# apache/cloudberry

Hardware: NVIDIA H100
Metric: TPC-H SF100 Q1 rows/sec (higher is better)
Workload: dtype int64

## Files before the change

### cloudberry_b200/capi.py

```python
import ctypes as C
import os
import re

import numpy as np

from . import plan as P
from .relation import HostRelation, NP_DTYPE

HERE = os.path.dirname(os.path.abspath(__file__))
ROOT = os.path.dirname(HERE)
_GPU = None
_EXEC = None


class CbgpuError(RuntimeError):
    def __init__(self, code, msg):
        super().__init__("cbgpu error %d: %s" % (code, msg))
        self.code = code


class CbgpuVisimapEntry(C.Structure):
    _fields_ = [("first_row_num", C.c_int64), ("data", C.c_void_p), ("len", C.c_int32)]


class CbgpuPairs(C.Structure):
    _fields_ = [("npairs", C.c_int64), ("outer_idx", C.c_void_p), ("inner_idx", C.c_void_p)]


class CbpOp(C.Structure):
    _fields_ = [("code", C.c_int32), ("a", C.c_int32), ("imm", C.c_int64)]


class CbpColumn(C.Structure):
    _fields_ = [("data", C.c_void_p), ("nulls", C.c_void_p), ("dict_hash", C.c_void_p), ("type", C.c_int32), ("src", C.c_int32)]


class CbgpuJoinFilter(C.Structure):
    _fields_ = [("ncols", C.c_int32), ("cols", C.POINTER(CbpColumn)), ("nops", C.c_int32), ("ops", C.POINTER(CbpOp))]


(CBP_END, CBP_LOAD, CBP_CONST, CBP_ADD, CBP_SUB, CBP_MUL, CBP_FADD, CBP_FSUB, CBP_FMUL, CBP_I2F, CBP_EQ, CBP_NE, CBP_LT, CBP_LE,
 CBP_GT, CBP_GE, CBP_FEQ, CBP_FNE, CBP_FLT, CBP_FLE, CBP_FGT, CBP_FGE, CBP_AND, CBP_OR, CBP_NOT, CBP_FILTER, CBP_PROBE, CBP_DUP,
 CBP_POP, CBP_F8ORD) = range(30)


def join_filter(cols, ops):
    ca = (CbpColumn * max(len(cols), 1))()
    for i, (rel, c, src) in enumerate(cols):
        L = rel.ctx.L
        ca[i] = CbpColumn(L.cbgpu_rel_col_devptr(rel.h, c), L.cbgpu_rel_nulls_dev(rel.h, c), L.cbgpu_rel_dict_hash_dev(rel.h, c),
                          L.cbgpu_rel_col_type(rel.h, c), src)
    oa = (CbpOp * max(len(ops), 1))(*[CbpOp(code, a, imm) for code, a, imm in ops])
    f = CbgpuJoinFilter(len(cols), ca, len(ops), oa)
    f._keep = (ca, oa)
    return f


class CbAggStateDatum(C.Structure):
    _fields_ = [("n", C.c_int64), ("lo", C.c_int64), ("hi", C.c_int64)]


TUPSER_STATE_NUMERIC, TUPSER_STATE_INT8 = 101, 102


class CbTupAttr(C.Structure):
    _fields_ = [("type", C.c_int32), ("dscale", C.c_int32), ("bpchar_len", C.c_int32), ("ntexts", C.c_int32),
                ("texts", C.POINTER(C.c_char_p)), ("text_lens", C.POINTER(C.c_int32)), ("state", C.POINTER(CbAggStateDatum))]


def _tup_attrs(attrs):
    arr = (CbTupAttr * max(len(attrs), 1))()
    keep = []
    for i, a in enumerate(attrs):
        arr[i].type, arr[i].dscale, arr[i].bpchar_len = a[0], a[1], a[2]
        if a[0] in (TUPSER_STATE_NUMERIC, TUPSER_STATE_INT8):
            st = CbAggStateDatum()
            keep.append(st)
            arr[i].state = C.pointer(st)
        texts = a[3] if len(a) > 3 and a[3] is not None else []
        if texts:
            bufs = [C.create_string_buffer(bytes(t), len(t)) for t in texts]
            ptrs = (C.c_char_p * len(texts))(*[C.cast(b, C.c_char_p) for b in bufs])
            lens = (C.c_int32 * len(texts))(*[len(t) for t in texts])
            keep += [bufs, ptrs, lens]
            arr[i].ntexts = len(texts)
            arr[i].texts = ptrs
            arr[i].text_lens = lens
    return arr, keep


def tupser_rows(attrs, rows, nulls=None, max_chunk=8160, end=True):
    L = ex()
    n = len(attrs)
    arr, keep = _tup_attrs(attrs)
    out = bytearray()
    buf = C.create_string_buffer(1 << 20)
    for r, row in enumerate(rows):
        cells, held = [], []
        for i, v in enumerate(row):
            if attrs[i][0] in (TUPSER_STATE_NUMERIC, TUPSER_STATE_INT8) and v is not None:
                st = CbAggStateDatum(*[int(x) for x in v])
                held.append(st)
                cells.append(C.addressof(st))
            else:
                cells.append(0 if v is None else int(v))
        vals = (C.c_int64 * max(n, 1))(*cells)
        isn = (C.c_uint8 * max(n, 1))(*([int(x) for x in nulls[r]] if nulls is not None else [0] * n))
        k = L.cb_tupser_row(arr, n, vals, isn, max_chunk, buf, len(buf))
        if k < 0:
            raise CbgpuError(int(k), "cb_tupser_row failed")
        out += buf.raw[:k]
    if end:
        k = L.cb_tupser_end_of_stream(buf, len(buf))
        out += buf.raw[:k]
    return bytes(out)


def tupser_parse(attrs, data):
    L = ex()
    n = len(attrs)
    arr, keep = _tup_attrs(attrs)
    buf = C.create_string_buffer(bytes(data), len(data))
    pos = 0
    rows, nulls = [], []
    vals = (C.c_int64 * max(n, 1))()
    isn = (C.c_uint8 * max(n, 1))()
    used = C.c_int64()
    while True:
        rc = L.cb_tupser_next(arr, n, C.byref(buf, pos), len(data) - pos, C.byref(used), vals, isn)
        if rc == 1:
            row = []
            for i in range(n):
                if attrs[i][0] in (TUPSER_STATE_NUMERIC, TUPSER_STATE_INT8) and not isn[i]:
                    st = arr[i].state.contents
                    row.append((int(st.n), int(st.lo), int(st.hi)))
                else:
                    row.append(int(vals[i]))
            rows.append(row)
            nulls.append([int(isn[i]) for i in range(n)])
            pos += used.value
            continue
        if rc == 0:
            return rows, nulls, pos + used.value, True
        if rc == -1:
            return rows, nulls, pos, False
        raise CbgpuError(int(rc), "cb_tupser_next: malformed chunk stream at byte %d" % pos)


class CbAocsColumnSpec(C.Structure):
    _fields_ = [("relcol", C.c_int32), ("filenum", C.c_int32), ("attlen", C.c_int32), ("varkind", C.c_int32), ("typalign", C.c_int32),
                ("compresstype", C.c_int32), ("eof", C.c_int64), ("dict", C.c_void_p)]


def aocs_column_spec(c):
    return CbAocsColumnSpec(*c[:7], c[7].h if len(c) > 7 and c[7] is not None else None)


def aocs_dict_collect_segfile(ctx, basepath, segno, checksum, col):
    spec = aocs_column_spec(col)
    err = C.create_string_buffer(512)
    rc = ex().cb_aocs_dict_collect_segfile(ctx.h, os.fsencode(basepath), segno, 1 if checksum else 0, C.byref(spec), err, 512)
    if rc != 0:
        raise CbgpuError(rc, err.value.decode() or ctx.error())


def aocs_segfile_path(basepath, segno, filenum):
    buf = C.create_string_buffer(4096)
    if ex().cb_aocs_segfile_path(os.fsencode(basepath), segno, filenum, buf, 4096) != 0:
        return None
    return os.fsdecode(buf.value)


class DeviceDict:

    def __init__(self, ctx, max_entries=4096, arena_bytes=1 << 20, bpchar=True):
        self.ctx = ctx
        h = C.c_void_p()
        ctx.check(ctx.L.cbgpu_dict_create(ctx.h, max_entries, arena_bytes, 1 if bpchar else 0, C.byref(h)))
        self.h = h

    def collect(self, file_bytes, checksum, compresstype=0, typalign=4):
        buf = np.frombuffer(file_bytes, dtype=np.uint8)
        self.ctx.check(self.ctx.L.cbgpu_aocs_dict_collect(self.ctx.h, buf.ctypes.data, len(buf), 1 if checksum else 0, compresstype, typalign,
                                                          self.h))

    def finalize(self):
        n = C.c_int32()
        self.ctx.check(self.ctx.L.cbgpu_dict_finalize(self.h, C.byref(n)))
        return int(n.value)

    def entries(self):
        out = []
        n = self.finalize()
        p = C.c_void_p()
        ln = C.c_int32()
        f = self.ctx.L.cbgpu_dict_entry
        f.argtypes = [C.c_void_p, C.c_int32, C.POINTER(C.c_void_p), C.POINTER(C.c_int32)]
        for i in range(n):
            self.ctx.check(f(self.h, i, C.byref(p), C.byref(ln)))
            out.append(C.string_at(p.value, ln.value))
        return out

    def lookup(self, text):
        b = text if isinstance(text, bytes) else text.encode()
        return int(self.ctx.L.cbgpu_dict_lookup(self.h, b, len(b)))

    def free(self):
        if self.h:
            self.ctx.L.cbgpu_dict_free(self.h)
            self.h = None


class CbNumericDatum(C.Structure):
    _fields_ = [("lo", C.c_int64), ("hi", C.c_int64), ("dscale", C.c_int32), ("text", C.c_char * 84)]


class CbTupleTableSlot(C.Structure):
    _fields_ = [("tts_empty", C.c_bool), ("tts_nvalid", C.c_int32), ("tts_types", C.POINTER(C.c_int32)),
                ("tts_values", C.POINTER(C.c_int64)), ("tts_isnull", C.POINTER(C.c_bool)),
                ("tts_state_n", C.POINTER(C.c_int64)), ("tts_state_lo", C.POINTER(C.c_int64)),
                ("tts_state_hi", C.POINTER(C.c_int64))]


class CbInstrumentation(C.Structure):
    _fields_ = [("ntuples", C.c_double), ("nloops", C.c_double), ("kernels", C.c_int64), ("device_ms", C.c_double),
                ("rows_in", C.c_int64), ("motion_repartitions", C.c_int64), ("hashjoin_nbatch", C.c_int64), ("agg_npartitions", C.c_int64)]


class CbPlanState(C.Structure):
    pass


CbPlanState._fields_ = [
    ("type", C.c_int), ("plan", C.POINTER(P.CbPlan)), ("state", C.c_void_p), ("ExecProcNode", C.c_void_p),
    ("instrument", CbInstrumentation), ("lefttree", C.POINTER(CbPlanState)), ("righttree", C.POINTER(CbPlanState)),
    ("ps_ResultTupleSlot", C.POINTER(CbTupleTableSlot)), ("squelched", C.c_bool), ("priv", C.c_void_p),
]


class CbEState(C.Structure):
    _fields_ = [("es_ctx", C.c_void_p), ("es_nrels", C.c_int32), ("es_range_table", C.POINTER(C.c_void_p)),
                ("es_segindex", C.c_int32), ("es_numsegments", C.c_int32), ("es_interconnect", C.c_void_p),
                ("es_errcode", C.c_int32), ("es_errmsg", C.c_char * 512), ("es_error_hook", C.c_void_p),
                ("es_force_generic", C.c_int32), ("es_processed", C.c_int64), ("es_cluster", C.c_void_p),
                ("es_interrupt_pending", C.c_void_p), ("es_interrupt_arg", C.c_void_p), ("es_operator_mem_kb", C.c_int64),
                ("es_hashjoin_batches_run", C.c_int64), ("es_agg_partitions_run", C.c_int64)]


def header_symbols(header):
    text = open(os.path.join(ROOT, "include", header)).read()
    text = re.sub(r"/\*.*?\*/", "", text, flags=re.S)
    names = set()
    for m in re.finditer(r"\b((?:cbgpu|cb)_[A-Za-z0-9_]+)\s*\(", text):
        name = m.group(1)
        if name.startswith(("cb_type_width",)):
            continue
        names.add(name)
    return sorted(names)


def build():
    import subprocess
    subprocess.check_call(["make", "-s", "-C", os.path.join(HERE, "csrc"), "-j8", "all"])


def _preload_bundled_nccl():
    try:
        import importlib.util
        spec = importlib.util.find_spec("nvidia.nccl")
        for d in (spec.submodule_search_locations if spec else []):
            cand = os.path.join(d, "lib", "libnccl.so.2")
            if os.path.exists(cand):
                C.CDLL(cand, mode=C.RTLD_GLOBAL)
                return
    except Exception:
        pass


def gpu():
    global _GPU
    if _GPU is None:
        so = os.path.join(os.environ.get("CBGPU_LIBDIR") or HERE, "libcbgpu.so")
        if not os.path.exists(so):
            raise CbgpuError(-1, "libcbgpu.so is not built (run __graft_entry__.build()); there is no CPU fallback")
        _preload_bundled_nccl()
        L = C.CDLL(so, mode=C.RTLD_GLOBAL)
        vp, i32, i64, u64, dbl = C.c_void_p, C.c_int32, C.c_int64, C.c_uint64, C.c_double
        sig = {
            "cbgpu_ctx_create": (C.c_int, [C.c_int, C.POINTER(vp)]),
            "cbgpu_ctx_destroy": (None, [vp]),
            "cbgpu_last_error": (C.c_char_p, [vp]),
            "cbgpu_sync": (C.c_int, [vp]),
            "cbgpu_check_status": (C.c_int, [vp]),
            "cbgpu_device_count": (C.c_int, []),
            "cbgpu_sm_count": (C.c_int, [vp]),
            "cbgpu_kernel_launches": (i64, [vp]),
            "cbgpu_timer_start": (C.c_int, [vp]),
            "cbgpu_timer_stop_ms": (C.c_int, [vp, C.POINTER(dbl)]),
            "cbgpu_last_kernel_ms": (dbl, [vp]),
            "cbgpu_last_kernel_name": (C.c_char_p, [vp]),
            "cbgpu_kernel_log_reset": (None, [vp]),
            "cbgpu_kernel_log_longest": (C.c_int, [vp, C.c_char_p, C.c_int, C.POINTER(dbl)]),
            "cbgpu_trace_begin": (C.c_int, [vp]),
            "cbgpu_trace_end": (C.c_int, [vp]),
            "cbgpu_trace_get": (C.c_int, [vp, C.c_int, C.c_char_p, C.c_int, C.POINTER(dbl)]),
            "cbgpu_flush_l2": (C.c_int, [vp]),
            "cbgpu_host_alloc": (vp, [C.c_size_t]),
            "cbgpu_host_free": (None, [vp]),
            "cbgpu_hashbpchar": (C.c_uint32, [C.c_char_p, i32]),
            "cbgpu_rel_create": (C.c_int, [vp, i64, i32, C.POINTER(i32), C.POINTER(i32), C.POINTER(vp)]),
            "cbgpu_rel_free": (None, [vp]),
            "cbgpu_rel_nrows": (i64, [vp]),
            "cbgpu_rel_ncols": (i32, [vp]),
            "cbgpu_rel_col_type": (i32, [vp, i32]),
            "cbgpu_rel_col_dscale": (i32, [vp, i32]),
            "cbgpu_rel_load_column": (C.c_int, [vp, i32, vp, vp]),
            "cbgpu_rel_load_column_narrow": (C.c_int, [vp, i32, vp, i32]),
            "cbgpu_rel_read_column": (C.c_int, [vp, i32, i64, i64, vp, vp]),
            "cbgpu_rel_set_visimap": (C.c_int, [vp, vp]),
            "cbgpu_rel_read_visimap": (C.c_int, [vp, vp]),
            "cbgpu_dict_create": (C.c_int, [vp, i32, i64, i32, C.POINTER(vp)]),
            "cbgpu_dict_free": (None, [vp]),
            "cbgpu_aocs_dict_collect": (C.c_int, [vp, vp, i64, i32, i32, i32, vp]),
            "cbgpu_dict_finalize": (C.c_int, [vp, C.POINTER(i32)]),
            "cbgpu_dict_entry": (C.c_int, [vp, i32, C.POINTER(C.c_char_p), C.POINTER(i32)]),
            "cbgpu_dict_lookup": (i32, [vp, C.c_char_p, i32]),
            "cbgpu_aocs_decode_dict_column": (C.c_int, [vp, vp, i64, i32, i32, i32, vp, vp, i32, i64, C.POINTER(i64)]),
            "cbgpu_aocs_apply_visimap": (C.c_int, [vp, vp, i64, i32, vp, i32, vp, i64, C.POINTER(i64)]),
            "cbgpu_rel_set_dict_hash": (C.c_int, [vp, i32, vp, i32]),
            "cbgpu_rel_set_nrows": (C.c_int, [vp, i64]),
            "cbgpu_rel_copy_rows": (C.c_int, [vp, i64, vp, i64, i64]),
            "cbgpu_rel_col_devptr": (vp, [vp, i32]),
            "cbgpu_rel_nbytes": (C.c_size_t, [vp]),
            "cbgpu_ht_build": (C.c_int, [vp, vp, C.POINTER(i32), i32, C.POINTER(vp)]),
            "cbgpu_ht_free": (None, [vp]),
            "cbgpu_ht_nrows": (i64, [vp]),
            "cbgpu_ht_has_duplicates": (C.c_int, [vp]),
            "cbgpu_ht_probe_pairs": (C.c_int, [vp, vp, vp, C.POINTER(i32), i32, vp, i64, vp]),
            "cbgpu_ht_probe_pairs_outer": (C.c_int, [vp, vp, vp, C.POINTER(i32), i32, i32, i32, vp]),
            "cbgpu_ht_build_batched": (C.c_int, [vp, vp, C.POINTER(i32), i32, i32, C.POINTER(vp)]),
            "cbgpu_ht_nbatch": (C.c_int, [vp]),
            "cbgpu_ht_load_batch": (C.c_int, [vp, i32]),
            "cbgpu_ht_probe_pairs_batched": (C.c_int, [vp, vp, vp, C.POINTER(i32), i32, i32, i32, vp, vp, vp, C.POINTER(i64)]),
            "cbgpu_ht_probe_pairs_filtered": (C.c_int, [vp, vp, vp, C.POINTER(i32), i32, i32, C.POINTER(CbgpuJoinFilter), vp, vp, vp,
                                                        C.POINTER(i64)]),
            "cbgpu_rel_nulls_dev": (vp, [vp, i32]),
            "cbgpu_rel_dict_hash_dev": (vp, [vp, i32]),
            "cbgpu_pairs_free": (None, [vp]),
            "cbgpu_merge_sorted_runs": (C.c_int, [vp, vp, C.POINTER(i32), C.POINTER(i32), C.POINTER(i32), i32, i32, C.POINTER(vp),
                                                  C.POINTER(i32)]),
            "cbgpu_dev_free": (None, [vp, vp]),
            "cbgpu_read_u32": (C.c_int, [vp, vp, i64, vp]),
            "cbgpu_motion_unique_id": (C.c_int, [vp]),
            "cbgpu_motion_create": (C.c_int, [vp, C.c_int, C.c_int, vp, C.POINTER(vp)]),
            "cbgpu_motion_create_boot": (C.c_int, [vp, C.c_int, C.c_int, vp, vp, C.POINTER(vp)]),
            "cbgpu_motion_destroy": (None, [vp]),
            "cbgpu_motion_abort": (None, [vp]),
            "cbgpu_motion_host_syncs": (i64, [vp]),
            "cbgpu_motion_collectives": (i64, [vp]),
            "cbgpu_motion_bytes_sent": (i64, [vp]),
            "cbgpu_motion_direct_bytes": (i64, [vp]),
            "cbgpu_motion_direct_available": (C.c_int, [vp]),
            "cbgpu_gen_lineitem": (C.c_int, [vp, vp, u64, i64, i64, i64]),
            "cbgpu_gen_orders": (C.c_int, [vp, vp, u64, i64, i64]),
            "cbgpu_gen_customer": (C.c_int, [vp, vp, u64]),
            "cbgpu_gen_supplier": (C.c_int, [vp, vp, u64]),
            "cbgpu_aocs_decode_column": (C.c_int, [vp, vp, i64, i32, i32, i32, i32, vp, i32, i64, C.POINTER(i64)]),
            "cbgpu_aocs_decode_column_ex": (C.c_int, [vp, vp, i64, i32, i32, i32, i32, i32, vp, i32, i64, C.POINTER(i64)]),
            "cbgpu_gen_customer_range": (C.c_int, [vp, vp, u64, i64]),
            "cbgpu_gen_supplier_range": (C.c_int, [vp, vp, u64, i64]),
            "cbgpu_gen_ssb_lineorder": (C.c_int, [vp, vp, u64, i64, i64, i64, i64]),
        }
        for name, (res, args) in sig.items():
            f = getattr(L, name)
            f.restype = res
            f.argtypes = args
        _GPU = L
    return _GPU


def ex():
    global _EXEC
    if _EXEC is None:
        gpu()
        so = os.path.join(os.environ.get("CBGPU_LIBDIR") or HERE, "libcbexec.so")
        if not os.path.exists(so):
            raise CbgpuError(-1, "libcbexec.so is not built (run __graft_entry__.build())")
        L = C.CDLL(so)
        vp = C.c_void_p
        L.cb_CreateExecutorState.restype = C.POINTER(CbEState)
        L.cb_CreateExecutorState.argtypes = [vp, C.POINTER(vp), C.c_int32]
        L.cb_FreeExecutorState.argtypes = [C.POINTER(CbEState)]
        L.cb_estate_error.restype = C.c_char_p
        L.cb_estate_error.argtypes = [C.POINTER(CbEState)]
        L.cb_ExecInitNode.restype = C.POINTER(CbPlanState)
        L.cb_ExecInitNode.argtypes = [C.POINTER(P.CbPlan), C.POINTER(CbEState), C.c_int]
        L.cb_ExecProcNode.restype = C.POINTER(CbTupleTableSlot)
        L.cb_ExecProcNode.argtypes = [C.POINTER(CbPlanState)]
        L.cb_MultiExecProcNode.restype = vp
        L.cb_MultiExecProcNode.argtypes = [C.POINTER(CbPlanState)]
        L.cb_ExecProcNodeBatch.restype = C.c_int
        L.cb_ExecProcNodeBatch.argtypes = [C.POINTER(CbPlanState), C.POINTER(vp)]
        for n in ("cb_ExecEndNode", "cb_ExecReScan", "cb_ExecSquelchNode"):
            getattr(L, n).restype = None
            getattr(L, n).argtypes = [C.POINTER(CbPlanState)]
        L.cb_slot_text.restype = C.c_int
        L.cb_slot_text.argtypes = [C.POINTER(CbTupleTableSlot), C.c_int, C.c_char_p, C.c_int]
        L.cb_slot_float8.restype = C.c_double
        L.cb_slot_float8.argtypes = [C.POINTER(CbTupleTableSlot), C.c_int]
        L.cb_numeric_sum_text.argtypes = [C.c_int64, C.c_int64, C.c_int32, C.c_char_p, C.c_int32]
        L.cb_numeric_avg_text.argtypes = [C.c_int64, C.c_int64, C.c_int32, C.c_int64, C.c_char_p, C.c_int32]
        L.cb_interconnect_nccl_create.restype = vp
        L.cb_interconnect_nccl_create.argtypes = [vp]
        L.cb_interconnect_destroy.argtypes = [vp]
        L.cb_aocs_segfile_path.restype = C.c_int
        L.cb_aocs_segfile_path.argtypes = [C.c_char_p, C.c_int, C.c_int, C.c_char_p, C.c_size_t]
        L.cb_aocs_dict_collect_segfile.restype = C.c_int
        L.cb_aocs_dict_collect_segfile.argtypes = [vp, C.c_char_p, C.c_int, C.c_int, C.POINTER(CbAocsColumnSpec), C.c_char_p, C.c_size_t]
        L.cb_aocs_load_segfile.restype = C.c_int
        L.cb_aocs_load_segfile.argtypes = [vp, C.c_char_p, C.c_int, C.c_int, C.c_int, C.POINTER(CbAocsColumnSpec), vp, C.c_int64,
                                           C.POINTER(CbgpuVisimapEntry), C.c_int, C.POINTER(C.c_int64), C.POINTER(C.c_int64),
                                           C.c_char_p, C.c_size_t]
        L.cb_tupser_row.restype = C.c_int64
        L.cb_tupser_row.argtypes = [C.POINTER(CbTupAttr), C.c_int, C.POINTER(C.c_int64), C.POINTER(C.c_uint8), C.c_int, vp, C.c_int64]
        L.cb_tupser_end_of_stream.restype = C.c_int
        L.cb_tupser_end_of_stream.argtypes = [vp, C.c_int64]
        L.cb_tupser_next.restype = C.c_int64
        L.cb_tupser_next.argtypes = [C.POINTER(CbTupAttr), C.c_int, vp, C.c_int64, C.POINTER(C.c_int64), C.POINTER(C.c_int64),
                                     C.POINTER(C.c_uint8)]
        L.cb_cluster_create.restype = vp
        L.cb_cluster_create.argtypes = [vp, C.c_int32]
        L.cb_cluster_set_range_table.restype = C.c_int
        L.cb_cluster_set_range_table.argtypes = [vp, C.c_int32, C.POINTER(vp), C.c_int32]
        L.cb_cluster_estate.restype = C.POINTER(CbEState)
        L.cb_cluster_estate.argtypes = [vp, C.c_int32]
        L.cb_cluster_init_plan.restype = C.c_int
        L.cb_cluster_init_plan.argtypes = [vp, C.POINTER(P.CbPlan)]
        L.cb_cluster_next.restype = C.POINTER(CbTupleTableSlot)
        L.cb_cluster_next.argtypes = [vp]
        L.cb_cluster_current_segment.restype = C.c_int32
        L.cb_cluster_current_segment.argtypes = [vp]
        L.cb_cluster_end.argtypes = [vp]
        L.cb_cluster_destroy.argtypes = [vp]
        L.cb_cluster_error.restype = C.c_char_p
        L.cb_cluster_error.argtypes = [vp]
        _EXEC = L
    return _EXEC


def hashbpchar(text):
    b = text.encode() if isinstance(text, str) else text
    return int(gpu().cbgpu_hashbpchar(b, len(b)))


class Context:
    def __init__(self, device=0):
        self.L = gpu()
        h = C.c_void_p()
        rc = self.L.cbgpu_ctx_create(device, C.byref(h))
        self.h = h
        if rc:
            raise CbgpuError(rc, self.error())

    def error(self):
        return (self.L.cbgpu_last_error(self.h) or b"").decode()

    def check(self, rc):
        if rc:
            raise CbgpuError(rc, self.error())

    def sync(self):
        self.check(self.L.cbgpu_sync(self.h))

    def launches(self):
        return int(self.L.cbgpu_kernel_launches(self.h))

    def timer_start(self):
        self.check(self.L.cbgpu_timer_start(self.h))

    def timer_stop_ms(self):
        ms = C.c_double()
        self.check(self.L.cbgpu_timer_stop_ms(self.h, C.byref(ms)))
        return ms.value

    def last_kernel(self):
        return (self.L.cbgpu_last_kernel_name(self.h) or b"").decode(), float(self.L.cbgpu_last_kernel_ms(self.h))

    def kernel_log_reset(self):
        self.L.cbgpu_kernel_log_reset(self.h)

    def longest_kernel(self):
        buf = C.create_string_buffer(128)
        ms = C.c_double()
        self.check(self.L.cbgpu_kernel_log_longest(self.h, buf, 128, C.byref(ms)))
        return buf.value.decode(), ms.value

    def trace_begin(self):
        self.check(self.L.cbgpu_trace_begin(self.h))

    def trace_end(self):
        n = self.L.cbgpu_trace_end(self.h)
        out = []
        buf = C.create_string_buffer(128)
        ms = C.c_double()
        for i in range(n):
            self.check(self.L.cbgpu_trace_get(self.h, i, buf, 128, C.byref(ms)))
            out.append((buf.value.decode(), ms.value))
        return out

    def flush_l2(self):
        self.check(self.L.cbgpu_flush_l2(self.h))

    def sm_count(self):
        return int(self.L.cbgpu_sm_count(self.h))

    def close(self):
        if self.h:
            self.L.cbgpu_ctx_destroy(self.h)
            self.h = None


ALLGATHER_FN = C.CFUNCTYPE(C.c_int, C.c_void_p, C.c_void_p, C.c_void_p, C.c_size_t)


class Motion:

    @staticmethod
    def unique_id():
        buf = C.create_string_buffer(128)
        rc = gpu().cbgpu_motion_unique_id(buf)
        if rc:
            raise CbgpuError(rc, "ncclGetUniqueId failed")
        return buf.raw

    def __init__(self, ctx, rank, nranks, unique_id=None, allgather=None):
        self.ctx = ctx
        self.rank = rank
        self.nranks = nranks
        h = C.c_void_p()
        if unique_id is not None:
            buf = C.create_string_buffer(unique_id, 128)
            ctx.check(ctx.L.cbgpu_motion_create(ctx.h, rank, nranks, buf, C.byref(h)))
        else:
            def _cb(_arg, mine, allp, nbytes):
                try:
                    parts = allgather(C.string_at(mine, nbytes))
                    if len(parts) != nranks or any(len(x) != nbytes for x in parts):
                        return 1
                    C.memmove(allp, b"".join(parts), nbytes * nranks)
                    return 0
                except Exception:
                    return 1
            self._cb = ALLGATHER_FN(_cb)
            ctx.check(ctx.L.cbgpu_motion_create_boot(ctx.h, rank, nranks, C.cast(self._cb, C.c_void_p), None, C.byref(h)))
        self.h = h

    def bytes_sent(self):
        return int(self.ctx.L.cbgpu_motion_bytes_sent(self.h)) + int(self.ctx.L.cbgpu_motion_direct_bytes(self.h))

    def direct(self):
        return bool(self.ctx.L.cbgpu_motion_direct_available(self.h))

    def host_syncs(self):
        return int(self.ctx.L.cbgpu_motion_host_syncs(self.h))

    def collectives(self):
        return int(self.ctx.L.cbgpu_motion_collectives(self.h))

    def close(self):
        if self.h:
            self.ctx.L.cbgpu_motion_destroy(self.h)
            self.h = None

    def abort(self):
        if self.h:
            self.ctx.L.cbgpu_motion_abort(self.h)
            self.h = None


class DeviceRelation:

    def __init__(self, ctx, nrows, types, dscales=None, name="rel"):
        self.ctx = ctx
        self.name = name
        self.types = list(types)
        self.dscales = list(dscales) if dscales is not None else [2 if t == P.NUMERIC else 0 for t in types]
        n = len(types)
        h = C.c_void_p()
        ctx.check(ctx.L.cbgpu_rel_create(ctx.h, nrows, n, (C.c_int32 * n)(*self.types), (C.c_int32 * n)(*self.dscales),
                                         C.byref(h)))
        self.h = h
        self.nrows = nrows

    @classmethod
    def adopt(cls, ctx, handle, name="batch"):
        L = ctx.L
        d = cls.__new__(cls)
        d.ctx = ctx
        d.name = name
        d.h = C.c_void_p(handle) if not isinstance(handle, C.c_void_p) else handle
        n = int(L.cbgpu_rel_ncols(d.h))
        d.types = [int(L.cbgpu_rel_col_type(d.h, i)) for i in range(n)]
        d.dscales = [int(L.cbgpu_rel_col_dscale(d.h, i)) for i in range(n)]
        d.nrows = int(L.cbgpu_rel_nrows(d.h))
        return d

    @classmethod
    def from_host(cls, ctx, rel: HostRelation):
        d = cls(ctx, rel.nrows, rel.types, rel.dscales, rel.name)
        d.load(rel)
        return d

    def load(self, rel: HostRelation, sync=True):
        L = self.ctx.L
        for i, col in enumerate(rel.columns):
            nl = rel.nulls[i]
            if nl is not None:
                nl = np.ascontiguousarray(nl, dtype=np.uint8)
            self.ctx.check(L.cbgpu_rel_load_column(self.h, i, col.ctypes.data, nl.ctypes.data if nl is not None else None))
            if rel.dict_hashes[i] is not None:
                dh = np.ascontiguousarray(rel.dict_hashes[i], dtype=np.uint32)
                self.ctx.check(L.cbgpu_rel_set_dict_hash(self.h, i, dh.ctypes.data, len(dh)))
        if rel.visimap is not None:
            vm = np.ascontiguousarray(rel.visimap, dtype=np.uint8)
            self.ctx.check(L.cbgpu_rel_set_visimap(self.h, vm.ctypes.data))
        if sync:
            self.ctx.sync()

    def load_aocs_column(self, col, file_bytes, checksum, attlen, varkind=0, typalign=4, row_offset=0, compresstype=0):
        buf = np.frombuffer(file_bytes, dtype=np.uint8)
        n = C.c_int64()
        self.ctx.check(self.ctx.L.cbgpu_aocs_decode_column_ex(self.ctx.h, buf.ctypes.data, len(buf), 1 if checksum else 0, compresstype,
                                                              attlen, varkind, typalign, self.h, col, row_offset, C.byref(n)))
        return int(n.value)

    def load_aocs_dict_column(self, col, file_bytes, checksum, dictionary, compresstype=0, typalign=4, row_offset=0):
        buf = np.frombuffer(file_bytes, dtype=np.uint8)
        n = C.c_int64()
        self.ctx.check(self.ctx.L.cbgpu_aocs_decode_dict_column(self.ctx.h, buf.ctypes.data, len(buf), 1 if checksum else 0, compresstype,
                                                                typalign, dictionary.h, self.h, col, row_offset, C.byref(n)))
        return int(n.value)

    def apply_visimap(self, file_bytes, checksum, entries, row_offset=0):
        buf = np.frombuffer(file_bytes, dtype=np.uint8)
        arr = (CbgpuVisimapEntry * max(len(entries), 1))()
        keep = []
        for i, (first, payload) in enumerate(entries):
            arr[i].first_row_num = first
            if payload is None:
                arr[i].data = None
                arr[i].len = 0
            else:
                b = C.create_string_buffer(bytes(payload), len(payload))
                keep.append(b)
                arr[i].data = C.cast(b, C.c_void_p)
                arr[i].len = len(payload)
        n = C.c_int64()
        self.ctx.check(self.ctx.L.cbgpu_aocs_apply_visimap(self.ctx.h, buf.ctypes.data, len(buf), 1 if checksum else 0, arr, len(entries),
                                                           self.h, row_offset, C.byref(n)))
        return int(n.value)

    def load_segfile(self, basepath, segno, checksum, cols, entries=(), row_offset=0):
        specs = (CbAocsColumnSpec * len(cols))(*[aocs_column_spec(c) for c in cols])
        arr = (CbgpuVisimapEntry * max(len(entries), 1))()
        keep = []
        for i, (first, payload) in enumerate(entries):
            arr[i].first_row_num = first
            if payload is not None:
                b = C.create_string_buffer(bytes(payload), len(payload))
                keep.append(b)
                arr[i].data = C.cast(b, C.c_void_p)
                arr[i].len = len(payload)
        n, h = C.c_int64(), C.c_int64()
        err = C.create_string_buffer(512)
        rc = ex().cb_aocs_load_segfile(self.ctx.h, os.fsencode(basepath), segno, 1 if checksum else 0, len(cols), specs, self.h, row_offset,
                                       arr, len(entries), C.byref(n), C.byref(h), err, 512)
        if rc != 0:
            raise CbgpuError(rc, err.value.decode() or self.ctx.error())
        return int(n.value), int(h.value)

    def read_visimap(self):
        out = np.zeros((self.rows() + 7) // 8, dtype=np.uint8)
        self.ctx.check(self.ctx.L.cbgpu_rel_read_visimap(self.h, out.ctypes.data))
        return np.unpackbits(out, bitorder="little")[:self.rows()].astype(bool)

    def load_column_ptr(self, col, host_ptr, host_width=None):
        if host_width is None or host_width == P.TYPE_WIDTH[self.types[col]]:
            self.ctx.check(self.ctx.L.cbgpu_rel_load_column(self.h, col, host_ptr, None))
        else:
            self.ctx.check(self.ctx.L.cbgpu_rel_load_column_narrow(self.h, col, host_ptr, host_width))

    def set_dict_hash(self, col, hashes):
        dh = np.ascontiguousarray(hashes, dtype=np.uint32)
        self.ctx.check(self.ctx.L.cbgpu_rel_set_dict_hash(self.h, col, dh.ctypes.data, len(dh)))

    def read_column(self, col, lo=0, hi=None):
        hi = self.rows() if hi is None else hi
        out = np.empty(hi - lo, dtype=NP_DTYPE[self.types[col]])
        nulls = np.zeros(hi - lo, dtype=np.uint8)
        self.ctx.check(self.ctx.L.cbgpu_rel_read_column(self.h, col, lo, hi, out.ctypes.data, nulls.ctypes.data))
        return out, nulls

    def rows(self):
        return int(self.ctx.L.cbgpu_rel_nrows(self.h))

    def nbytes(self):
        return int(self.ctx.L.cbgpu_rel_nbytes(self.h))

    def free(self):
        if self.h:
            self.ctx.L.cbgpu_rel_free(self.h)
            self.h = None


def _slot_row(E, slot):
    s = slot.contents
    row, states = [], []
    buf = C.create_string_buffer(160)
    for i in range(s.tts_nvalid):
        states.append((s.tts_state_n[i], ((s.tts_state_hi[i] << 64) | (s.tts_state_lo[i] & (2 ** 64 - 1)))))
        if s.tts_isnull[i]:
            row.append(None)
            continue
        t = s.tts_types[i]
        if t == P.FLOAT8:
            row.append(E.cb_slot_float8(slot, i + 1))
        elif t in (P.NUMERIC, P.NUMERIC128):
            E.cb_slot_text(slot, i + 1, buf, 160)
            row.append(buf.value.decode())
        else:
            row.append(int(s.tts_values[i]))
    return row, states


class Result:
    def __init__(self):
        self.rows = []
        self.states = []
        self.segments = []
        self.instrument = {}


def _collect_instrument(ps, out):
    if not ps:
        return
    n = ps.contents
    ins = n.instrument
    out[n.plan.contents.plan_node_id] = {"node": n.type, "ntuples": ins.ntuples, "kernels": ins.kernels,
                                         "device_ms": ins.device_ms, "rows_in": ins.rows_in,
                                         "motion_repartitions": ins.motion_repartitions, "hashjoin_nbatch": ins.hashjoin_nbatch,
                                         "agg_npartitions": ins.agg_npartitions}
    _collect_instrument(n.lefttree, out)
    _collect_instrument(n.righttree, out)


class Executor:

    def __init__(self, ctx, range_table, force_generic=False, motion=None, operator_mem_kb=0):
        self.ctx = ctx
        self.E = ex()
        n = len(range_table)
        arr = (C.c_void_p * max(n, 1))(*[r.h for r in range_table])
        self.estate = self.E.cb_CreateExecutorState(ctx.h, arr, n)
        self.estate.contents.es_force_generic = 1 if force_generic else 0
        self.estate.contents.es_operator_mem_kb = int(operator_mem_kb)
        self._keep = [arr, range_table]
        self.ic = None
        if motion is not None:
            self.ic = self.E.cb_interconnect_nccl_create(motion.h)
            self.estate.contents.es_interconnect = self.ic
            self.estate.contents.es_segindex = motion.rank
            self.estate.contents.es_numsegments = motion.nranks
            self._keep.append(motion)

    def run(self, plan_node):
        E = self.E
        es = self.estate
        es.contents.es_errcode = 0
        ps = E.cb_ExecInitNode(P.plan_ptr(plan_node), es, 0)
        if not ps:
            raise CbgpuError(es.contents.es_errcode, E.cb_estate_error(es).decode())
        res = Result()
        try:
            while True:
                slot = E.cb_ExecProcNode(ps)
                if es.contents.es_errcode:
                    raise CbgpuError(es.contents.es_errcode, E.cb_estate_error(es).decode())
                if not slot or slot.contents.tts_empty:
                    break
                row, st = _slot_row(E, slot)
                res.rows.append(row)
                res.states.append(st)
                res.segments.append(0)
            _collect_instrument(ps, res.instrument)
        finally:
            E.cb_ExecEndNode(ps)
        return res

    def run_batch(self, plan_node, name="batch"):
        E = self.E
        es = self.estate
        es.contents.es_errcode = 0
        ps = E.cb_ExecInitNode(P.plan_ptr(plan_node), es, 0)
        if not ps:
            raise CbgpuError(es.contents.es_errcode, E.cb_estate_error(es).decode())
        try:
            h = C.c_void_p()
            rc = E.cb_ExecProcNodeBatch(ps, C.byref(h))
            if rc or es.contents.es_errcode:
                raise CbgpuError(rc or es.contents.es_errcode, E.cb_estate_error(es).decode())
            return DeviceRelation.adopt(self.ctx, h, name)
        finally:
            E.cb_ExecEndNode(ps)

    def close(self):
        if self.estate:
            self.E.cb_FreeExecutorState(self.estate)
            self.estate = None
        if self.ic:
            self.E.cb_interconnect_destroy(self.ic)
            self.ic = None


class Cluster:

    def __init__(self, ctx, segment_range_tables, force_generic=False):
        self.ctx = ctx
        self.E = ex()
        self.nsegs = len(segment_range_tables)
        self.h = self.E.cb_cluster_create(ctx.h, self.nsegs)
        self._keep = []
        for s, rt in enumerate(segment_range_tables):
            arr = (C.c_void_p * max(len(rt), 1))(*[r.h for r in rt])
            self._keep += [arr, rt]
            rc = self.E.cb_cluster_set_range_table(self.h, s, arr, len(rt))
            if rc:
                raise CbgpuError(rc, "bad range table")
            self.E.cb_cluster_estate(self.h, s).contents.es_force_generic = 1 if force_generic else 0

    def run(self, plan_node):
        E = self.E
        rc = E.cb_cluster_init_plan(self.h, P.plan_ptr(plan_node))
        if rc:
            msg = E.cb_cluster_error(self.h).decode()
            E.cb_cluster_end(self.h)
            raise CbgpuError(rc, msg)
        res = Result()
        try:
            while True:
                slot = E.cb_cluster_next(self.h)
                err = E.cb_cluster_error(self.h)
                if err:
                    raise CbgpuError(-1, err.decode())
                if not slot or slot.contents.tts_empty:
                    break
                row, st = _slot_row(E, slot)
                res.rows.append(row)
                res.states.append(st)
                res.segments.append(int(E.cb_cluster_current_segment(self.h)))
        finally:
            E.cb_cluster_end(self.h)
        return res

    def close(self):
        if self.h:
            self.E.cb_cluster_destroy(self.h)
            self.h = None
```

### cloudberry_b200/csrc/common.cuh

```cuda
#pragma once

#include <cuda_runtime.h>
#include <stdint.h>
#include <stdio.h>
#include <string.h>

#include "../../include/cbgpu.h"

#include <stdlib.h>
#include <string.h>

#define CB_MAX_COLS_REL 64

struct cbgpu_ctx
{
	int			device;
	cudaStream_t stream;
	char		err[512];
	int			sm_count;
	int64_t		launches;
	cudaEvent_t ev_t0, ev_t1, ev_k0, ev_k1;
	double		last_kernel_ms;
	const char *last_kernel_name;
	bool		kernel_timed;
#define CB_KLOG 32
	cudaEvent_t klog_ev[CB_KLOG][2];
	const char *klog_name[CB_KLOG];
	int			klog_n;
	bool		klog_ready;
#define CB_TRACE 1024
	bool		trace_on;
	int			trace_n;
	cudaEvent_t *trace_ev;
	const char *trace_name[CB_TRACE];
	void	   *flush_buf;
	size_t		flush_bytes;
	int		   *d_status;
	int		   *h_status;
	int64_t		status_seen_at;
	bool		opt_debug, opt_pf_spec;
	int			opt_bloom_div;
#define CB_SCRATCH_SLOTS 7
	void	   *scratch[CB_SCRATCH_SLOTS];
	size_t		scratch_bytes[CB_SCRATCH_SLOTS];
#define CB_EARLY_CACHE 16
	struct
	{
		const void *keydata;
		int64_t		nrows;
		const void *red0;
		int			worth;
	}			early_cache[CB_EARLY_CACHE];
	int			early_cache_n;
	uint64_t	pf_cache[32];
	int			pf_cache_n;
	int			opt_pf_keep_div;
	int64_t		opt_pf_min_rows;
	struct AggSnap *agg_snap;
	void	   *small_dev;
	size_t		small_dev_bytes;
};

static inline void *
cb_scratch(cbgpu_ctx *ctx, int slot, size_t bytes)
{
	if (ctx->scratch_bytes[slot] < bytes)
	{
		free(ctx->scratch[slot]);
		ctx->scratch[slot] = malloc(bytes);
		ctx->scratch_bytes[slot] = ctx->scratch[slot] ? bytes : 0;
	}
	if (ctx->scratch[slot])
		memset(ctx->scratch[slot], 0, bytes);
	return ctx->scratch[slot];
}

struct cbgpu_rel
{
	cbgpu_ctx  *ctx;
	int64_t		nrows;
	int64_t		capacity;
	int32_t		ncols;
	int32_t		types[CB_MAX_COLS_REL];
	int32_t		dscales[CB_MAX_COLS_REL];
	void	   *data[CB_MAX_COLS_REL];
	uint8_t	   *nulls[CB_MAX_COLS_REL];
	uint32_t   *dict_hash[CB_MAX_COLS_REL];
	int32_t		dict_n[CB_MAX_COLS_REL];
	uint8_t	   *visimap;
	bool		owns[CB_MAX_COLS_REL];
	void	   *slab;
};

struct AggDev
{
	uint32_t	mask;
	int32_t		nkeys;
	int32_t		naccs;
	int32_t		npart;
	int32_t		part_shift;
	int32_t		part_id;
	int32_t    *state;
	uint32_t   *hash;
	int64_t    *keys;
	uint32_t   *keynull;
	int64_t    *n;
	unsigned long long *sum;
	int32_t    *ngroups;
	int32_t    *full;
};

#define AGG_SNAP_MAXG 64
#define AGG_SNAP_MAXCAP 4096
struct AggSnap
{
	int32_t		ngroups;
	int32_t		full;
	int32_t		anynull;
	int32_t		retry;
	int32_t		audit;
	int32_t		pad[3];
	uint32_t	keynull[AGG_SNAP_MAXG];
	int64_t		keys[AGG_SNAP_MAXG][CBP_MAX_KEYS];
	int64_t		n[AGG_SNAP_MAXG][CBP_MAX_AGGS];
	int64_t		lo[AGG_SNAP_MAXG][CBP_MAX_AGGS];
	int64_t		hi[AGG_SNAP_MAXG][CBP_MAX_AGGS];
};

struct cbgpu_aggtable
{
	cbgpu_ctx  *ctx;
	AggDev		d;
	void	   *base;
	int64_t		capacity;
	int32_t		kinds[CBP_MAX_AGGS];
	bool		counted;
	int64_t		ngroups;
	int32_t		anynull;
	bool		snap_valid;
	AggSnap    *snap;
};

#ifdef __CUDACC__
__device__ __forceinline__ void
agg_snapshot_block(const AggDev &t, AggSnap *out)
{
	__shared__ int s_n,
				s_an;
	const size_t cap = (size_t) t.mask + 1;

	if (threadIdx.x == 0)
	{
		s_n = 0;
		s_an = 0;
	}
	__syncthreads();
	for (size_t i = threadIdx.x; i < cap; i += blockDim.x)
	{
		if (((volatile int32_t *) t.state)[i] != 2)
			continue;
		const int	g = atomicAdd(&s_n, 1);

		if (t.keynull[i])
			s_an = 1;
		if (g >= AGG_SNAP_MAXG)
			continue;
		out->keynull[g] = t.keynull[i];
		for (int k = 0; k < t.nkeys; k++)
			out->keys[g][k] = t.keys[i * t.nkeys + k];
		for (int a = 0; a < t.naccs; a++)
		{
			out->n[g][a] = ((volatile int64_t *) t.n)[i * t.naccs + a];
			out->lo[g][a] = (int64_t) ((volatile unsigned long long *) t.sum)[(i * t.naccs + a) * 2];
			out->hi[g][a] = (int64_t) ((volatile unsigned long long *) t.sum)[(i * t.naccs + a) * 2 + 1];
		}
	}
	__syncthreads();
	if (threadIdx.x == 0)
	{
		out->full = *(volatile int32_t *) t.full;
		out->anynull = s_an;
		out->ngroups = s_n;
	}
	__threadfence_system();
}
#endif
void		cb_agg_adopt_snapshot(cbgpu_aggtable *t, const AggSnap *snap);


#ifdef __CUDACC__
#define CB_HD_DECL __host__ __device__ __forceinline__
#else
#define CB_HD_DECL static inline
#endif
#define HT_EMPTY 0xFFFFFFFFFFFFFFFFull
struct HtDev
{
	unsigned long long *slots;
	uint32_t	mask;
	uint32_t   *bloom;
	uint32_t	bloom_mask;
	int32_t		nkeys;
	const void *keydata[CBP_MAX_KEYS];
	const uint8_t *keynulls[CBP_MAX_KEYS];
	const uint32_t *keydict[CBP_MAX_KEYS];
	int32_t		keytype[CBP_MAX_KEYS];
	int32_t		keyslot;
	int32_t		nbatch;
	int32_t		batch_shift;
	int32_t		batch_id;
};

CB_HD_DECL bool
ht_in_batch(int32_t nbatch, int32_t batch_shift, int32_t batch_id, uint32_t hash)
{
	return nbatch <= 1 || (int32_t) (hash >> batch_shift) == batch_id;
}

CB_HD_DECL bool
ht_key_in_domain(int32_t keyslot, int64_t key)
{
	return keyslot == 1 ? key == (int64_t) (int32_t) key : (uint64_t) key <= 0xFFFFFFFFull;
}

struct cbgpu_hashtable
{
	cbgpu_ctx  *ctx;
	HtDev		d;
	cbgpu_rel  *inner;
	int64_t		nslots;
	int64_t		ninserted;
	int		   *d_flags;
	int			has_dups;
	int64_t		total_rows;
	int64_t		built_bytes;
};

static inline int
cb_fail(cbgpu_ctx *ctx, int code, const char *fmt, const char *a = "", long long b = 0)
{
	if (ctx)
		snprintf(ctx->err, sizeof(ctx->err), fmt, a, b);
	return code;
}

#define CB_CUDA(ctx, call) \
	do { \
		cudaError_t e__ = (call); \
		if (e__ != cudaSuccess) \
		{ \
			if (ctx) \
				snprintf((ctx)->err, sizeof((ctx)->err), "%s:%d: %s: %s", __FILE__, __LINE__, #call, cudaGetErrorString(e__)); \
			(void) cudaGetLastError();	 \
			 \
			return e__ == cudaErrorMemoryAllocation ? CBGPU_ERR_NOMEM : CBGPU_ERR_CUDA; \
		} \
	} while (0)

void		cb_trace_mark(cbgpu_ctx *ctx, const char *name);
#define CB_LAUNCHED(ctx, name) \
	do { \
		(ctx)->launches++; \
		if ((ctx)->trace_on) \
			cb_trace_mark(ctx, name); \
		cudaError_t e__ = cudaGetLastError(); \
		if (e__ != cudaSuccess) \
		{ \
			snprintf((ctx)->err, sizeof((ctx)->err), "launch %s: %s", name, cudaGetErrorString(e__)); \
			return CBGPU_ERR_CUDA; \
		} \
	} while (0)

int			cb_check_status(cbgpu_ctx *ctx, const char *what);
#define CB_STATUS_RIDE(ctx) cudaMemcpyAsync((ctx)->h_status, (ctx)->d_status, sizeof(int), cudaMemcpyDeviceToHost, (ctx)->stream)
#define CB_STATUS_FETCHED(ctx) ((ctx)->status_seen_at = (ctx)->launches)

static inline int
cb_type_w(int t)
{
	return cb_type_width((CbTypeId) t);
}

#define CB_HD __host__ __device__ __forceinline__

CB_HD uint32_t
pg_rot(uint32_t x, int k)
{
	return (x << k) | (x >> (32 - k));
}

#define PG_FINAL(a, b, c) \
	do { \
		c ^= b; c -= pg_rot(b, 14); \
		a ^= c; a -= pg_rot(c, 11); \
		b ^= a; b -= pg_rot(a, 25); \
		c ^= b; c -= pg_rot(b, 16); \
		a ^= c; a -= pg_rot(c, 4); \
		b ^= a; b -= pg_rot(a, 14); \
		c ^= b; c -= pg_rot(b, 24); \
	} while (0)

#define PG_MIX(a, b, c) \
	do { \
		a -= c; a ^= pg_rot(c, 4); c += b; \
		b -= a; b ^= pg_rot(a, 6); a += c; \
		c -= b; c ^= pg_rot(b, 8); b += a; \
		a -= c; a ^= pg_rot(c, 16); c += b; \
		b -= a; b ^= pg_rot(a, 19); a += c; \
		c -= b; c ^= pg_rot(b, 4); b += a; \
	} while (0)

CB_HD uint32_t
pg_hash_uint32(uint32_t k)
{
	uint32_t	a, b, c;

	a = b = c = 0x9e3779b9u + (uint32_t) sizeof(uint32_t) + 3923095u;
	a += k;
	PG_FINAL(a, b, c);
	return c;
}

CB_HD uint32_t
pg_hashint8(int64_t val)
{
	uint32_t	lohalf = (uint32_t) val;
	uint32_t	hihalf = (uint32_t) ((uint64_t) val >> 32);

	lohalf ^= (val >= 0) ? hihalf : ~hihalf;
	return pg_hash_uint32(lohalf);
}

CB_HD uint32_t
pg_hash_bytes8(uint32_t w0, uint32_t w1)
{
	uint32_t	a, b, c;

	a = b = c = 0x9e3779b9u + 8u + 3923095u;
	b += w1;
	a += w0;
	PG_FINAL(a, b, c);
	return c;
}

CB_HD uint32_t
pg_hash_bpchar1(uint8_t ch)
{
	uint32_t	a, b, c;
	uint32_t	len = (ch == (uint8_t) ' ') ? 0u : 1u;

	a = b = c = 0x9e3779b9u + len + 3923095u;
	if (len)
		a += ch;
	PG_FINAL(a, b, c);
	return c;
}

CB_HD uint32_t
pg_hashfloat8(uint64_t bits)
{
	if ((bits << 1) == 0)
		return 0;
	if (((bits >> 52) & 0x7ff) == 0x7ff && (bits & 0xfffffffffffffull) != 0)
		bits = 0x7ff8000000000000ull;
	return pg_hash_bytes8((uint32_t) bits, (uint32_t) (bits >> 32));
}

static inline uint32_t
pg_hash_bytes_host(const unsigned char *k, int keylen)
{
	uint32_t	a, b, c;
	int			len = keylen;

	a = b = c = 0x9e3779b9u + (uint32_t) len + 3923095u;
	while (len >= 12)
	{
		a += (k[0] + ((uint32_t) k[1] << 8) + ((uint32_t) k[2] << 16) + ((uint32_t) k[3] << 24));
		b += (k[4] + ((uint32_t) k[5] << 8) + ((uint32_t) k[6] << 16) + ((uint32_t) k[7] << 24));
		c += (k[8] + ((uint32_t) k[9] << 8) + ((uint32_t) k[10] << 16) + ((uint32_t) k[11] << 24));
		PG_MIX(a, b, c);
		k += 12;
		len -= 12;
	}
	switch (len)
	{
		case 11: c += ((uint32_t) k[10] << 24);
		case 10: c += ((uint32_t) k[9] << 16);
		case 9:  c += ((uint32_t) k[8] << 8);
		case 8:  b += ((uint32_t) k[7] << 24);
		case 7:  b += ((uint32_t) k[6] << 16);
		case 6:  b += ((uint32_t) k[5] << 8);
		case 5:  b += k[4];
		case 4:  a += ((uint32_t) k[3] << 24);
		case 3:  a += ((uint32_t) k[2] << 16);
		case 2:  a += ((uint32_t) k[1] << 8);
		case 1:  a += k[0];
	}
	PG_FINAL(a, b, c);
	return c;
}

CB_HD uint32_t
pg_murmurhash32(uint32_t h)
{
	h ^= h >> 16;
	h *= 0x85ebca6bu;
	h ^= h >> 13;
	h *= 0xc2b2ae35u;
	h ^= h >> 16;
	return h;
}

CB_HD uint32_t
pg_hash_combine(uint32_t acc, uint32_t h, bool isnull)
{
	acc = (acc << 1) | (acc >> 31);
	return isnull ? acc : (acc ^ h);
}

CB_HD int32_t
pg_jump_consistent_hash(uint64_t key, int32_t num_segments)
{
	int64_t		b = -1;
	int64_t		j = 0;

	while (j < num_segments)
	{
		b = j;
		key = key * 2862933555777941757ULL + 1;
#ifdef __CUDA_ARCH__
		double		q = __ddiv_rn((double) (1LL << 31), (double) ((key >> 33) + 1));

		j = (int64_t) __dmul_rn((double) (b + 1), q);
#else
		double		q = (double) (1LL << 31) / (double) ((key >> 33) + 1);

		j = (int64_t) ((double) (b + 1) * q);
#endif
	}
	return (int32_t) b;
}

__device__ __forceinline__ uint32_t
pg_hash_datum(int type, int64_t v, const uint32_t *dict)
{
	switch (type)
	{
		case CB_INT4: case CB_DATE:
			return pg_hash_uint32((uint32_t) (int32_t) v);
		case CB_INT8:
			return pg_hashint8(v);
		case CB_FLOAT8:
			return pg_hashfloat8((uint64_t) v);
		case CB_BPCHAR1:
			return pg_hash_bpchar1((uint8_t) v);
		case CB_DICT8: case CB_DICT32:
			return dict ? __ldg(dict + v) : 0u;
		case CB_BOOL:
			return pg_hash_uint32((uint32_t) (int32_t) (int8_t) v);
		default:
			return 0u;
	}
}

CB_HD uint32_t
jh_mix32(uint32_t x)
{
	x ^= x >> 16;
	x *= 0x7feb352du;
	x ^= x >> 15;
	x *= 0x846ca68bu;
	x ^= x >> 16;
	return x;
}

CB_HD uint32_t
jh_int8(int64_t val)
{
	uint32_t	lohalf = (uint32_t) val;
	const uint32_t hihalf = (uint32_t) ((uint64_t) val >> 32);

	lohalf ^= (val >= 0) ? hihalf : ~hihalf;
	return jh_mix32(lohalf);
}

#ifdef __CUDACC__
__device__ __forceinline__ uint32_t
jh_hash_datum(int type, int64_t v, const uint32_t *dict)
{
	switch (type)
	{
		case CB_INT4: case CB_DATE:
			return jh_mix32((uint32_t) (int32_t) v);
		case CB_INT8:
			return jh_int8(v);
		default:
			return pg_hash_datum(type, v, dict);
	}
}
#endif

CB_HD uint32_t
ht_bloom_bits(uint32_t h, uint32_t *word, uint32_t bloom_mask)
{
	const uint32_t m1 = h * 0x9e3779b1u;
	const uint32_t m2 = h * 0x85ebca6bu;

	*word = (m1 >> 4) & bloom_mask;
	return (1u << (m2 >> 27)) | (1u << ((m2 >> 22) & 31));
}

#ifdef __CUDACC__
__device__ __forceinline__ uint64_t
l2_policy_evict_first(void)
{
	uint64_t	p;

	asm volatile("createpolicy.fractional.L2::evict_first.b64 %0, 1.0;" : "=l"(p));
	return p;
}

__device__ __forceinline__ uint64_t
l2_policy_evict_last(void)
{
	uint64_t	p;

	asm volatile("createpolicy.fractional.L2::evict_last.b64 %0, 1.0;" : "=l"(p));
	return p;
}

__device__ __forceinline__ uint32_t
ldg_hint_u32(const uint32_t *a, uint64_t pol)
{
	uint32_t	v;

	asm volatile("ld.global.nc.L2::cache_hint.u32 %0, [%1], %2;" : "=r"(v) : "l"(a), "l"(pol));
	return v;
}

// ... 171 lines not shown
```

### cloudberry_b200/csrc/ctx.cu

```cuda
#include "common.cuh"

#include <nvtx3/nvToolsExt.h>

#include <stdlib.h>

extern "C" int
cbgpu_device_count(void)
{
	int			n = 0;

	if (cudaGetDeviceCount(&n) != cudaSuccess)
		return 0;
	return n;
}

extern "C" int
cbgpu_ctx_create(int device, cbgpu_ctx **out)
{
	cbgpu_ctx  *ctx = (cbgpu_ctx *) calloc(1, sizeof(cbgpu_ctx));
	cudaDeviceProp prop;

	if (!ctx)
		return CBGPU_ERR_NOMEM;
	*out = ctx;
	ctx->device = device;
	CB_CUDA(ctx, cudaSetDevice(device));
	CB_CUDA(ctx, cudaGetDeviceProperties(&prop, device));
	ctx->sm_count = prop.multiProcessorCount;
	CB_CUDA(ctx, cudaStreamCreateWithFlags(&ctx->stream, cudaStreamNonBlocking));
	{
		cudaMemPool_t pool;
		unsigned long long keep = ~0ull;

		CB_CUDA(ctx, cudaDeviceGetDefaultMemPool(&pool, device));
		CB_CUDA(ctx, cudaMemPoolSetAttribute(pool, cudaMemPoolAttrReleaseThreshold, &keep));
	}
	CB_CUDA(ctx, cudaEventCreate(&ctx->ev_t0));
	CB_CUDA(ctx, cudaEventCreate(&ctx->ev_t1));
	CB_CUDA(ctx, cudaEventCreate(&ctx->ev_k0));
	CB_CUDA(ctx, cudaEventCreate(&ctx->ev_k1));
	CB_CUDA(ctx, cudaMalloc(&ctx->d_status, sizeof(int)));
	CB_CUDA(ctx, cudaMemsetAsync(ctx->d_status, 0, sizeof(int), ctx->stream));
	CB_CUDA(ctx, cudaMallocHost(&ctx->h_status, sizeof(int)));
	*ctx->h_status = 0;
	CB_CUDA(ctx, cudaMallocHost(&ctx->agg_snap, sizeof(AggSnap)));
	memset(ctx->agg_snap, 0, sizeof(AggSnap));
	ctx->opt_debug = getenv("CBGPU_DEBUG") != NULL;
	ctx->opt_pf_spec = getenv("CBGPU_PF_SPEC") != NULL;
	ctx->opt_pf_keep_div = getenv("CBGPU_PREFILTER_KEEP_DIV") && atoi(getenv("CBGPU_PREFILTER_KEEP_DIV")) > 0 ? atoi(getenv("CBGPU_PREFILTER_KEEP_DIV")) : 12;
	ctx->opt_pf_min_rows = getenv("CBGPU_PREFILTER_MIN_ROWS") ? atoll(getenv("CBGPU_PREFILTER_MIN_ROWS")) : ((int64_t) 16 << 20);
	ctx->opt_bloom_div = getenv("CBGPU_BLOOM_DIV") && atoi(getenv("CBGPU_BLOOM_DIV")) > 0 ? atoi(getenv("CBGPU_BLOOM_DIV")) : 2;
	ctx->flush_bytes = (size_t) 512 << 20;
	ctx->flush_buf = NULL;
	return CBGPU_OK;
}

extern "C" void
cbgpu_ctx_destroy(cbgpu_ctx *ctx)
{
	if (!ctx)
		return;
	cudaSetDevice(ctx->device);
	cudaStreamSynchronize(ctx->stream);
	if (ctx->flush_buf)
		cudaFree(ctx->flush_buf);
	cudaFree(ctx->d_status);
	cudaFreeHost(ctx->h_status);
	cudaFreeHost(ctx->agg_snap);
	if (ctx->small_dev)
		cudaFree(ctx->small_dev);
	for (int i = 0; i < CB_SCRATCH_SLOTS; i++)
		free(ctx->scratch[i]);
	cudaEventDestroy(ctx->ev_t0);
	cudaEventDestroy(ctx->ev_t1);
	cudaEventDestroy(ctx->ev_k0);
	cudaEventDestroy(ctx->ev_k1);
	cudaStreamDestroy(ctx->stream);
	free(ctx);
}

extern "C" const char *
cbgpu_last_error(cbgpu_ctx *ctx)
{
	return ctx ? ctx->err : "no context";
}

extern "C" void
cbgpu_range_push(const char *name)
{
	nvtxRangePushA(name);
}

extern "C" void
cbgpu_range_pop(void)
{
	nvtxRangePop();
}

extern "C" int
cbgpu_sync(cbgpu_ctx *ctx)
{
	CB_CUDA(ctx, cudaStreamSynchronize(ctx->stream));
	return CBGPU_OK;
}

int
cb_check_status(cbgpu_ctx *ctx, const char *what)
{
	if (ctx->status_seen_at != ctx->launches)
	{
		CB_CUDA(ctx, CB_STATUS_RIDE(ctx));
		CB_CUDA(ctx, cudaStreamSynchronize(ctx->stream));
		CB_STATUS_FETCHED(ctx);
	}
	if (*ctx->h_status != 0)
	{
		int			code = *ctx->h_status;

		CB_CUDA(ctx, cudaMemsetAsync(ctx->d_status, 0, sizeof(int), ctx->stream));
		*ctx->h_status = 0;
		snprintf(ctx->err, sizeof(ctx->err), "%s: %s", what,
				 code == CBGPU_ERR_OVERFLOW ? "value out of range (integer/numeric overflow)" :
				 code == CBGPU_ERR_NOMEM ? "device table or output buffer full" :
				 code == CBGPU_ERR_CORRUPT ? "stored block fails its checksum" :
				 code == CBGPU_ERR_PEER ? "a peer segment did not signal within the interconnect's time limit" : "device-side error");
		if (code > 0 || code < CBGPU_ERR_INTERRUPTED)
		{
			snprintf(ctx->err, sizeof(ctx->err), "%s: device status word holds %d, not an error code of this library", what, code);
			return CBGPU_ERR_CUDA;
		}
		return code;
	}
	return CBGPU_OK;
}

extern "C" int
cbgpu_check_status(cbgpu_ctx *ctx)
{
	return cb_check_status(ctx, "GPU pipeline");
}

extern "C" int
cbgpu_sm_count(cbgpu_ctx *ctx)
{
	return ctx->sm_count;
}

extern "C" int64_t
cbgpu_kernel_launches(cbgpu_ctx *ctx)
{
	return ctx->launches;
}

extern "C" int
cbgpu_timer_start(cbgpu_ctx *ctx)
{
	CB_CUDA(ctx, cudaEventRecord(ctx->ev_t0, ctx->stream));
	return CBGPU_OK;
}

extern "C" int
cbgpu_timer_stop_ms(cbgpu_ctx *ctx, double *ms)
{
	float		f = 0;

	CB_CUDA(ctx, cudaEventRecord(ctx->ev_t1, ctx->stream));
	CB_CUDA(ctx, cudaEventSynchronize(ctx->ev_t1));
	CB_CUDA(ctx, cudaEventElapsedTime(&f, ctx->ev_t0, ctx->ev_t1));
	*ms = f;
	return CBGPU_OK;
}

extern "C" double
cbgpu_last_kernel_ms(cbgpu_ctx *ctx)
{
	float		f = 0;

	if (!ctx->kernel_timed)
		return -1.0;
	if (cudaEventSynchronize(ctx->ev_k1) != cudaSuccess)
		return -1.0;
	if (cudaEventElapsedTime(&f, ctx->ev_k0, ctx->ev_k1) != cudaSuccess)
		return -1.0;
	return f;
}

int
cb_klog_begin(cbgpu_ctx *ctx, const char *name)
{
	int			i = ctx->klog_n;

	if (i >= CB_KLOG)
		return -1;
	if (!ctx->klog_ready)
	{
		for (int k = 0; k < CB_KLOG; k++)
		{
			cudaEventCreate(&ctx->klog_ev[k][0]);
			cudaEventCreate(&ctx->klog_ev[k][1]);
		}
		ctx->klog_ready = true;
	}
	ctx->klog_name[i] = name;
	cudaEventRecord(ctx->klog_ev[i][0], ctx->stream);
	ctx->klog_n = i + 1;
	return i;
}

void
cb_klog_end(cbgpu_ctx *ctx, int i)
{
	if (i >= 0)
		cudaEventRecord(ctx->klog_ev[i][1], ctx->stream);
}

void
cb_trace_mark(cbgpu_ctx *ctx, const char *name)
{
	if (ctx->trace_n >= CB_TRACE)
		return;
	ctx->trace_name[ctx->trace_n] = name;
	cudaEventRecord(ctx->trace_ev[ctx->trace_n + 1], ctx->stream);
	ctx->trace_n++;
}

extern "C" int
cbgpu_trace_begin(cbgpu_ctx *ctx)
{
	if (!ctx->trace_ev)
	{
		ctx->trace_ev = (cudaEvent_t *) calloc(CB_TRACE + 1, sizeof(cudaEvent_t));
		if (!ctx->trace_ev)
			return CBGPU_ERR_NOMEM;
		for (int i = 0; i <= CB_TRACE; i++)
			CB_CUDA(ctx, cudaEventCreate(&ctx->trace_ev[i]));
	}
	ctx->trace_n = 0;
	ctx->trace_on = true;
	CB_CUDA(ctx, cudaEventRecord(ctx->trace_ev[0], ctx->stream));
	return CBGPU_OK;
}

extern "C" int
cbgpu_trace_end(cbgpu_ctx *ctx)
{
	ctx->trace_on = false;
	CB_CUDA(ctx, cudaStreamSynchronize(ctx->stream));
	return ctx->trace_n;
}

extern "C" int
cbgpu_trace_get(cbgpu_ctx *ctx, int i, char *name, int namelen, double *ms)
{
	float		f = 0;

	if (i < 0 || i >= ctx->trace_n)
		return CBGPU_ERR_INVALID;
	CB_CUDA(ctx, cudaEventElapsedTime(&f, ctx->trace_ev[i], ctx->trace_ev[i + 1]));
	*ms = f;
	if (name && namelen > 0)
		snprintf(name, (size_t) namelen, "%s", ctx->trace_name[i]);
	return CBGPU_OK;
}

extern "C" void
cbgpu_kernel_log_reset(cbgpu_ctx *ctx)
{
	ctx->klog_n = 0;
}

extern "C" int
cbgpu_kernel_log_longest(cbgpu_ctx *ctx, char *name, int namelen, double *ms)
{
	float		best = -1.f;
	int			bi = -1;

	CB_CUDA(ctx, cudaStreamSynchronize(ctx->stream));
	for (int i = 0; i < ctx->klog_n; i++)
	{
		float		f = 0;

		if (cudaEventElapsedTime(&f, ctx->klog_ev[i][0], ctx->klog_ev[i][1]) == cudaSuccess && f > best)
		{
			best = f;
			bi = i;
		}
	}
	*ms = best;
	if (name && namelen > 0)
		snprintf(name, (size_t) namelen, "%s", bi >= 0 ? ctx->klog_name[bi] : "");
	return CBGPU_OK;
}

extern "C" const char *
cbgpu_last_kernel_name(cbgpu_ctx *ctx)
{
	return ctx->last_kernel_name ? ctx->last_kernel_name : "";
}

__global__ void
k_flush_fill(uint4 *p, size_t n, uint32_t v)
{
	size_t		i = (size_t) blockIdx.x * blockDim.x + threadIdx.x;
	size_t		stride = (size_t) gridDim.x * blockDim.x;

	for (; i < n; i += stride)
		p[i] = make_uint4(v, v, v, v);
}

extern "C" int
cbgpu_flush_l2(cbgpu_ctx *ctx)
{
	static uint32_t gen = 0;

	if (!ctx->flush_buf)
		CB_CUDA(ctx, cudaMalloc(&ctx->flush_buf, ctx->flush_bytes));
	k_flush_fill<<<ctx->sm_count * 4, 512, 0, ctx->stream>>>((uint4 *) ctx->flush_buf, ctx->flush_bytes / 16, ++gen);
	CB_LAUNCHED(ctx, "k_flush_fill");
	return CBGPU_OK;
}

extern "C" void *
cbgpu_host_alloc(size_t bytes)
{
	void	   *p = NULL;

	if (cudaMallocHost(&p, bytes ? bytes : 1) != cudaSuccess)
		return NULL;
	return p;
}

// ... 584 lines not shown
```

### cloudberry_b200/csrc/exec/cb_exec.c

```c
#include <stdarg.h>
#include <stdio.h>
#include <stdlib.h>
#include <string.h>

#include "../../../include/cb_exec.h"

static int
es_fail(CbEState *es, int code, const char *fmt,...)
{
	va_list		ap;

	if (es->es_errcode == 0)
	{
		va_start(ap, fmt);
		vsnprintf(es->es_errmsg, sizeof(es->es_errmsg), fmt, ap);
		va_end(ap);
		es->es_errcode = code;
		if (es->es_error_hook)
			es->es_error_hook(es, code, es->es_errmsg);
	}
	return code;
}

#define GPU(es, call) \
// ... 2912 lines not shown
		int32_t		types[CBP_MAX_OUT],
					dscales[CBP_MAX_OUT];
		int			ncols = cbgpu_rel_ncols(rel);
		cbgpu_rel  *small;

		for (int c = 0; c < ncols; c++)
		{
			types[c] = cbgpu_rel_col_type(rel, c);
			dscales[c] = cbgpu_rel_col_dscale(rel, c);
		}
		GPU(es, cbgpu_rel_create(es->es_ctx, nout, ncols, types, dscales, &small));
		p->owned.rels[p->owned.nrels++] = small;
		if (nout > 0)
		{
			void	   *didx;

			GPU(es, cbgpu_dev_alloc(es->es_ctx, sizeof(uint32_t) * (size_t) nout, &didx));
			p->owned.devs[p->owned.ndevs++] = didx;
			GPU(es, cbgpu_dev_write(es->es_ctx, didx, sizeof(uint32_t) * (size_t) nout, idx));
			GPU(es, cbgpu_rel_take_rows(small, rel, (const uint32_t *) didx, nout));
		}
		for (int c = 0; c < ncols; c++)
			if (cbgpu_rel_dict_hash_dev(rel, c))
				GPU(es, cbgpu_rel_share_dict_hash(small, c, rel, c));
		*out_rel = small;
	}
	memcpy(out_shape, shape, sizeof(PExpr) * (size_t) nshape);
	*out_nshape = nshape;
	return CBGPU_OK;
}

static int
limitsort_result(CbPlanState *ps)
{
	cbgpu_rel  *small;
	PExpr		shape[MAX_OUT];
	int			nshape;

	TRY(limitsort_run(ps, &small, shape, &nshape));
	return rel_to_result(ps->state, small, shape, nshape, NULL, 0, &np(ps)->rs);
}

static int
open_limitsort(CbPlanState *ps, CbStream **out)
{
	cbgpu_rel  *small;
	PExpr		shape[MAX_OUT];
	int			nshape;
	CbStream   *s;

	TRY(limitsort_run(ps, &small, shape, &nshape));
	s = stream_new(np(ps));
	TRY(stream_over_rel(ps->state, s, small, shape, nshape));
	*out = s;
	return CBGPU_OK;
}

static int
node_result(CbPlanState *ps)
{
	CbEState   *es = ps->state;
	NodePriv   *p = np(ps);

	if (p->rs)
		return CBGPU_OK;
	if (ps->type == T_CbAgg && !(es->es_operator_mem_kb > 0 && ((CbAgg *) ps->plan)->numCols > 0) && ps->plan->nquals == 0)
		return agg_result(ps);
	if (ps->type == T_CbLimitSort)
		return limitsort_result(ps);
	{
		CbStream   *s;
		cbgpu_rel  *rel;
		PExpr		shape[MAX_OUT];
		int			nshape;

		const uint32_t *sel = NULL;

		TRY(node_open(ps, &s));
		if (stream_is_plain(s, &rel, &sel))
		{
			int			exact = 1,
						c = 0;

			for (int i = 0; i < s->nout && exact; i++)
			{
				PExpr	   *x = &s->pe[s->out[i]];

				shape[i] = *x;
				if (x->kind == PE_STATE)
				{
					if (s->pe[x->cn].kind != PE_COL || s->col_idx[s->pe[x->cn].col] != c)
						exact = 0;
					c += 3;
				}
				else
				{
					if (x->kind != PE_COL || s->col_idx[x->col] != c)
						exact = 0;
					c++;
				}
			}
			if (exact && c == cbgpu_rel_ncols(rel) && !sel)
				return rel_to_result(es, rel, shape, s->nout, NULL, 0, &p->rs);
			if (exact && c == cbgpu_rel_ncols(rel))
			{
				int32_t		types[CBP_MAX_OUT],
							dscales[CBP_MAX_OUT];
				cbgpu_rel  *ordered;

				for (int k = 0; k < c; k++)
				{
					types[k] = cbgpu_rel_col_type(rel, k);
					dscales[k] = cbgpu_rel_col_dscale(rel, k);
				}
				GPU(es, cbgpu_rel_create(es->es_ctx, s->pipe.nrows, c, types, dscales, &ordered));
				p->owned.rels[p->owned.nrels++] = ordered;
				GPU(es, cbgpu_rel_take_rows(ordered, rel, sel, s->pipe.nrows));
				return rel_to_result(es, ordered, shape, s->nout, NULL, 0, &p->rs);
			}
		}
		TRY(stream_materialize(es, ps, s, &p->owned, &rel, shape, &nshape));
		return rel_to_result(es, rel, shape, nshape, NULL, 0, &p->rs);
	}
}

CbEState *
cb_CreateExecutorState(cbgpu_ctx *ctx, cbgpu_rel **range_table, int32_t nrels)
{
	CbEState   *es = calloc(1, sizeof(CbEState));

	es->es_ctx = ctx;
	es->es_nrels = nrels;
	es->es_range_table = calloc((size_t) (nrels ? nrels : 1), sizeof(cbgpu_rel *));
	for (int i = 0; i < nrels; i++)
		es->es_range_table[i] = range_table[i];
	es->es_numsegments = 1;
	return es;
}

void
cb_FreeExecutorState(CbEState *estate)
{
	if (!estate)
		return;
	free(estate->es_range_table);
	free(estate);
}

static CbTupleTableSlot *
make_slot(int natts)
{
	CbTupleTableSlot *slot = calloc(1, sizeof(CbTupleTableSlot));
	size_t		n = (size_t) (natts ? natts : 1);

	slot->tts_empty = true;
	slot->tts_nvalid = natts;
	slot->tts_types = calloc(n, sizeof(int32_t));
	slot->tts_values = calloc(n, sizeof(int64_t));
	slot->tts_isnull = calloc(n, sizeof(bool));
	slot->tts_state_n = calloc(n, sizeof(int64_t));
	slot->tts_state_lo = calloc(n, sizeof(int64_t));
	slot->tts_state_hi = calloc(n, sizeof(int64_t));
	return slot;
}

static void
free_slot(CbTupleTableSlot *slot)
{
	if (!slot)
		return;
	free(slot->tts_types);
	free(slot->tts_values);
	free(slot->tts_isnull);
	free(slot->tts_state_n);
	free(slot->tts_state_lo);
	free(slot->tts_state_hi);
	free(slot);
}

static CbTupleTableSlot *
exec_generic(CbPlanState *ps)
{
	NodePriv   *p = np(ps);
	CbTupleTableSlot *slot = ps->ps_ResultTupleSlot;
	ResultSet  *rs;

	slot->tts_empty = true;
	if (ps->squelched || ps->state->es_errcode)
		return NULL;
	if (ps->type == T_CbHash)
	{
		es_fail(ps->state, CBGPU_ERR_INVALID, "Hash node does not support ExecProcNode call convention");
		return NULL;
	}
	if (!p->rs)
	{
		if (node_result(ps) != CBGPU_OK)
			return NULL;
		ps->instrument.nloops += 1;
	}
	rs = p->rs;
	if (rs->cursor >= rs->nrows)
		return NULL;
	for (int i = 0; i < rs->ncols; i++)
	{
		size_t		o = (size_t) rs->cursor * rs->ncols + i;

		slot->tts_types[i] = rs->types[i];
		slot->tts_values[i] = rs->vals[o];
		slot->tts_isnull[i] = rs->nulls[o];
		slot->tts_state_n[i] = rs->st_n[o];
		slot->tts_state_lo[i] = rs->st_lo[o];
		slot->tts_state_hi[i] = rs->st_hi[o];
	}
	rs->cursor++;
	slot->tts_empty = false;
	ps->instrument.ntuples += 1;
	ps->state->es_processed++;
	return slot;
}

int
cb_ExecProcNodeBatch(CbPlanState *ps, cbgpu_rel **out)
{
	CbEState   *es = ps->state;
	NodePriv   *p = np(ps);
	CbStream   *s;
	cbgpu_rel  *rel = NULL;
	PExpr		shape[MAX_OUT];
	int			nshape;
	int			found = -1;

	*out = NULL;
	if (ps->squelched || es->es_errcode)
		return es->es_errcode ? es->es_errcode : CBGPU_ERR_INVALID;
	if (ps->type == T_CbHash || ps->type == T_CbAgg || ps->type == T_CbLimitSort)
		return es_fail(es, CBGPU_ERR_UNSUPPORTED, "batch output of node type %d (its result is finalised on the host)", (int) ps->type);
	TRY(node_open(ps, &s));
	TRY(stream_materialize_ex(es, ps, s, &p->owned, &rel, shape, &nshape, 2));
	for (int i = 0; i < p->owned.nrels; i++)
		if (p->owned.rels[i] == rel)
			found = i;
	if (found < 0)
		return es_fail(es, CBGPU_ERR_INVALID, "batch output lost track of its relation");
	p->owned.rels[found] = p->owned.rels[--p->owned.nrels];
	ps->instrument.ntuples += (double) cbgpu_rel_nrows(rel);
	ps->instrument.nloops += 1;
	*out = rel;
	return CBGPU_OK;
}

CbPlanState *
cb_ExecInitNode(CbPlan *node, CbEState *estate, int eflags)
{
	CbPlanState *ps;

	(void) eflags;
	if (!node)
		return NULL;
	switch (node->type)
	{
		case T_CbSeqScan: case T_CbHash: case T_CbHashJoin: case T_CbAgg: case T_CbMotion: case T_CbLimitSort:
			break;
		default:
			es_fail(estate, CBGPU_ERR_UNSUPPORTED, "unrecognized / unsupported node type: %d", (int) node->type);
			return NULL;
	}
	ps = calloc(1, sizeof(CbPlanState));
	ps->type = node->type;
	ps->plan = node;
	ps->state = estate;
	ps->ExecProcNode = exec_generic;
	ps->priv = calloc(1, sizeof(NodePriv));
	ps->ps_ResultTupleSlot = make_slot(node->ntargets);
	if (node->lefttree)
	{
		ps->lefttree = cb_ExecInitNode(node->lefttree, estate, eflags);
		if (!ps->lefttree)
			goto fail;
	}
	if (node->righttree)
	{
		ps->righttree = cb_ExecInitNode(node->righttree, estate, eflags);
		if (!ps->righttree)
			goto fail;
	}
	if (node->type != T_CbSeqScan && !ps->lefttree)
	{
		es_fail(estate, CBGPU_ERR_INVALID, "plan node %d needs an outer child", (int) node->type);
		goto fail;
	}
	return ps;
fail:
	cb_ExecEndNode(ps);
	return NULL;
}

CbTupleTableSlot *
cb_ExecProcNode(CbPlanState *node)
{
	return node->ExecProcNode(node);
}

cbgpu_hashtable *
cb_MultiExecProcNode(CbPlanState *node)
{
	if (node->type != T_CbHash)
	{
		es_fail(node->state, CBGPU_ERR_INVALID, "unrecognized node type for MultiExecProcNode: %d", (int) node->type);
		return NULL;
	}
	if (hash_build(node) != CBGPU_OK)
		return NULL;
	return np(node)->ht;
}

static void
node_reset(CbPlanState *node)
{
	NodePriv   *p = np(node);

	rs_free(p->rs);
	p->rs = NULL;
	owned_free(node->state, &p->owned);
	p->stream = NULL;
	p->opened = 0;
	p->ht = NULL;
	p->inner_rel = NULL;
	p->recv = NULL;
	p->recv_ready = 0;
	p->xstage = 0;
}

void
cb_ExecReScan(CbPlanState *node)
{
	if (!node)
		return;
	cb_ExecReScan(node->lefttree);
	cb_ExecReScan(node->righttree);
	node_reset(node);
	node->squelched = false;
}

void
cb_ExecSquelchNode(CbPlanState *node)
{
	if (!node || node->squelched)
		return;
	node->squelched = true;
	cb_ExecSquelchNode(node->lefttree);
	cb_ExecSquelchNode(node->righttree);
}

void
cb_ExecEndNode(CbPlanState *node)
{
	if (!node)
		return;
	cb_ExecEndNode(node->lefttree);
	cb_ExecEndNode(node->righttree);
	if (node->priv)
	{
		node_reset(node);
		free(node->priv);
	}
	free_slot(node->ps_ResultTupleSlot);
	free(node);
}

int
cb_slot_natts(const CbTupleTableSlot *slot)
{
	return slot->tts_nvalid;
}

int
cb_slot_isnull(const CbTupleTableSlot *slot, int attno)
{
	return slot->tts_isnull[attno - 1];
}

int64_t
cb_slot_int64(const CbTupleTableSlot *slot, int attno)
{
	return slot->tts_values[attno - 1];
}

double
cb_slot_float8(const CbTupleTableSlot *slot, int attno)
{
	double		d;

	memcpy(&d, &slot->tts_values[attno - 1], 8);
	return d;
}

int
cb_slot_text(const CbTupleTableSlot *slot, int attno, char *buf, int buflen)
{
	int			i = attno - 1;

	if (slot->tts_isnull[i])
		return snprintf(buf, (size_t) buflen, "NULL");
	switch (slot->tts_types[i])
	{
		case CB_NUMERIC:
		case CB_NUMERIC128:
			return snprintf(buf, (size_t) buflen, "%s", ((CbNumericDatum *) (intptr_t) slot->tts_values[i])->text);
		case CB_FLOAT8:
			return snprintf(buf, (size_t) buflen, "%.17g", cb_slot_float8(slot, attno));
		default:
			return snprintf(buf, (size_t) buflen, "%lld", (long long) slot->tts_values[i]);
	}
}

static int
ic_nccl_redistribute(CbInterconnect *ic, CbEState *es, int32_t motion_id, cbgpu_rel *send, const int64_t *counts,
					 const int64_t *offsets, cbgpu_rel **recv)
{
	(void) motion_id;
	GPU(es, cbgpu_motion_redistribute((cbgpu_motion *) ic->priv, send, counts, offsets, recv));
	return CBGPU_OK;
}

static int
ic_nccl_gather(CbInterconnect *ic, CbEState *es, int32_t motion_id, int32_t root, cbgpu_rel *send, int64_t nrows, cbgpu_rel **recv)
{
	(void) motion_id;
	GPU(es, cbgpu_motion_gather((cbgpu_motion *) ic->priv, root, send, nrows, recv));
	return CBGPU_OK;
}

static int
ic_nccl_broadcast(CbInterconnect *ic, CbEState *es, int32_t motion_id, cbgpu_rel *send, int64_t nrows, cbgpu_rel **recv)
{
	(void) motion_id;
	GPU(es, cbgpu_motion_broadcast((cbgpu_motion *) ic->priv, send, nrows, recv));
	return CBGPU_OK;
}

static int
ic_nccl_direct_begin(CbInterconnect *ic, CbEState *es, int32_t motion_id, int32_t ncols, const int32_t *types, const int32_t *dscales,
					 cbgpu_direct_dest *dest)
{
	(void) motion_id;
	(void) es;
	return cbgpu_motion_direct_begin((cbgpu_motion *) ic->priv, ncols, types, dscales, dest);
}

static int
ic_nccl_direct_end(CbInterconnect *ic, CbEState *es, int32_t motion_id, int32_t local_flags, uint64_t local_nullmask,
				   const int64_t *dev_sent_counts, int64_t *sent_counts, cbgpu_rel **recv, int32_t *outcome)
{
	int			rc;

	(void) motion_id;
	rc = cbgpu_motion_direct_end((cbgpu_motion *) ic->priv, local_flags, local_nullmask, dev_sent_counts, sent_counts, recv, outcome);
	if (rc != CBGPU_OK && es->es_errcode == 0)
		es_fail(es, rc, "%s", cbgpu_last_error(es->es_ctx));
	return rc;
}

static void
ic_nccl_abandon(CbInterconnect *ic, CbEState *es, int32_t motion_id, int32_t after_direct)
{
	(void) motion_id;
	(void) es;
	cbgpu_motion_abandon((cbgpu_motion *) ic->priv, after_direct);
}

CbInterconnect *
cb_interconnect_nccl_create(cbgpu_motion *motion)
{
	CbInterconnect *ic = calloc(1, sizeof(CbInterconnect));

	if (cbgpu_motion_direct_available(motion))
	{
		ic->direct_begin = ic_nccl_direct_begin;
		ic->direct_end = ic_nccl_direct_end;
	}
	ic->name = cbgpu_motion_direct_available(motion) ? "peer-memory windows + nccl" : "nccl";
	ic->nsegs = cbgpu_motion_nranks(motion);
	ic->segindex = cbgpu_motion_rank(motion);
	ic->redistribute = ic_nccl_redistribute;
	ic->gather = ic_nccl_gather;
	ic->broadcast = ic_nccl_broadcast;
	ic->abandon = ic_nccl_abandon;
	ic->priv = motion;
	return ic;
}

void
cb_interconnect_destroy(CbInterconnect *ic)
{
	free(ic);
}

struct CbCluster
{
	cbgpu_ctx  *ctx;
	int			nsegs;
	CbEState  **estates;
	CbPlanState **roots;
	int			cur;
	int			singleton;
	char		err[512];
};

CbCluster *
cb_cluster_create(cbgpu_ctx *ctx, int32_t nsegs)
{
	CbCluster  *c = calloc(1, sizeof(CbCluster));

	c->ctx = ctx;
	c->nsegs = nsegs;
	c->estates = calloc((size_t) nsegs, sizeof(CbEState *));
	c->roots = calloc((size_t) nsegs, sizeof(CbPlanState *));
	for (int s = 0; s < nsegs; s++)
	{
		c->estates[s] = cb_CreateExecutorState(ctx, NULL, 0);
		c->estates[s]->es_segindex = s;
		c->estates[s]->es_numsegments = nsegs;
		c->estates[s]->es_cluster = c;
	}
	return c;
}

int
cb_cluster_set_range_table(CbCluster *c, int32_t seg, cbgpu_rel **range_table, int32_t nrels)
{
	CbEState   *es;

	if (seg < 0 || seg >= c->nsegs)
		return CBGPU_ERR_INVALID;
	es = c->estates[seg];
	free(es->es_range_table);
	es->es_nrels = nrels;
	es->es_range_table = calloc((size_t) (nrels ? nrels : 1), sizeof(cbgpu_rel *));
	for (int i = 0; i < nrels; i++)
		es->es_range_table[i] = range_table[i];
	return CBGPU_OK;
}

CbEState *
cb_cluster_estate(CbCluster *c, int32_t seg)
{
	return (seg >= 0 && seg < c->nsegs) ? c->estates[seg] : NULL;
}

static int
slice_is_singleton(const CbPlan *p)
{
	if (!p)
		return 0;
	if (p->type == T_CbMotion)
	{
		int			t = ((const CbMotion *) p)->motionType;

		return t == CB_MOTIONTYPE_GATHER || t == CB_MOTIONTYPE_GATHER_SINGLE;
	}
	return slice_is_singleton(p->lefttree) || slice_is_singleton(p->righttree);
}

int
cb_cluster_init_plan(CbCluster *c, CbPlan *plan)
{
	for (int s = 0; s < c->nsegs; s++)
	{
		c->roots[s] = cb_ExecInitNode(plan, c->estates[s], 0);
		if (!c->roots[s])
		{
			snprintf(c->err, sizeof(c->err), "segment %d: %.480s", s, c->estates[s]->es_errmsg);
			return c->estates[s]->es_errcode ? c->estates[s]->es_errcode : CBGPU_ERR_INVALID;
		}
	}
	c->singleton = slice_is_singleton(plan);
	c->cur = 0;
	return CBGPU_OK;
}

static CbPlanState *
find_state(CbPlanState *ps, const CbPlan *plan)
{
	CbPlanState *r;

	if (!ps)
		return NULL;
	if (ps->plan == plan)
		return ps;
	r = find_state(ps->lefttree, plan);
	return r ? r : find_state(ps->righttree, plan);
}

static int
cluster_run_motion(CbPlanState *me)
{
	CbCluster  *c = (CbCluster *) me->state->es_cluster;
	CbMotion   *m = (CbMotion *) me->plan;
	int			nsegs = c->nsegs;
	CbPlanState **mps = calloc((size_t) nsegs, sizeof(CbPlanState *));
	cbgpu_rel **send = calloc((size_t) nsegs, sizeof(cbgpu_rel *));
	int64_t    *counts = calloc((size_t) nsegs * (size_t) nsegs, sizeof(int64_t));
	int64_t    *soff = calloc((size_t) nsegs * (size_t) nsegs, sizeof(int64_t));
	int			rc = CBGPU_OK;

// ... 190 lines not shown
```

### cloudberry_b200/csrc/hashtable.cu

```cuda
#include "common.cuh"
#include "pipeline.cuh"

#include <stdlib.h>

struct BuildParams
{
	HtDev		ht;
	int64_t		nrows;
	int		   *flags;
};

__device__ __forceinline__ bool
ht_row_hash(const HtDev &ht, uint32_t row, uint32_t *hash, int64_t *key0)
{
	uint32_t	h = 0;

	for (int k = 0; k < ht.nkeys; k++)
	{
		if (ht.keynulls[k] && ht.keynulls[k][row])
			return false;
		int64_t		v = cb_load_widen(ht.keydata[k], ht.keytype[k], row);

		if (k == 0)
			*key0 = v;
		h = pg_hash_combine(h, jh_hash_datum(ht.keytype[k], v, ht.keydict[k]), false);
	}
	*hash = h;
	return true;
}

__device__ __forceinline__ bool
ht_keys_equal_rows(const HtDev &ht, uint32_t ra, uint32_t rb)
{
	for (int k = 0; k < ht.nkeys; k++)
		if (cb_load_widen(ht.keydata[k], ht.keytype[k], ra) != cb_load_widen(ht.keydata[k], ht.keytype[k], rb))
			return false;
	return true;
}

__global__ void
k_ht_clear(unsigned long long *slots, size_t n)
{
	size_t		i = (size_t) blockIdx.x * blockDim.x + threadIdx.x;
	size_t		stride = (size_t) gridDim.x * blockDim.x;

	for (; i < n; i += stride)
		slots[i] = HT_EMPTY;
}

__global__ void __launch_bounds__(256)
k_ht_build(BuildParams p)
{
	const int64_t stride = (int64_t) gridDim.x * blockDim.x;
	int			inserted = 0;
	bool		dup = false;
	bool		outside = false;

	for (int64_t i = (int64_t) blockIdx.x * blockDim.x + threadIdx.x; i < p.nrows; i += stride)
	{
		uint32_t	h = 0, w;
		int64_t		key0 = 0;
		bool		v = ht_row_hash(p.ht, (uint32_t) i, &h, &key0);

		if (v && !ht_in_batch(p.ht.nbatch, p.ht.batch_shift, p.ht.batch_id, h))
			v = false;
		if (v && p.ht.keyslot && !ht_key_in_domain(p.ht.keyslot, key0))
		{
			outside = true;
			v = false;
		}
		const unsigned long long e = ((unsigned long long) (p.ht.keyslot ? (uint32_t) key0 : h) << 32) | (uint32_t) i;
		uint32_t	pos = h & p.ht.mask;
		const uint32_t bits = ht_bloom_bits(h, &w, p.ht.bloom_mask);

		if (p.ht.bloom)
		{
			const uint32_t word = v ? p.ht.bloom[w] : 0xFFFFFFFFu;

			if ((word & bits) != bits)
				atomicOr(p.ht.bloom + w, bits);
		}
		if (!v)
			continue;
		unsigned long long cur = p.ht.slots[pos];

		for (;;)
		{
			unsigned long long c = cur;

			if (c == HT_EMPTY)
			{
				c = atomicCAS(p.ht.slots + pos, HT_EMPTY, e);
				if (c == HT_EMPTY)
					break;
			}
			if (!dup && (uint32_t) (c >> 32) == (uint32_t) (e >> 32) &&
				(p.ht.keyslot || ht_keys_equal_rows(p.ht, (uint32_t) c, (uint32_t) e)))
				dup = true;
			pos = (pos + 1) & p.ht.mask;
			cur = p.ht.slots[pos];
		}
		inserted++;
	}
	if (dup)
		atomicExch(p.flags, 1);
	if (outside)
		atomicExch(p.flags + 2, 1);
	for (int o = 16; o; o >>= 1)
		inserted += __shfl_xor_sync(0xffffffffu, inserted, o);
	if ((threadIdx.x & 31) == 0 && inserted)
		atomicAdd(p.flags + 1, inserted);
}

static int
ht_fill(cbgpu_hashtable *ht, int batch)
{
	cbgpu_ctx  *ctx = ht->ctx;
	cbgpu_rel  *inner = ht->inner;
	BuildParams p;
	int			h_flags[3];

	ht->d.batch_id = batch;
	if (ht->d.bloom)
		CB_CUDA(ctx, cudaMemsetAsync(ht->d.bloom, 0, ((size_t) ht->d.bloom_mask + 1) * sizeof(uint32_t), ctx->stream));
	for (;;)
	{
		int			blocks = (int) ((ht->nslots + 255) / 256);

		CB_CUDA(ctx, cudaMemsetAsync(ht->d_flags, 0, 3 * sizeof(int), ctx->stream));
		if (blocks > ctx->sm_count * 8)
			blocks = ctx->sm_count * 8;
		k_ht_clear<<<blocks, 256, 0, ctx->stream>>>(ht->d.slots, (size_t) ht->nslots);
		CB_LAUNCHED(ctx, "k_ht_clear");
		p.ht = ht->d;
		p.nrows = inner->nrows;
		p.flags = ht->d_flags;
		if (inner->nrows > 0)
		{
			blocks = (int) ((inner->nrows + 255) / 256);
			if (blocks > ctx->sm_count * 8)
				blocks = ctx->sm_count * 8;
			k_ht_build<<<blocks, 256, 0, ctx->stream>>>(p);
			CB_LAUNCHED(ctx, "k_ht_build");
		}
		CB_CUDA(ctx, cudaMemcpyAsync(h_flags, ht->d_flags, sizeof(h_flags), cudaMemcpyDeviceToHost, ctx->stream));
		CB_CUDA(ctx, cudaStreamSynchronize(ctx->stream));
		if (h_flags[2] && ht->d.keyslot)
		{
			ht->d.keyslot = 0;
			if (ht->d.bloom)
				CB_CUDA(ctx, cudaMemsetAsync(ht->d.bloom, 0, ((size_t) ht->d.bloom_mask + 1) * sizeof(uint32_t), ctx->stream));
			continue;
		}
		break;
	}
	if (h_flags[0])
		ht->has_dups = 1;
	ht->ninserted = h_flags[1];
	return CBGPU_OK;
}

__global__ void
k_ht_batch_histogram(HtDev ht, int64_t nrows, unsigned long long *hist)
{
	for (int64_t i = (int64_t) blockIdx.x * blockDim.x + threadIdx.x; i < nrows; i += (int64_t) gridDim.x * blockDim.x)
	{
		uint32_t	h;
		int64_t		key0;

		if (ht_row_hash(ht, (uint32_t) i, &h, &key0))
			atomicAdd(hist + (h >> ht.batch_shift), 1ull);
	}
}

static int
ht_create(cbgpu_ctx *ctx, cbgpu_rel *inner, const int32_t *keycols, int32_t nkeys, int32_t nbatch, cbgpu_hashtable **out)
{
	cbgpu_hashtable *ht;
	int64_t		nslots = 64;
	int64_t		resident_rows = inner->nrows;

	*out = NULL;
	if (nkeys < 1 || nkeys > CBP_MAX_KEYS)
		return cb_fail(ctx, CBGPU_ERR_UNSUPPORTED, "hash join with %s%lld key columns is beyond the GPU path's limit (4)", "", nkeys);
	if (nbatch < 1 || nbatch > 4096 || (nbatch & (nbatch - 1)) != 0)
		return cb_fail(ctx, CBGPU_ERR_INVALID, "hash join with %s%lld batches (a power of two up to 4096 is expected)", "", nbatch);
	ht = (cbgpu_hashtable *) calloc(1, sizeof(cbgpu_hashtable));
	if (!ht)
		return CBGPU_ERR_NOMEM;
	ht->ctx = ctx;
	ht->inner = inner;
	ht->total_rows = inner->nrows;
	ht->d.nkeys = nkeys;
	ht->d.nbatch = nbatch;
	ht->d.batch_shift = 32;
	for (int b = nbatch; b > 1; b >>= 1)
		ht->d.batch_shift--;
	for (int k = 0; k < nkeys; k++)
	{
		int			c = keycols[k];

		if (c < 0 || c >= inner->ncols)
		{
			free(ht);
			return cb_fail(ctx, CBGPU_ERR_INVALID, "cbgpu_ht_build: bad key column%s %lld", "", c);
		}
		if (inner->types[c] == CB_NUMERIC)
		{
			free(ht);
			return cb_fail(ctx, CBGPU_ERR_UNSUPPORTED, "numeric hash join keys (hash_numeric) are not on the GPU path%s", "", 0);
		}
		if ((inner->types[c] == CB_DICT8 || inner->types[c] == CB_DICT32) && !inner->dict_hash[c])
		{
			free(ht);
			return cb_fail(ctx, CBGPU_ERR_INVALID, "dictionary column %s%lld used as a join key without dict hashes", "", c);
		}
		ht->d.keydata[k] = inner->data[c];
		ht->d.keynulls[k] = inner->nulls[c];
		ht->d.keydict[k] = inner->dict_hash[c];
		ht->d.keytype[k] = inner->types[c];
	}
	CB_CUDA(ctx, cudaSetDevice(ctx->device));
	if (nbatch > 1 && inner->nrows > 0)
	{
		unsigned long long *d_hist,
				   *h_hist = (unsigned long long *) calloc((size_t) nbatch, sizeof(unsigned long long));
		int			blocks = (int) ((inner->nrows + 255) / 256);

		if (!h_hist)
		{
			free(ht);
			return CBGPU_ERR_NOMEM;
		}
		if (blocks > ctx->sm_count * 8)
			blocks = ctx->sm_count * 8;
		CB_CUDA(ctx, cudaMallocAsync(&d_hist, sizeof(unsigned long long) * (size_t) nbatch, ctx->stream));
		CB_CUDA(ctx, cudaMemsetAsync(d_hist, 0, sizeof(unsigned long long) * (size_t) nbatch, ctx->stream));
		k_ht_batch_histogram<<<blocks, 256, 0, ctx->stream>>>(ht->d, inner->nrows, d_hist);
		CB_LAUNCHED(ctx, "k_ht_batch_histogram");
		CB_CUDA(ctx, cudaMemcpyAsync(h_hist, d_hist, sizeof(unsigned long long) * (size_t) nbatch, cudaMemcpyDeviceToHost, ctx->stream));
		CB_CUDA(ctx, cudaStreamSynchronize(ctx->stream));
		CB_CUDA(ctx, cudaFreeAsync(d_hist, ctx->stream));
		resident_rows = 0;
		for (int b = 0; b < nbatch; b++)
			if ((int64_t) h_hist[b] > resident_rows)
				resident_rows = (int64_t) h_hist[b];
		free(h_hist);
	}
	while (nslots < resident_rows * 2)
		nslots <<= 1;
	if (nslots > (1ll << 32))
	{
		free(ht);
		return cb_fail(ctx, CBGPU_ERR_UNSUPPORTED, "hash join build side too large for 32-bit slots%s (%lld rows)", "", inner->nrows);
	}
	ht->nslots = nslots;
	ht->d.mask = (uint32_t) (nslots - 1);
	CB_CUDA(ctx, cudaMallocAsync(&ht->d.slots, (size_t) nslots * sizeof(unsigned long long), ctx->stream));
	CB_CUDA(ctx, cudaMallocAsync(&ht->d_flags, 3 * sizeof(int), ctx->stream));
	if (nkeys == 1)
		switch (ht->d.keytype[0])
		{
			case CB_INT8:
				ht->d.keyslot = 2;
				break;
			case CB_INT4: case CB_DATE: case CB_DICT8: case CB_DICT32: case CB_BPCHAR1: case CB_BOOL:
				ht->d.keyslot = 1;
				break;
			default:
				break;
		}
	{
		int64_t		words = 32;
		const int	div = ctx->opt_bloom_div;

		while (words < resident_rows / div)
			words <<= 1;
		CB_CUDA(ctx, cudaMallocAsync(&ht->d.bloom, (size_t) words * sizeof(uint32_t), ctx->stream));
		ht->d.bloom_mask = (uint32_t) (words - 1);
		ht->built_bytes = nslots * 8 + words * 4;
	}
	*out = ht;
	return CBGPU_OK;
}

extern "C" int
cbgpu_ht_build(cbgpu_ctx *ctx, cbgpu_rel *inner, const int32_t *keycols, int32_t nkeys, cbgpu_hashtable **out)
{
	int			rc = ht_create(ctx, inner, keycols, nkeys, 1, out);

	if (rc == CBGPU_OK)
		rc = ht_fill(*out, 0);
	if (rc != CBGPU_OK && *out)
	{
		cbgpu_ht_free(*out);
		*out = NULL;
	}
	return rc;
}

extern "C" int64_t
cbgpu_ht_bytes_for(int64_t rows)
{
	int64_t		nslots = 64,
				words = 32;

	while (nslots < rows * 2)
		nslots <<= 1;
	while (words < rows / 2)
		words <<= 1;
	return nslots * 8 + words * 4;
}

extern "C" int
cbgpu_ht_build_batched(cbgpu_ctx *ctx, cbgpu_rel *inner, const int32_t *keycols, int32_t nkeys, int32_t nbatch, cbgpu_hashtable **out)
{
	int			rc = ht_create(ctx, inner, keycols, nkeys, nbatch, out);

	for (int b = 0; b < nbatch && rc == CBGPU_OK; b++)
		rc = ht_fill(*out, b);
	if (rc == CBGPU_OK && (*out)->d.keyslot == 0 && nbatch > 1)
		rc = ht_fill(*out, nbatch - 1);
	if (rc != CBGPU_OK && *out)
	{
		cbgpu_ht_free(*out);
		*out = NULL;
	}
	return rc;
}

extern "C" int
cbgpu_ht_nbatch(const cbgpu_hashtable *ht)
{
	return ht->d.nbatch > 1 ? ht->d.nbatch : 1;
}

extern "C" int
cbgpu_ht_load_batch(cbgpu_hashtable *ht, int32_t batch)
{
	if (batch < 0 || batch >= cbgpu_ht_nbatch(ht))
		return cb_fail(ht->ctx, CBGPU_ERR_INVALID, "hash join batch %s%lld out of range", "", batch);
	if (ht->d.nbatch > 1 && ht->d.batch_id == batch)
		return CBGPU_OK;
	return ht_fill(ht, batch);
}

extern "C" void
cbgpu_ht_free(cbgpu_hashtable *ht)
{
	if (!ht)
		return;
	cudaSetDevice(ht->ctx->device);
	cudaFreeAsync(ht->d.slots, ht->ctx->stream);
	if (ht->d.bloom)
		cudaFreeAsync(ht->d.bloom, ht->ctx->stream);
	cudaFreeAsync(ht->d_flags, ht->ctx->stream);
	free(ht);
}

extern "C" int64_t
cbgpu_ht_nrows(const cbgpu_hashtable *ht)
{
	return ht->d.nbatch > 1 ? ht->total_rows : ht->ninserted;
}

extern "C" int
cbgpu_ht_has_duplicates(const cbgpu_hashtable *ht)
{
	return ht->has_dups;
}

extern "C" const uint32_t *
cbgpu_ht_key_dict_hash(const cbgpu_hashtable *ht, int32_t k)
{
	return (k >= 0 && k < ht->d.nkeys) ? ht->d.keydict[k] : NULL;
}

struct JoinFilterDev
{
	const CbpColumn *cols;
	const CbpOp *ops;
	int32_t		nops;
	int32_t		jointype;
	uint32_t   *decision;
	int		   *status;
};

struct ProbeParams
{
	HtDev		ht;
	const void *okey[CBP_MAX_KEYS];
	const uint8_t *onulls[CBP_MAX_KEYS];
	const uint32_t *odict[CBP_MAX_KEYS];
	int32_t		otype[CBP_MAX_KEYS];
	const uint32_t *sel;
	int64_t		n;
	int32_t		left;
	uint8_t    *matched;
	int64_t		ninner;
	unsigned long long *counts;
	uint32_t   *out_outer;
	uint32_t   *out_inner;
	JoinFilterDev f;
};

__device__ __forceinline__ int32_t
ht_probe_row_batch(const ProbeParams &p, uint32_t row, int64_t *key, uint32_t *hash, bool *keynull)
{
	uint32_t	h = 0;
	bool		isnull = false;

	for (int k = 0; k < p.ht.nkeys; k++)
	{
		if (p.onulls[k] && p.onulls[k][row])
			isnull = true;
		key[k] = cb_load_widen(p.okey[k], p.otype[k], row);
		h = pg_hash_combine(h, jh_hash_datum(p.otype[k], key[k], p.odict[k]), false);
	}
	*hash = h;
	*keynull = isnull;
	return (p.ht.nbatch <= 1 || isnull) ? 0 : (int32_t) (h >> p.ht.batch_shift);
}

__device__ __forceinline__ bool
ht_probe_admits(const ProbeParams &p, uint32_t row, int64_t *key, uint32_t *h, bool *mine)
{
	bool		isnull;

	*mine = ht_probe_row_batch(p, row, key, h, &isnull) == p.ht.batch_id || p.ht.nbatch <= 1;
	if (!isnull && p.ht.bloom)
	{
		uint32_t	w;
		uint32_t	bits = ht_bloom_bits(*h, &w, p.ht.bloom_mask);

		if ((__ldg(p.ht.bloom + w) & bits) != bits)
			isnull = true;
	}
	if (!isnull && p.ht.keyslot && !ht_key_in_domain(p.ht.keyslot, key[0]))
		isnull = true;
	if (!isnull && !*mine)
		isnull = true;
	return !isnull;
}

__device__ __forceinline__ bool
ht_slot_key_equal(const ProbeParams &p, unsigned long long e, uint32_t h, const int64_t *key)
{
	if ((uint32_t) (e >> 32) != (p.ht.keyslot ? (uint32_t) key[0] : h))
		return false;
	for (int k = 0; k < p.ht.nkeys && !p.ht.keyslot; k++)
		if (cb_load_widen(p.ht.keydata[k], p.ht.keytype[k], (uint32_t) e) != key[k])
			return false;
	return true;
}

template <bool WRITE>
__global__ void __launch_bounds__(256)
k_ht_probe_pairs(ProbeParams p)
{
	int64_t		i = (int64_t) blockIdx.x * blockDim.x + threadIdx.x;
	int64_t		stride = (int64_t) gridDim.x * blockDim.x;

	for (; i < p.n; i += stride)
	{
		uint32_t	row = p.sel ? p.sel[i] : (uint32_t) i;
		uint32_t	h;
		int64_t		key[CBP_MAX_KEYS];
		bool		mine;
		unsigned long long cnt = 0;
		unsigned long long base = WRITE ? p.counts[i] : 0;

		if (ht_probe_admits(p, row, key, &h, &mine))
		{
			uint32_t	pos = h & p.ht.mask;

			for (;;)
			{
				unsigned long long e = p.ht.slots[pos];

				if (e == HT_EMPTY)
					break;
				if (ht_slot_key_equal(p, e, h, key))
				{
					if (WRITE)
					{
						p.out_outer[base + cnt] = row;
						p.out_inner[base + cnt] = (uint32_t) e;
					}
					else if (p.matched)
						p.matched[(uint32_t) e] = 1;
					cnt++;
				}
				pos = (pos + 1) & p.ht.mask;
			}
		}
		if (p.left && cnt == 0 && mine)
		{
			if (WRITE)
			{
				p.out_outer[base] = row;
				p.out_inner[base] = 0xFFFFFFFFu;
			}
			cnt = 1;
		}
		if (!WRITE)
			p.counts[i] = cnt;
	}
}

__device__ __forceinline__ bool
join_filter_passes(const JoinFilterDev &f, uint32_t orow, uint32_t irow)
{
	int64_t		st[CBP_STACK];
	uint64_t	snull = 0;
	int			sp = 0;

	for (int pc = 0; pc < f.nops; pc++)
	{
		const CbpOp op = f.ops[pc];

		if (op.code == CBP_LOAD)
		{
			const CbpColumn &c = f.cols[op.a];
			const uint32_t r = c.src ? irow : orow;
			const bool	isnull = c.nulls && c.nulls[r];

			st[sp] = isnull ? 0 : cb_load_widen(c.data, c.type, r);
			snull = isnull ? (snull | (1ull << sp)) : (snull & ~(1ull << sp));
			sp++;
		}
		else
			cbp_scalar_op(op, st, snull, sp, true, f.status);
	}
	return !(snull & 1) && st[0] != 0;
}

template <bool WRITE>
__global__ void __launch_bounds__(256)
k_ht_probe_filtered(ProbeParams p)
{
	int64_t		i = (int64_t) blockIdx.x * blockDim.x + threadIdx.x;
	int64_t		stride = (int64_t) gridDim.x * blockDim.x;
	const bool	left = p.f.jointype == CB_JOIN_LEFT;

	for (; i < p.n; i += stride)
	{
		const uint32_t row = p.sel ? p.sel[i] : (uint32_t) i;

		if (WRITE && !left)
		{
			const unsigned long long at = p.counts[i];

			if (p.counts[i + 1] != at)
			{
				p.out_outer[at] = row;
				p.out_inner[at] = p.f.decision[i];
			}
			continue;
		}
		uint32_t	h;
		int64_t		key[CBP_MAX_KEYS];
		bool		mine;
		unsigned long long cnt = 0;
		const unsigned long long base = WRITE ? p.counts[i] : 0;
		uint32_t	first = 0xFFFFFFFFu;

		if (ht_probe_admits(p, row, key, &h, &mine))
		{
			uint32_t	pos = h & p.ht.mask;

			for (;;)
			{
				unsigned long long e = p.ht.slots[pos];

				if (e == HT_EMPTY)
					break;
				if (ht_slot_key_equal(p, e, h, key) && join_filter_passes(p.f, row, (uint32_t) e))
				{
					if (!left)
					{
						first = (uint32_t) e;
						break;
					}
					if (WRITE)
					{
						p.out_outer[base + cnt] = row;
						p.out_inner[base + cnt] = (uint32_t) e;
					}
					cnt++;
				}
				pos = (pos + 1) & p.ht.mask;
			}
		}
		if (!left)
		{
			p.f.decision[i] = first;
			p.counts[i] = p.f.jointype == CB_JOIN_SEMI ? first != 0xFFFFFFFFu : (first == 0xFFFFFFFFu && mine);
			continue;
		}
		if (cnt == 0 && mine)
		{
			if (WRITE)
			{
				p.out_outer[base] = row;
				p.out_inner[base] = 0xFFFFFFFFu;
			}
			cnt = 1;
		}
		if (!WRITE)
			p.counts[i] = cnt;
	}
}

__global__ void
k_exclusive_scan_u64(unsigned long long *a, int64_t n)
{
	__shared__ unsigned long long carry;
	__shared__ unsigned long long warp_tot[32];

	if (threadIdx.x == 0)
		carry = 0;
	__syncthreads();
	for (int64_t base = 0; base < n; base += blockDim.x)
	{
		int64_t		i = base + threadIdx.x;
		unsigned long long v = i < n ? a[i] : 0;
		unsigned long long x = v;
		int			lane = threadIdx.x & 31,
					w = threadIdx.x >> 5;

		for (int o = 1; o < 32; o <<= 1)
		{
			unsigned long long y = __shfl_up_sync(0xffffffffu, x, o);

			if (lane >= o)
				x += y;
		}
		if (lane == 31)
			warp_tot[w] = x;
		__syncthreads();
		if (w == 0)
		{
			unsigned long long t = lane < (int) (blockDim.x >> 5) ? warp_tot[lane] : 0;

			for (int o = 1; o < 32; o <<= 1)
			{
				unsigned long long y = __shfl_up_sync(0xffffffffu, t, o);

				if (lane >= o)
					t += y;
			}
			warp_tot[lane] = t;
		}
		__syncthreads();
		unsigned long long prev = (w ? warp_tot[w - 1] : 0) + carry;

		if (i < n)
			a[i] = prev + x - v;
		__syncthreads();
// ... 579 lines not shown
```

### cloudberry_b200/csrc/probe_chain.cu

```cuda
#include "pipeline.cuh"
#include "xmatch.h"

#include <stdio.h>
#include <stdlib.h>

#define PC_THREADS 256
#define PC_TILE 2048
#define PC_BATCH 1024
#define PC_OCC 4
#define PC_U (PC_BATCH / PC_THREADS)
#define PC_Q0CAP (PC_BATCH + PC_TILE)
#define PC_QCAP (2 * PC_BATCH)
#define PC_MAXP 4
#define PC_MAXOUT 8
#define PC_NQ (2 * PC_MAXP + 1)

struct PcCol
{
	const void *data;
	const uint32_t *dict;
	int32_t		type;
	int32_t		src;
};

struct PcFilter
{
	const void *col;
	int32_t		width;
	int32_t		lo;
	uint32_t	span;
};

struct PcProbe
{
	HtDev		ht;
	int32_t		nkeys;
	int32_t		jointype;
	int32_t		kind;
	PcCol		key[2];
	int32_t		keytype[2];
	int32_t		mode;
	int32_t		smem_off;
};

#define PC_MAXEARLY 2
struct PcEarly
{
	const void *col;
	int32_t		width;
	int32_t		hashtype;
	const uint32_t *bloom;
	uint32_t	mask;
};

struct PcParams
{
	int64_t		nrows;
	const uint32_t *sel;
	const uint8_t *visimap;
	int32_t		nfilters;
	int32_t		np;
	PcFilter	filt[2];
	PcProbe		probe[PC_MAXP];
	int32_t		nearly;
	PcEarly		early[PC_MAXEARLY];
	uint32_t   *qmem;
	int64_t		q_cta_words;
	int32_t		q_off[PC_NQ];
	int32_t		q_cap[PC_NQ];
	int32_t		fuse0;
	uint32_t	smem_table_bytes;
	int32_t		sink_kind;
	AggDev		agg;
	int32_t		nkeys;
	PcCol		key[CBP_MAX_KEYS];
	int32_t		naccs;
	int32_t		acc_term[CBP_MAX_AGGS];
	int32_t		nterms;
	int32_t		term_kind[2];
	PcCol		term_a[2], term_b[2];
	long long	term_k[2];
	int32_t		nout;
	PcCol		out[PC_MAXOUT];
	void	   *outcol[PC_MAXOUT];
	int32_t		outtype[PC_MAXOUT];
	unsigned long long *out_count;
	int64_t		out_capacity;
	int32_t		nhash;
	int32_t		hashtype[CBP_MAX_KEYS];
	const uint32_t *hashdict[CBP_MAX_KEYS];
	int32_t		nsegs;
	int64_t		seg_capacity;
	void *const *part_cols;
	unsigned long long *const *part_counts;
	int32_t    *part_flags;
	int64_t		seg_base[64];
	int64_t		seg_cap[64];
	int		   *status;
};

struct PcPart
{
	unsigned	count[64];
	unsigned long long base[64];
	uint8_t		seg[PC_BATCH];
	uint16_t	rank[PC_BATCH];
};

struct PcQ
{
	const uint32_t *q;
	uint32_t	cap;
	uint32_t	iota_base;
	const uint32_t *sel;
};

__device__ __forceinline__ uint32_t
pc_row(const PcQ &Q, int src, uint32_t e)
{
	return Q.q ? Q.q[(size_t) src * Q.cap + e] : (Q.sel ? Q.sel[Q.iota_base + e] : Q.iota_base + e);
}

__device__ __forceinline__ int64_t
pc_load(const PcCol &c, const PcQ &Q, uint32_t e)
{
	return cb_load_widen(c.data, c.type, pc_row(Q, c.src, e));
}

__device__ __forceinline__ uint32_t
pc_reserve(unsigned *cnt, bool alive)
{
	const unsigned m = __ballot_sync(0xffffffffu, alive);
	const int	lane = threadIdx.x & 31;
	unsigned	base = 0;

	if (m == 0)
		return 0;
	if (lane == (__ffs(m) - 1))
		base = atomicAdd(cnt, (unsigned) __popc(m));
	base = __shfl_sync(0xffffffffu, base, __ffs(m) - 1);
	return base + __popc(m & ((1u << lane) - 1));
}

template <int KIND>
__device__ __forceinline__ uint32_t
pc_key_hash(const PcProbe &pr, int64_t k0, int64_t k1)
{
	if (KIND == 0)
		return pg_hash_combine(0u, jh_mix32((uint32_t) (int32_t) k0), false);
	if (KIND == 1)
		return pg_hash_combine(0u, jh_int8(k0), false);
	uint32_t	h = pg_hash_combine(0u, jh_hash_datum(pr.keytype[0], k0, pr.key[0].dict), false);

	if (pr.nkeys > 1)
		h = pg_hash_combine(h, jh_hash_datum(pr.keytype[1], k1, pr.key[1].dict), false);
	return h;
}

template <int KIND>
__device__ __forceinline__ int64_t
pc_load_key0(const PcProbe &pr, uint32_t row, uint64_t pol_stream)
{
	if (KIND == 0)
		return pr.key[0].src == 0 ? (int64_t) ldg_stream_s32((const int32_t *) pr.key[0].data + row, pol_stream)
			: (int64_t) __ldg((const int32_t *) pr.key[0].data + row);
	if (KIND == 1)
		return pr.key[0].src == 0 ? ldg_stream_s64((const long long *) pr.key[0].data + row, pol_stream)
			: __ldg((const long long *) pr.key[0].data + row);
	return cb_load_widen(pr.key[0].data, pr.key[0].type, row);
}

template <int KIND>
__device__ __noinline__ void
pc_stage_bloom(const PcProbe &pr, int j, PcQ Q, unsigned base, unsigned n, uint32_t *out, unsigned ocap, unsigned *ocnt)
{
	const bool	use_bloom = pr.ht.bloom != NULL && pr.jointype != CB_JOIN_ANTI;
	const uint64_t pol_stream = l2_policy_evict_first();
	const uint64_t pol_keep = l2_policy_evict_last();
	const int	lane = threadIdx.x & 31;
	uint32_t	e[PC_U], h[PC_U], w[PC_U], bits[PC_U], word[PC_U], bal[PC_U];
	int64_t		k0[PC_U], k1[PC_U];
	bool		v[PC_U];

#pragma unroll
	for (int u = 0; u < PC_U; u++)
	{
		const unsigned i = u * PC_THREADS + threadIdx.x;
		uint32_t	r0;

		v[u] = i < n;
		e[u] = base + (v[u] ? i : 0u);
		r0 = pc_row(Q, pr.key[0].src, e[u]);
		k0[u] = pc_load_key0<KIND>(pr, r0, pol_stream);
		k1[u] = (KIND == 2 && pr.nkeys > 1) ? pc_load(pr.key[1], Q, e[u]) : 0;
	}
#pragma unroll
	for (int u = 0; u < PC_U; u++)
	{
		h[u] = pc_key_hash<KIND>(pr, k0[u], k1[u]);
		bits[u] = ht_bloom_bits(h[u], &w[u], pr.ht.bloom_mask);
	}
	if (use_bloom)
	{
#pragma unroll
		for (int u = 0; u < PC_U; u++)
			word[u] = ldg_hint_u32(pr.ht.bloom + w[u], pol_keep);
	}
	unsigned	tot = 0,
				wb = 0;

#pragma unroll
	for (int u = 0; u < PC_U; u++)
	{
		const bool	pass = v[u] && (!use_bloom || (word[u] & bits[u]) == bits[u]);

		bal[u] = __ballot_sync(0xffffffffu, pass);
		tot += __popc(bal[u]);
	}
	if (tot == 0)
		return;
	if (lane == 0)
		wb = atomicAdd(ocnt, tot);
	wb = __shfl_sync(0xffffffffu, wb, 0);
#pragma unroll
	for (int u = 0; u < PC_U; u++)
	{
		if ((bal[u] >> lane) & 1)
		{
			const uint32_t pos = wb + __popc(bal[u] & ((1u << lane) - 1));

			for (int s = 0; s <= j; s++)
				out[(size_t) s * ocap + pos] = pc_row(Q, s, e[u]);
			out[(size_t) (j + 1) * ocap + pos] = h[u];
		}
		wb += __popc(bal[u]);
	}
}

template <int KIND>
__device__ __noinline__ void
pc_stage_ht(const PcProbe &pr, int j, PcQ Q, unsigned base, unsigned n, uint32_t *out, unsigned ocap, unsigned *ocnt)
{
	const uint64_t pol_stream = l2_policy_evict_first();
	const int	lane = threadIdx.x & 31;
	uint32_t	e[PC_U], h[PC_U], pos[PC_U], irow[PC_U], bal[PC_U];
	unsigned long long slot[PC_U];
	bool		v[PC_U];

#pragma unroll
	for (int u = 0; u < PC_U; u++)
	{
		const unsigned i = u * PC_THREADS + threadIdx.x;

		v[u] = i < n;
		e[u] = base + (v[u] ? i : 0u);
		h[u] = Q.q[(size_t) (j + 1) * Q.cap + e[u]];
		pos[u] = h[u] & pr.ht.mask;
	}
#pragma unroll
	for (int u = 0; u < PC_U; u++)
		slot[u] = v[u] ? __ldg(pr.ht.slots + pos[u]) : HT_EMPTY;
	unsigned	tot = 0,
				wb = 0;

#pragma unroll
	for (int u = 0; u < PC_U; u++)
	{
		bool		found = false;

		irow[u] = 0;
		if (slot[u] != HT_EMPTY)
		{
			const int64_t k0 = pc_load_key0<KIND>(pr, pc_row(Q, pr.key[0].src, e[u]), pol_stream);
			const int64_t k1 = (KIND == 2 && pr.nkeys > 1) ? pc_load(pr.key[1], Q, e[u]) : 0;
			unsigned long long x = slot[u];
			uint32_t	p = pos[u];

			if (pr.ht.keyslot)
			{
				const uint32_t tag = (uint32_t) k0;

				if (ht_key_in_domain(pr.ht.keyslot, k0))
					while (x != HT_EMPTY)
					{
						if ((uint32_t) (x >> 32) == tag)
						{
							found = true;
							irow[u] = (uint32_t) x;
							break;
						}
						p = (p + 1) & pr.ht.mask;
						x = __ldg(pr.ht.slots + p);
					}
			}
			else
				while (x != HT_EMPTY)
				{
					if ((uint32_t) (x >> 32) == h[u])
					{
						const uint32_t r = (uint32_t) x;

						if (cb_load_widen(pr.ht.keydata[0], pr.ht.keytype[0], r) == k0 &&
							(KIND != 2 || pr.nkeys < 2 || cb_load_widen(pr.ht.keydata[1], pr.ht.keytype[1], r) == k1))
						{
							found = true;
							irow[u] = r;
							break;
						}
					}
					p = (p + 1) & pr.ht.mask;
					x = __ldg(pr.ht.slots + p);
				}
		}
		bal[u] = __ballot_sync(0xffffffffu, v[u] && (pr.jointype == CB_JOIN_ANTI ? !found : found));
		tot += __popc(bal[u]);
	}
	if (tot == 0)
		return;
	if (lane == 0)
		wb = atomicAdd(ocnt, tot);
	wb = __shfl_sync(0xffffffffu, wb, 0);
#pragma unroll
	for (int u = 0; u < PC_U; u++)
	{
		if ((bal[u] >> lane) & 1)
		{
			const uint32_t opos = wb + __popc(bal[u] & ((1u << lane) - 1));

			for (int s = 0; s <= j; s++)
				out[(size_t) s * ocap + opos] = pc_row(Q, s, e[u]);
			out[(size_t) (j + 1) * ocap + opos] = irow[u];
		}
		wb += __popc(bal[u]);
	}
}

template <int KIND>
__device__ __noinline__ void
pc_stage_direct(const PcProbe &pr, int j, PcQ Q, unsigned base, unsigned n, uint32_t *out, unsigned ocap, unsigned *ocnt, const unsigned long long *slots)
{
	const uint64_t pol_stream = l2_policy_evict_first();
	const int	lane = threadIdx.x & 31;
	uint32_t	e[PC_U], h[PC_U], pos[PC_U], irow[PC_U], bal[PC_U];
	int64_t		k0[PC_U], k1[PC_U];
	unsigned long long slot[PC_U];
	bool		v[PC_U];

#pragma unroll
	for (int u = 0; u < PC_U; u++)
	{
		const unsigned i = u * PC_THREADS + threadIdx.x;

		v[u] = i < n;
		e[u] = base + (v[u] ? i : 0u);
		k0[u] = pc_load_key0<KIND>(pr, pc_row(Q, pr.key[0].src, e[u]), pol_stream);
// ... 73 lines not shown
				out[(size_t) s * ocap + opos] = pc_row(Q, s, e[u]);
			out[(size_t) (j + 1) * ocap + opos] = irow[u];
		}
		wb += __popc(bal[u]);
	}
}

__device__ __noinline__ void
pc_stage_sink(const PcParams &P, PcQ Q, unsigned base, unsigned n, unsigned long long *s_obase, PcPart *part)
{
	if (P.sink_kind == CBP_SINK_AGG)
	{
		for (unsigned b = 0; b < n; b += PC_THREADS)
		{
			const unsigned i = b + threadIdx.x;

			if (i < n)
			{
				const uint32_t e = base + i;
				int64_t		kv[CBP_MAX_KEYS];
				uint32_t	h = 0;

				for (int k = 0; k < P.nkeys; k++)
				{
					kv[k] = pc_load(P.key[k], Q, e);
					h = pg_hash_combine(h, pg_hash_datum(P.key[k].type, kv[k], P.key[k].dict), false);
				}
				h = pg_murmurhash32(h);
				int64_t		tv[2] = {0, 0};

				for (int t = 0; t < P.nterms; t++)
				{
					int64_t		a = pc_load(P.term_a[t], Q, e);

					if (P.term_kind[t] == 1)
					{
						int64_t		bb = pc_load(P.term_b[t], Q, e);
						int64_t		k = P.term_k[t];
						int64_t		d = (int64_t) ((uint64_t) k - (uint64_t) bb);
						int64_t		r = (int64_t) ((uint64_t) a * (uint64_t) d);

						if ((((k ^ bb) & (k ^ d)) < 0) || (__mul64hi(a, d) != (r >> 63)))
							atomicExch(P.status, CBGPU_ERR_OVERFLOW);
						tv[t] = r;
					}
					else if (P.term_kind[t] >= 2)
					{
						const int64_t bb = pc_load(P.term_b[t], Q, e);
						const int64_t r = P.term_kind[t] == 2 ? (int64_t) ((uint64_t) a - (uint64_t) bb) : (int64_t) ((uint64_t) a + (uint64_t) bb);

						if (P.term_kind[t] == 2 ? (((a ^ bb) & (a ^ r)) < 0) : ((~(a ^ bb) & (a ^ r)) < 0))
							atomicExch(P.status, CBGPU_ERR_OVERFLOW);
						tv[t] = r;
					}
					else
						tv[t] = a;
				}
				int			slot = agg_find_or_insert(P.agg, h, kv, 0);

				if (slot >= 0)
					for (int a = 0; a < P.naccs; a++)
					{
						atomicAdd((unsigned long long *) (P.agg.n + (size_t) slot * P.agg.naccs + a), 1ull);
						if (P.acc_term[a] >= 0)
							atomic_add128_signed(P.agg.sum + ((size_t) slot * P.agg.naccs + a) * 2, tv[P.acc_term[a]]);
					}
			}
			__syncwarp();
		}
	}
	else if (P.sink_kind == CBP_SINK_PARTITION)
	{
		if (threadIdx.x < 64)
			part->count[threadIdx.x] = 0;
		__syncthreads();
		for (unsigned i = threadIdx.x; i < n; i += PC_THREADS)
		{
			uint32_t	h = 0;

			for (int k = 0; k < P.nhash; k++)
				h = pg_hash_combine(h, pg_hash_datum(P.hashtype[k], pc_load(P.out[k], Q, base + i), P.hashdict[k]), false);
			const int	seg = pg_jump_consistent_hash(h, P.nsegs);

			part->seg[i] = (uint8_t) seg;
			part->rank[i] = (uint16_t) atomicAdd(&part->count[seg], 1u);
		}
		__syncthreads();
		if (threadIdx.x < P.nsegs && part->count[threadIdx.x])
		{
			unsigned long long b = atomicAdd(P.out_count + threadIdx.x, (unsigned long long) part->count[threadIdx.x]);

			if (P.part_cols)
				b = atomicAdd_system(P.part_counts[threadIdx.x], (unsigned long long) part->count[threadIdx.x]);
			part->base[threadIdx.x] = b;
			if ((int64_t) (b + part->count[threadIdx.x]) > P.seg_cap[threadIdx.x])
			{
				if (P.part_flags)
					atomicOr(P.part_flags, CBGPU_DX_OVERFLOW);
				else
					atomicExch(P.status, CBGPU_ERR_NOMEM);
			}
		}
		__syncthreads();
		for (unsigned i = threadIdx.x; i < n; i += PC_THREADS)
		{
			const int	seg = part->seg[i];
			const unsigned long long pos = part->base[seg] + part->rank[i];

			if ((int64_t) pos < P.seg_cap[seg])
			{
				const uint64_t dst = P.part_cols ? pos : (uint64_t) P.seg_base[seg] + pos;

				for (int c = 0; c < P.nout; c++)
					sink_store(P.part_cols ? P.part_cols[seg * P.nout + c] : P.outcol[c], P.outtype[c], dst, pc_load(P.out[c], Q, base + i));
			}
		}
	}
	else
	{
		if (threadIdx.x == 0)
			*s_obase = atomicAdd(P.out_count, (unsigned long long) n);
		__syncthreads();
		const unsigned long long ob = *s_obase;

		if ((int64_t) (ob + n) > P.out_capacity)
		{
			if (threadIdx.x == 0)
				atomicExch(P.status, CBGPU_ERR_NOMEM);
		}
		else
			for (unsigned i = threadIdx.x; i < n; i += PC_THREADS)
				for (int c = 0; c < P.nout; c++)
					sink_store(P.outcol[c], P.outtype[c], ob + i, pc_load(P.out[c], Q, base + i));
	}
}

__device__ __forceinline__ int32_t
pc_filter_value(const PcFilter &f, int64_t row)
{
	return f.width == 4 ? __ldg((const int32_t *) f.col + row) : (int32_t) __ldg((const uint8_t *) f.col + row);
}

__device__ __forceinline__ void
pc_unpack8(unsigned long long v, int4 *a, int4 *b)
{
	const unsigned lo = (unsigned) v,
				hi = (unsigned) (v >> 32);

	*a = make_int4((int) (lo & 0xff), (int) ((lo >> 8) & 0xff), (int) ((lo >> 16) & 0xff), (int) (lo >> 24));
	*b = make_int4((int) (hi & 0xff), (int) ((hi >> 8) & 0xff), (int) ((hi >> 16) & 0xff), (int) (hi >> 24));
}

__device__ __forceinline__ unsigned
pc_range8(int4 a, int4 b, int32_t lo, uint32_t span)
{
	return ((unsigned) ((unsigned) (a.x - lo) <= span) << 0) | ((unsigned) ((unsigned) (a.y - lo) <= span) << 1) |
		((unsigned) ((unsigned) (a.z - lo) <= span) << 2) | ((unsigned) ((unsigned) (a.w - lo) <= span) << 3) |
		((unsigned) ((unsigned) (b.x - lo) <= span) << 4) | ((unsigned) ((unsigned) (b.y - lo) <= span) << 5) |
		((unsigned) ((unsigned) (b.z - lo) <= span) << 6) | ((unsigned) ((unsigned) (b.w - lo) <= span) << 7);
}

struct PcKeys8
{
	int4		q[4];
};

template <bool WIDE>
__device__ __forceinline__ PcKeys8
pc_keys8_vec(const void *col, int64_t row0, uint64_t pol)
{
	PcKeys8		k;

	if (WIDE)
	{
		const int4 *p = (const int4 *) ((const long long *) col + row0);

#pragma unroll
		for (int i = 0; i < 4; i++)
			k.q[i] = ldg_stream_v4(p + i, pol);
	}
	else
	{
		const int4 *p = (const int4 *) ((const int32_t *) col + row0);

		k.q[0] = ldg_stream_v4(p, pol);
		k.q[1] = ldg_stream_v4(p + 1, pol);
		k.q[2] = k.q[3] = make_int4(0, 0, 0, 0);
	}
	return k;
}

template <bool WIDE>
__device__ __forceinline__ PcKeys8
pc_keys8_pred(const void *col, int64_t row0, unsigned am, uint64_t pol)
{
	PcKeys8		k;
	int			v[8];

	if (WIDE)
	{
		long long	t[8];

#pragma unroll
		for (int u = 0; u < 8; u++)
			t[u] = ((am >> u) & 1) ? ldg_stream_s64((const long long *) col + row0 + u, pol) : 0;
#pragma unroll
		for (int i = 0; i < 4; i++)
			k.q[i] = make_int4((int) (unsigned) t[2 * i], (int) (unsigned) ((unsigned long long) t[2 * i] >> 32), (int) (unsigned) t[2 * i + 1],
							   (int) (unsigned) ((unsigned long long) t[2 * i + 1] >> 32));
	}
	else
	{
#pragma unroll
		for (int u = 0; u < 8; u++)
			v[u] = ((am >> u) & 1) ? ldg_stream_s32((const int32_t *) col + row0 + u, pol) : 0;
		k.q[0] = make_int4(v[0], v[1], v[2], v[3]);
		k.q[1] = make_int4(v[4], v[5], v[6], v[7]);
		k.q[2] = k.q[3] = make_int4(0, 0, 0, 0);
	}
	return k;
}

template <bool WIDE>
__device__ __forceinline__ int64_t
pc_keys8_get(const PcKeys8 &k, int u)
{
	if (WIDE)
	{
		const int4	t = k.q[u >> 1];
		const unsigned lo = (u & 1) ? (unsigned) t.z : (unsigned) t.x;
		const unsigned hi = (u & 1) ? (unsigned) t.w : (unsigned) t.y;

		return (int64_t) (((unsigned long long) hi << 32) | lo);
	}
	const int4	t = k.q[u >> 2];

	return (int64_t) ((u & 3) == 0 ? t.x : (u & 3) == 1 ? t.y : (u & 3) == 2 ? t.z : t.w);
}

__device__ __forceinline__ bool
pc_warp_dense(bool full, unsigned am, unsigned at_least = 64u)
{
	return __all_sync(0xffffffffu, full) && __reduce_add_sync(0xffffffffu, (unsigned) __popc(am)) >= at_least;
}

template <bool WIDE>
__device__ __forceinline__ void
pc_stage_f_probe0(const PcProbe &pr, int64_t row0, const PcKeys8 &keys, unsigned am, uint32_t *out, unsigned cap, unsigned *ocnt)
{
	const bool	use_bloom = pr.ht.bloom != NULL && pr.jointype != CB_JOIN_ANTI;
	const uint64_t pol_keep = l2_policy_evict_last();
	const int	lane = threadIdx.x & 31;
	uint32_t	h[8];

#pragma unroll
	for (int u = 0; u < 8; u++)
		h[u] = WIDE ? jh_int8(pc_keys8_get<true>(keys, u)) : jh_mix32((uint32_t) (int32_t) pc_keys8_get<false>(keys, u));
	if (use_bloom)
	{
		uint32_t	bits[8], word[8];

#pragma unroll
		for (int u = 0; u < 8; u++)
		{
			uint32_t	w;

			bits[u] = ht_bloom_bits(h[u], &w, pr.ht.bloom_mask);
			word[u] = ((am >> u) & 1) ? ldg_hint_u32(pr.ht.bloom + w, pol_keep) : 0u;
		}
#pragma unroll
		for (int u = 0; u < 8; u++)
			if ((word[u] & bits[u]) != bits[u])
				am &= ~(1u << u);
	}
	const unsigned c = __popc(am);
	unsigned	x = c;

#pragma unroll
	for (int d = 1; d < 32; d <<= 1)
	{
		const unsigned y = __shfl_up_sync(0xffffffffu, x, d);

		if (lane >= d)
			x += y;
	}
	const unsigned total = __shfl_sync(0xffffffffu, x, 31);
	unsigned	wb = 0;

	if (lane == 31 && total)
		wb = atomicAdd(ocnt, total);
	wb = __shfl_sync(0xffffffffu, wb, 31);
	unsigned	pos = wb + x - c;

#pragma unroll
	for (int u = 0; u < 8; u++)
		if ((am >> u) & 1)
		{
			out[pos] = (uint32_t) (row0 + u);
			out[(size_t) cap + pos] = h[u];
			pos++;
		}
}

template <bool WIDE>
__device__ __forceinline__ unsigned
pc_early_filter8(const PcEarly &E, int64_t row0, bool full, unsigned am, uint64_t pol)
{
	const PcKeys8 keys = pc_warp_dense(full, am) ? pc_keys8_vec<WIDE>(E.col, row0, pol) : pc_keys8_pred<WIDE>(E.col, row0, am, pol);
	uint32_t	bits[8], word[8];

#pragma unroll
	for (int u = 0; u < 8; u++)
	{
		const int64_t kv = pc_keys8_get<WIDE>(keys, u);
		uint32_t	w;

		bits[u] = ht_bloom_bits(pg_hash_combine(0u, WIDE ? jh_int8(kv) : jh_mix32((uint32_t) (int32_t) kv), false), &w, E.mask);
		word[u] = ((am >> u) & 1) ? __ldg(E.bloom + w) : 0u;
	}
#pragma unroll
	for (int u = 0; u < 8; u++)
		if ((word[u] & bits[u]) != bits[u])
			am &= ~(1u << u);
	return am;
}

template <bool WIDE>
__device__ __forceinline__ unsigned
pc_bloom8_keys(const PcEarly &E, const PcKeys8 &keys, unsigned am)
{
	uint32_t	bits[8], word[8];

#pragma unroll
	for (int u = 0; u < 8; u++)
	{
		const int64_t kv = pc_keys8_get<WIDE>(keys, u);
		uint32_t	w;

		bits[u] = ht_bloom_bits(pg_hash_combine(0u, WIDE ? jh_int8(kv) : jh_mix32((uint32_t) (int32_t) kv), false), &w, E.mask);
		word[u] = ((am >> u) & 1) ? __ldg(E.bloom + w) : 0u;
	}
#pragma unroll
	for (int u = 0; u < 8; u++)
		if ((word[u] & bits[u]) != bits[u])
			am &= ~(1u << u);
	return am;
}

#define PF_MAXBLOOM 6
struct PfParams
{
	int64_t		nrows;
	const uint8_t *visimap;
	int32_t		nfilters;
	PcFilter	filt[2];
	int32_t		nbloom;
	PcEarly		bloom[PF_MAXBLOOM];
	uint32_t   *out;
	unsigned long long *out_count;
};

template <bool SPEC>
__global__ void __launch_bounds__(PC_THREADS, SPEC ? 4 : 8)
k_prefilter(const __grid_constant__ PfParams P)
{
	__shared__ uint32_t buf[PC_TILE];
	__shared__ unsigned s_cnt;
	__shared__ unsigned long long s_gbase;
	const int64_t ntiles = (P.nrows + PC_TILE - 1) / PC_TILE;
	const unsigned o0 = threadIdx.x * 8;
	const int	lane = threadIdx.x & 31;
	const uint64_t pol_stream = l2_policy_evict_first();

	for (int64_t tile = blockIdx.x; tile < ntiles; tile += gridDim.x)
	{
		const int64_t base = tile * PC_TILE;
		const unsigned nvalid = (unsigned) (P.nrows - base < PC_TILE ? P.nrows - base : PC_TILE);
		const bool	full = o0 + 8 <= nvalid;
		unsigned	am = 0;

		PcKeys8		keys0;
		bool		have0 = false;

		if (threadIdx.x == 0)
			s_cnt = 0;
		if (SPEC && P.nbloom > 0 && __all_sync(0xffffffffu, full))
		{
			keys0 = P.bloom[0].width == 8 ? pc_keys8_vec<true>(P.bloom[0].col, base + o0, pol_stream)
				: pc_keys8_vec<false>(P.bloom[0].col, base + o0, pol_stream);
			have0 = true;
		}
		if (full)
		{
			int4		a0 = make_int4(0, 0, 0, 0), b0 = a0, a1 = a0, b1 = a0;
			unsigned	vm = 0xff;

			if (P.nfilters > 0)
			{
				if (P.filt[0].width == 4)
				{
					a0 = ldg_stream_v4((const int4 *) ((const int32_t *) P.filt[0].col + base + o0), pol_stream);
					b0 = ldg_stream_v4((const int4 *) ((const int32_t *) P.filt[0].col + base + o0) + 1, pol_stream);
				}
				else
					pc_unpack8(ldg_stream_u64((const unsigned long long *) ((const uint8_t *) P.filt[0].col + base + o0), pol_stream), &a0, &b0);
			}
			if (P.nfilters > 1)
			{
				if (P.filt[1].width == 4)
				{
					a1 = ldg_stream_v4((const int4 *) ((const int32_t *) P.filt[1].col + base + o0), pol_stream);
					b1 = ldg_stream_v4((const int4 *) ((const int32_t *) P.filt[1].col + base + o0) + 1, pol_stream);
				}
				else
					pc_unpack8(ldg_stream_u64((const unsigned long long *) ((const uint8_t *) P.filt[1].col + base + o0), pol_stream), &a1, &b1);
			}
			if (P.visimap)
				vm = __ldg(P.visimap + ((base + o0) >> 3));
			am = vm;
			if (P.nfilters > 0)
				am &= pc_range8(a0, b0, P.filt[0].lo, P.filt[0].span);
			if (P.nfilters > 1)
				am &= pc_range8(a1, b1, P.filt[1].lo, P.filt[1].span);
		}
		else
			for (int u = 0; u < 8; u++)
			{
				const int64_t r = base + o0 + u;
				bool		alive = o0 + u < nvalid;

				if (alive && P.visimap)
					alive = (__ldg(P.visimap + (r >> 3)) >> (r & 7)) & 1;
				if (alive && P.nfilters > 0)
					alive = (unsigned) (pc_filter_value(P.filt[0], r) - P.filt[0].lo) <= P.filt[0].span;
				if (alive && P.nfilters > 1)
					alive = (unsigned) (pc_filter_value(P.filt[1], r) - P.filt[1].lo) <= P.filt[1].span;
				am |= (unsigned) alive << u;
			}
		for (int f = 0; f < P.nbloom && __any_sync(0xffffffffu, am != 0); f++)
		{
			if (SPEC && f == 0 && have0)
				am = P.bloom[0].width == 8 ? pc_bloom8_keys<true>(P.bloom[0], keys0, am) : pc_bloom8_keys<false>(P.bloom[0], keys0, am);
			else
				am = P.bloom[f].width == 8 ? pc_early_filter8<true>(P.bloom[f], base + o0, full, am, pol_stream)
					: pc_early_filter8<false>(P.bloom[f], base + o0, full, am, pol_stream);
		}
		__syncthreads();
		{
			const unsigned c = __popc(am);
			unsigned	x = c;

#pragma unroll
			for (int d = 1; d < 32; d <<= 1)
			{
				const unsigned y = __shfl_up_sync(0xffffffffu, x, d);

				if (lane >= d)
					x += y;
			}
			const unsigned total = __shfl_sync(0xffffffffu, x, 31);
			unsigned	wb = 0;

			if (lane == 31 && total)
				wb = atomicAdd(&s_cnt, total);
			wb = __shfl_sync(0xffffffffu, wb, 31);
			unsigned	pos = wb + x - c;

#pragma unroll
			for (int u = 0; u < 8; u++)
				if ((am >> u) & 1)
					buf[pos++] = (uint32_t) (base + o0 + u);
		}
		__syncthreads();
		if (threadIdx.x == 0 && s_cnt)
			s_gbase = atomicAdd(P.out_count, (unsigned long long) s_cnt);
		__syncthreads();
		for (unsigned i = threadIdx.x; i < s_cnt; i += PC_THREADS)
			P.out[s_gbase + i] = buf[i];
		__syncthreads();
	}
}

__global__ void __launch_bounds__(PC_THREADS, PC_OCC)
k_probe_chain(const __grid_constant__ PcParams P)
{
	__shared__ uint32_t q0[PC_Q0CAP];
	__shared__ PcProbe sprobe[PC_MAXP];
	__shared__ unsigned cnt[PC_NQ];
	__shared__ int s_stage;
	__shared__ unsigned s_n, s_base;
	__shared__ long long s_tile;
	__shared__ unsigned long long s_obase;
	__shared__ PcPart part;
	__shared__ uint64_t s_tbar;
	extern __shared__ __align__(16) unsigned long long s_tables[];
	const int	np = P.np;
	const int	last = 2 * np + 1;
	const bool	iota = P.nfilters == 0 && P.visimap == NULL && P.nearly == 0;
	const int64_t tile_rows = iota ? PC_BATCH : PC_TILE;
	const int64_t ntiles = (P.nrows + tile_rows - 1) / tile_rows;
	uint32_t   *const qg = P.qmem + (size_t) blockIdx.x * (size_t) P.q_cta_words;
	int64_t		next_tile = blockIdx.x;

	if (threadIdx.x < PC_NQ)
		cnt[threadIdx.x] = 0;
	for (int i = threadIdx.x; i < (int) (np * sizeof(PcProbe) / sizeof(uint32_t)); i += PC_THREADS)
		((uint32_t *) sprobe)[i] = ((const uint32_t *) P.probe)[i];
	if (P.smem_table_bytes)
	{
		if (threadIdx.x == 0)
		{
			mbar_init(&s_tbar, 1);
			asm volatile("fence.mbarrier_init.release.cluster;" ::: "memory");
		}
		__syncthreads();
		if (threadIdx.x == 0)
		{
			mbar_expect_tx(&s_tbar, P.smem_table_bytes);
			for (int j = 0; j < np; j++)
				if (P.probe[j].mode == 2)
					tma_load_1d(s_tables + P.probe[j].smem_off, P.probe[j].ht.slots, (P.probe[j].ht.mask + 1u) * 8u, &s_tbar);
		}
		mbar_wait(&s_tbar, 0);
	}
	for (;;)
	{
		__syncthreads();
		if (threadIdx.x == 0)
		{
			int			s = -1;
			bool		from_tile = false;

			for (int k = last; k >= 1; k--)
				if (cnt[k - 1] >= PC_BATCH)
				{
					s = k;
					break;
				}
			if (s < 0)
			{
				if (next_tile < ntiles)
				{
					s = iota ? 1 : 0;
					from_tile = true;
					s_tile = next_tile;
					next_tile += gridDim.x;
				}
				else
					for (int k = 1; k <= last; k++)
						if (cnt[k - 1] > 0)
						{
							s = k;
							break;
						}
			}
			if (s >= 1 && !from_tile)
			{
				const unsigned c = cnt[s - 1];
				const unsigned n = c < PC_BATCH ? c : PC_BATCH;

				s_n = n;
				s_base = c - n;
				cnt[s - 1] = c - n;
			}
			s_stage = from_tile ? -2 - s : s;
		}
		__syncthreads();
		const int	code = s_stage;

		if (code == -1)
			break;
		if (code == -2)
		{
			const int64_t base = s_tile * PC_TILE;
			const unsigned nvalid = (unsigned) (P.nrows - base < PC_TILE ? P.nrows - base : PC_TILE);
			const unsigned o0 = threadIdx.x * 8;
			const int	lane = threadIdx.x & 31;
			const uint64_t pol_stream = l2_policy_evict_first();
			const bool	full = o0 + 8 <= nvalid;
			const bool	wide0 = sprobe[0].kind == 1;
			unsigned	am = 0;

			if (full)
			{
				int4		a0 = make_int4(0, 0, 0, 0), b0 = a0, a1 = a0, b1 = a0;
				unsigned	vm = 0xff;

				if (P.nfilters > 0)
				{
					if (P.filt[0].width == 4)
					{
						a0 = ldg_stream_v4((const int4 *) ((const int32_t *) P.filt[0].col + base + o0), pol_stream);
						b0 = ldg_stream_v4((const int4 *) ((const int32_t *) P.filt[0].col + base + o0) + 1, pol_stream);
					}
					else
						pc_unpack8(ldg_stream_u64((const unsigned long long *) ((const uint8_t *) P.filt[0].col + base + o0), pol_stream), &a0, &b0);
				}
				if (P.nfilters > 1)
				{
					if (P.filt[1].width == 4)
					{
						a1 = ldg_stream_v4((const int4 *) ((const int32_t *) P.filt[1].col + base + o0), pol_stream);
						b1 = ldg_stream_v4((const int4 *) ((const int32_t *) P.filt[1].col + base + o0) + 1, pol_stream);
					}
					else
						pc_unpack8(ldg_stream_u64((const unsigned long long *) ((const uint8_t *) P.filt[1].col + base + o0), pol_stream), &a1, &b1);
				}
				if (P.visimap)
					vm = __ldg(P.visimap + ((base + o0) >> 3));
				am = vm;
				if (P.nfilters > 0)
					am &= pc_range8(a0, b0, P.filt[0].lo, P.filt[0].span);
				if (P.nfilters > 1)
					am &= pc_range8(a1, b1, P.filt[1].lo, P.filt[1].span);
			}
			else
				for (int u = 0; u < 8; u++)
				{
					const int64_t r = base + o0 + u;
					bool		alive = o0 + u < nvalid;

					if (alive && P.visimap)
						alive = (__ldg(P.visimap + (r >> 3)) >> (r & 7)) & 1;
					if (alive && P.nfilters > 0)
						alive = (unsigned) (pc_filter_value(P.filt[0], r) - P.filt[0].lo) <= P.filt[0].span;
					if (alive && P.nfilters > 1)
						alive = (unsigned) (pc_filter_value(P.filt[1], r) - P.filt[1].lo) <= P.filt[1].span;
					am |= (unsigned) alive << u;
				}
			for (int f = 0; f < P.nearly && __any_sync(0xffffffffu, am != 0); f++)
				am = P.early[f].width == 8 ? pc_early_filter8<true>(P.early[f], base + o0, full, am, pol_stream)
					: pc_early_filter8<false>(P.early[f], base + o0, full, am, pol_stream);
			if (P.fuse0 && pc_warp_dense(full, am, 96u))
			{
				if (wide0)
					pc_stage_f_probe0<true>(sprobe[0], base + o0, pc_keys8_vec<true>(sprobe[0].key[0].data, base + o0, pol_stream), am,
											qg + P.q_off[1], (unsigned) P.q_cap[1], &cnt[1]);
				else
					pc_stage_f_probe0<false>(sprobe[0], base + o0, pc_keys8_vec<false>(sprobe[0].key[0].data, base + o0, pol_stream), am,
											 qg + P.q_off[1], (unsigned) P.q_cap[1], &cnt[1]);
				continue;
			}
			const unsigned c = __popc(am);
			unsigned	x = c;

#pragma unroll
			for (int d = 1; d < 32; d <<= 1)
			{
				const unsigned y = __shfl_up_sync(0xffffffffu, x, d);

				if (lane >= d)
					x += y;
			}
			const unsigned total = __shfl_sync(0xffffffffu, x, 31);
			unsigned	wb = 0;

			if (lane == 31 && total)
				wb = atomicAdd(&cnt[0], total);
			wb = __shfl_sync(0xffffffffu, wb, 31);
			unsigned	pos = wb + x - c;

#pragma unroll
			for (int u = 0; u < 8; u++)
				if ((am >> u) & 1)
					q0[pos++] = (uint32_t) (base + o0 + u);
			continue;
		}
		int			s = code;
		PcQ			Q;
		unsigned	n = s_n,
					base = s_base;

		if (code == -3)
		{
			const int64_t tb = s_tile * PC_BATCH;

			s = 1;
			Q.q = NULL;
			Q.cap = 0;
			Q.iota_base = (uint32_t) tb;
			Q.sel = P.sel;
			n = (unsigned) (P.nrows - tb < PC_BATCH ? P.nrows - tb : PC_BATCH);
			base = 0;
		}
		else if (s == 1)
		{
			Q.q = q0;
			Q.cap = PC_Q0CAP;
			Q.iota_base = 0;
			Q.sel = NULL;
		}
		else
		{
			Q.q = qg + P.q_off[s - 1];
			Q.cap = (uint32_t) P.q_cap[s - 1];
			Q.iota_base = 0;
			Q.sel = NULL;
		}
		if (s == last)
			pc_stage_sink(P, Q, base, n, &s_obase, &part);
		else
		{
			const int	j = (s - 1) >> 1;
			const PcProbe &pr = sprobe[j];
			uint32_t   *out = qg + P.q_off[s];

			if ((s & 1) && pr.mode != 0)
			{
				const unsigned long long *slots = pr.mode == 2 ? s_tables + pr.smem_off : pr.ht.slots;
				uint32_t   *out2 = qg + P.q_off[s + 1];

				if (pr.kind == 0)
					pc_stage_direct<0>(pr, j, Q, base, n, out2, (unsigned) P.q_cap[s + 1], &cnt[s + 1], slots);
				else if (pr.kind == 1)
					pc_stage_direct<1>(pr, j, Q, base, n, out2, (unsigned) P.q_cap[s + 1], &cnt[s + 1], slots);
				else
					pc_stage_direct<2>(pr, j, Q, base, n, out2, (unsigned) P.q_cap[s + 1], &cnt[s + 1], slots);
			}
			else if (s & 1)
			{
				if (pr.kind == 0)
					pc_stage_bloom<0>(pr, j, Q, base, n, out, (unsigned) P.q_cap[s], &cnt[s]);
				else if (pr.kind == 1)
					pc_stage_bloom<1>(pr, j, Q, base, n, out, (unsigned) P.q_cap[s], &cnt[s]);
				else
					pc_stage_bloom<2>(pr, j, Q, base, n, out, (unsigned) P.q_cap[s], &cnt[s]);
			}
			else
			{
				if (pr.kind == 0)
					pc_stage_ht<0>(pr, j, Q, base, n, out, (unsigned) P.q_cap[s], &cnt[s]);
				else if (pr.kind == 1)
					pc_stage_ht<1>(pr, j, Q, base, n, out, (unsigned) P.q_cap[s], &cnt[s]);
				else
					pc_stage_ht<2>(pr, j, Q, base, n, out, (unsigned) P.q_cap[s], &cnt[s]);
			}
		}
	}
}

static bool
pc_col(const CbPipeline *p, int c, PcCol *out, int base)
{
	if (p->cols[c].nulls != NULL || p->cols[c].type == CB_FLOAT8 || p->cols[c].type == CB_NUMERIC128)
		return false;
	out->data = p->cols[c].data;
	out->dict = p->cols[c].dict_hash;
	out->type = p->cols[c].type;
	out->src = p->cols[c].src == 0 ? 0 : p->cols[c].src - base + 1;
	return true;
}

struct PcEarlyBuild
{
	int64_t		nrows;
	HtDev		self;
	int32_t		kc;
	int32_t		hashtype;
	int32_t		nred;
	HtDev		red[PC_MAXP];
	int32_t		red_nkeys[PC_MAXP];
	PcCol		red_key[PC_MAXP][2];
	int32_t		red_keytype[PC_MAXP][2];
	uint32_t   *bloom;
	uint32_t	mask;
	unsigned long long *passed;
};

__global__ void
k_pc_early_build(PcEarlyBuild B)
{
	for (int64_t r = (int64_t) blockIdx.x * blockDim.x + threadIdx.x; r < B.nrows; r += (int64_t) gridDim.x * blockDim.x)
	{
		bool		ok = true;

		for (int k = 0; k < B.self.nkeys; k++)
			if (B.self.keynulls[k] && B.self.keynulls[k][r])
				ok = false;
		for (int m = 0; m < B.nred && ok; m++)
		{
			const HtDev &T = B.red[m];
			int64_t		kv[2] = {0, 0};
			uint32_t	h = 0;
			bool		found = false;

			for (int i = 0; i < B.red_nkeys[m]; i++)
			{
				kv[i] = cb_load_widen(B.red_key[m][i].data, B.red_key[m][i].type, (uint32_t) r);
				h = pg_hash_combine(h, jh_hash_datum(B.red_keytype[m][i], kv[i], B.red_key[m][i].dict), false);
			}
			uint32_t	pos = h & T.mask;

			for (; !(T.keyslot && !ht_key_in_domain(T.keyslot, kv[0]));)
			{
				const unsigned long long e = T.slots[pos];

				if (e == HT_EMPTY)
					break;
				if ((uint32_t) (e >> 32) == (T.keyslot ? (uint32_t) kv[0] : h))
				{
					const uint32_t ir = (uint32_t) e;

					if (T.keyslot || (cb_load_widen(T.keydata[0], T.keytype[0], ir) == kv[0] &&
									  (B.red_nkeys[m] < 2 || cb_load_widen(T.keydata[1], T.keytype[1], ir) == kv[1])))
					{
						found = true;
						break;
					}
				}
				pos = (pos + 1) & T.mask;
			}
			ok = found;
		}
		if (ok && !B.bloom)
			atomicAdd(B.passed, 1ull);
		if (ok && B.bloom)
		{
			uint32_t	w;
			const int64_t kv = cb_load_widen(B.self.keydata[B.kc], B.self.keytype[B.kc], (uint32_t) r);
			const uint32_t bits = ht_bloom_bits(pg_hash_combine(0u, jh_hash_datum(B.hashtype, kv, NULL), false), &w, B.mask);

			atomicOr(B.bloom + w, bits);
		}
	}
}

#define PC_REJECT(n) \
	do { \
		if (ctx->opt_debug) \
			fprintf(stderr, "k_probe_chain: pipeline not matched (reason %d, line %d)\n", n, __LINE__); \
		return CBGPU_OK; \
	} while (0)

int
cb_try_probe_chain(cbgpu_ctx *ctx, const CbPipeline *p, const PipeDev *d, bool *handled)
{
	XProg	   *xp = (XProg *) cb_scratch(ctx, 2, sizeof(XProg));
	PcParams   *Pp = (PcParams *) cb_scratch(ctx, 3, sizeof(PcParams));
	if (!xp || !Pp)
		return CBGPU_ERR_NOMEM;
	XProg	   &x = *xp;
	PcParams   &P = *Pp;
	const CbpSink *s = &p->sink;
	int			np = 0;
	int			base = 1;
	int			term_node[2] = {-1, -1};

	*handled = false;
	if (p->nprobes < 0 || p->nprobes > PC_MAXP || p->drv_nsrc != 0)
		PC_REJECT(1);
	if (s->kind != CBP_SINK_AGG && s->kind != CBP_SINK_MATERIALIZE && s->kind != CBP_SINK_PARTITION)
		PC_REJECT(2);
	if (s->kind == CBP_SINK_PARTITION && s->nsegs > 64)
		PC_REJECT(2);
	if (!xm_decompile(p, &x))
		PC_REJECT(3);
	memset(&P, 0, sizeof(P));
	for (int i = 0; i < x.nsections; i++)
	{
		XSection   *sec = &x.sections[i];

		if (sec->kind == 0)
		{
			int			code, col;
			int64_t		v, lo = INT32_MIN, hi = INT32_MAX;

			if (np > 0)
				PC_REJECT(4);
			if (!xm_is_cmp_const(&x, sec->node, &code, &col, &v) || p->cols[col].src != 0 || p->cols[col].nulls ||
				(cb_type_w(p->cols[col].type) != 4 && cb_type_w(p->cols[col].type) != 1))
				PC_REJECT(5);
			if (cb_type_w(p->cols[col].type) == 1)
			{
				lo = 0;
				hi = 255;
			}
			switch (code)
			{
				case CBP_EQ: lo = hi = v; break;
				case CBP_LT: hi = v - 1; break;
				case CBP_LE: hi = v; break;
				case CBP_GT: lo = v + 1; break;
				case CBP_GE: lo = v; break;
				default: PC_REJECT(6);
			}
			if (lo > INT32_MAX || hi < INT32_MIN || lo > hi)
				PC_REJECT(7);
			if (hi > INT32_MAX)
				hi = INT32_MAX;
			if (lo < INT32_MIN)
				lo = INT32_MIN;
			if (((uintptr_t) p->cols[col].data & 15) != 0)
				PC_REJECT(100);
			{
				int			f = P.nfilters;

				for (int g = 0; g < P.nfilters; g++)
					if (P.filt[g].col == p->cols[col].data)
					{
						const int64_t olo = P.filt[g].lo,
									ohi = olo + (int64_t) P.filt[g].span;

						lo = lo > olo ? lo : olo;
						hi = hi < ohi ? hi : ohi;
						f = g;
					}
				if (lo > hi)
					PC_REJECT(7);
				if (f == P.nfilters && P.nfilters >= 2)
					PC_REJECT(4);
				P.filt[f].col = p->cols[col].data;
				P.filt[f].width = cb_type_w(p->cols[col].type);
				P.filt[f].lo = (int32_t) lo;
				P.filt[f].span = (uint32_t) (hi - lo);
				if (f == P.nfilters)
					P.nfilters++;
			}
		}
		else
		{
			const CbpProbe *pp = &p->probes[sec->probe];
			PcProbe    *q = &P.probe[np];

			if (sec->probe != np || pp->nkeys > 2)
				PC_REJECT(8);
			if (pp->jointype != CB_JOIN_INNER && pp->jointype != CB_JOIN_SEMI && pp->jointype != CB_JOIN_ANTI)
				PC_REJECT(9);
			if ((pp->jointype != CB_JOIN_INNER) && np != p->nprobes - 1)
				PC_REJECT(10);
			q->ht = d->probes[np].ht;
			q->nkeys = pp->nkeys;
			q->jointype = pp->jointype;
			if (!q->ht.bloom)
				PC_REJECT(11);
			for (int k = 0; k < pp->nkeys; k++)
			{
				int			col;

				if (!xm_is_load(&x, sec->keys[k], &col) || !pc_col(p, col, &q->key[k], base))
					PC_REJECT(12);
				if (q->key[k].src > np)
					PC_REJECT(13);
				q->keytype[k] = pp->keytype[k];
				q->key[k].type = p->cols[col].type;
				if (q->ht.keynulls[k])
					PC_REJECT(14);
			}
			if (pp->nkeys == 1 && (q->key[0].type == CB_INT4 || q->key[0].type == CB_DATE) &&
				(q->keytype[0] == CB_INT4 || q->keytype[0] == CB_DATE))
				q->kind = 0;
			else if (pp->nkeys == 1 && q->key[0].type == CB_INT8 && q->keytype[0] == CB_INT8)
				q->kind = 1;
			else
				q->kind = 2;
			np++;
		}
	}
	if (np != p->nprobes)
		PC_REJECT(15);
	P.np = np;
	P.nrows = p->nrows;
	P.visimap = p->visimap;
	P.status = ctx->d_status;
	P.sink_kind = s->kind;
	if (s->kind == CBP_SINK_AGG)
	{
		if (x.depth < s->nkeys)
			PC_REJECT(16);
		P.agg = d->sink.agg;
		P.nkeys = s->nkeys;
		for (int k = 0; k < s->nkeys; k++)
		{
			int			col;

			if (!xm_is_load(&x, x.stack[k], &col) || !pc_col(p, col, &P.key[k], base))
				PC_REJECT(17);
			P.key[k].type = s->keytype[k];
			P.key[k].dict = s->key_dict_hash[k];
		}
		P.naccs = s->naccs;
		for (int a = 0; a < s->naccs; a++)
		{
			int			node, col, b, c;
			int64_t		k;
			int			t = -1;

			if (s->accs[a].kind == CBP_ACC_COUNT && s->accs[a].arg < 0)
			{
				P.acc_term[a] = -1;
				continue;
			}
			if (s->accs[a].kind != CBP_ACC_SUM_INT)
				PC_REJECT(18);
			node = x.stack[s->nkeys + s->accs[a].arg];
			for (int u = 0; u < P.nterms; u++)
				if (term_node[u] == node)
					t = u;
			if (t >= 0)
			{
				P.acc_term[a] = t;
				continue;
			}
			if (P.nterms >= 2)
				PC_REJECT(19);
			t = P.nterms;
			term_node[t] = node;
			if (xm_is_rev(&x, node, &b, &k, &c))
			{
				P.term_kind[t] = 1;
				P.term_k[t] = k;
				if (!pc_col(p, b, &P.term_a[t], base) || !pc_col(p, c, &P.term_b[t], base))
					PC_REJECT(20);
			}
			else if ((x.nodes[node].code == CBP_SUB || x.nodes[node].code == CBP_ADD) && xm_is_load(&x, x.nodes[node].l, &b) &&
					 xm_is_load(&x, x.nodes[node].r, &c))
			{
				P.term_kind[t] = x.nodes[node].code == CBP_SUB ? 2 : 3;
				if (!pc_col(p, b, &P.term_a[t], base) || !pc_col(p, c, &P.term_b[t], base))
					PC_REJECT(30);
			}
			else if (xm_is_load(&x, node, &col))
			{
				P.term_kind[t] = 0;
				if (!pc_col(p, col, &P.term_a[t], base))
					PC_REJECT(21);
			}
			else
				PC_REJECT(22);
			P.nterms++;
			P.acc_term[a] = t;
		}
	}
	else
	{
		if (s->nout > PC_MAXOUT || x.depth != s->nout)
			PC_REJECT(23);
		P.nout = s->nout;
		for (int c = 0; c < s->nout; c++)
		{
			int			col;

			if (!xm_is_load(&x, x.stack[c], &col) || !pc_col(p, col, &P.out[c], base) || d->sink.outnull[c])
				PC_REJECT(24);
			P.outcol[c] = d->sink.outcol[c];
			P.outtype[c] = d->sink.outtype[c];
		}
		P.out_count = d->sink.out_count;
		P.out_capacity = d->sink.out_capacity;
		if (s->kind == CBP_SINK_PARTITION)
		{
			P.nhash = d->sink.nhash;
			P.nsegs = d->sink.nsegs;
			P.seg_capacity = d->sink.seg_capacity;
			P.part_cols = d->sink.part_cols;
			P.part_counts = d->sink.part_counts;
			P.part_flags = d->sink.part_flags;
			for (int g = 0; g < P.nsegs && g < 64; g++)
			{
				P.seg_base[g] = d->sink.seg_base[g];
				P.seg_cap[g] = d->sink.seg_cap[g];
			}
			for (int k = 0; k < P.nhash; k++)
			{
				P.hashtype[k] = d->sink.hashtype[k];
				P.hashdict[k] = d->sink.hashdict[k];
			}
		}
	}

	void	   *early_mem[PC_MAXEARLY] = {NULL, NULL};

	for (int k = 0; k < np && P.nearly < PC_MAXEARLY; k++)
	{
		PcEarlyBuild *Bp = (PcEarlyBuild *) cb_scratch(ctx, 4, sizeof(PcEarlyBuild));
		if (!Bp)
			return CBGPU_ERR_NOMEM;
		PcEarlyBuild &B = *Bp;
		PcProbe    *q = &P.probe[k];
		const cbgpu_rel *inner = p->probes[k].ht->inner;
		int			kc = -1;
		int64_t		words = 32;

		memset(&B, 0, sizeof(B));
		if (q->jointype != CB_JOIN_INNER || !inner || inner->nrows < 1)
			continue;
		for (int m = k + 1; m < np; m++)
		{
			bool		all = P.probe[m].jointype == CB_JOIN_INNER;

			for (int i = 0; i < P.probe[m].nkeys; i++)
				if (P.probe[m].key[i].src != k + 1)
					all = false;
			if (!all)
				continue;
			B.red[B.nred] = P.probe[m].ht;
			B.red_nkeys[B.nred] = P.probe[m].nkeys;
			for (int i = 0; i < P.probe[m].nkeys; i++)
			{
				B.red_key[B.nred][i] = P.probe[m].key[i];
				B.red_keytype[B.nred][i] = P.probe[m].keytype[i];
			}
			B.nred++;
		}
		if (B.nred == 0)
			continue;
		for (int i = 0; i < q->nkeys && kc < 0; i++)
			if (q->key[i].src == 0 && (q->key[i].type == CB_INT4 || q->key[i].type == CB_DATE || q->key[i].type == CB_INT8))
				kc = i;
		if (kc < 0)
			continue;
		{
			unsigned long long *d_passed,
						h_passed = 0;
			const int64_t sample = inner->nrows < 65536 ? inner->nrows : 65536;
			const void *sig = (const void *) (uintptr_t) ((uintptr_t) B.red[0].mask * 31u + (uintptr_t) B.nred * 7u + (uintptr_t) B.red[0].keytype[0]);
			int			known = -1;

			for (int i = 0; i < ctx->early_cache_n; i++)
				if (ctx->early_cache[i].keydata == q->ht.keydata[kc] && ctx->early_cache[i].nrows == inner->nrows && ctx->early_cache[i].red0 == sig)
					known = ctx->early_cache[i].worth;
			if (known < 0)
			{
				CB_CUDA(ctx, cudaMallocAsync(&d_passed, sizeof(*d_passed), ctx->stream));
				CB_CUDA(ctx, cudaMemsetAsync(d_passed, 0, sizeof(*d_passed), ctx->stream));
				B.nrows = sample;
				B.self = q->ht;
				B.kc = kc;
				B.hashtype = q->keytype[kc];
				B.bloom = NULL;
				B.passed = d_passed;
				k_pc_early_build<<<(int) ((sample + 255) / 256), 256, 0, ctx->stream>>>(B);
				CB_LAUNCHED(ctx, "k_pc_early_build");
				CB_CUDA(ctx, cudaMemcpyAsync(&h_passed, d_passed, sizeof(h_passed), cudaMemcpyDeviceToHost, ctx->stream));
				CB_CUDA(ctx, cudaStreamSynchronize(ctx->stream));
				CB_CUDA(ctx, cudaFreeAsync(d_passed, ctx->stream));
				known = (int64_t) h_passed * 2 <= sample;
				{
					const int	slot = ctx->early_cache_n < CB_EARLY_CACHE ? ctx->early_cache_n++ : (int) (inner->nrows % CB_EARLY_CACHE);

					ctx->early_cache[slot].keydata = q->ht.keydata[kc];
					ctx->early_cache[slot].nrows = inner->nrows;
					ctx->early_cache[slot].red0 = sig;
					ctx->early_cache[slot].worth = known;
				}
			}
			if (!known)
				continue;
		}
		while (words < inner->nrows / 2)
			words <<= 1;
		CB_CUDA(ctx, cudaMallocAsync(&early_mem[P.nearly], (size_t) words * sizeof(uint32_t), ctx->stream));
		CB_CUDA(ctx, cudaMemsetAsync(early_mem[P.nearly], 0, (size_t) words * sizeof(uint32_t), ctx->stream));
		B.nrows = inner->nrows;
		B.self = q->ht;
		B.kc = kc;
		B.hashtype = q->keytype[kc];
		B.bloom = (uint32_t *) early_mem[P.nearly];
		B.mask = (uint32_t) (words - 1);
		{
			int			eb = (int) ((inner->nrows + 255) / 256);

			if (eb > ctx->sm_count * 8)
				eb = ctx->sm_count * 8;
			k_pc_early_build<<<eb, 256, 0, ctx->stream>>>(B);
			CB_LAUNCHED(ctx, "k_pc_early_build");
		}
		P.early[P.nearly].col = q->key[kc].data;
		P.early[P.nearly].width = cb_type_w(q->key[kc].type);
		P.early[P.nearly].hashtype = q->keytype[kc];
		P.early[P.nearly].bloom = B.bloom;
		P.early[P.nearly].mask = B.mask;
		P.nearly++;
	}
	uint32_t   *pf_sel = NULL;
	unsigned long long *pf_count = NULL;
	bool		pf_bloom_done[PC_MAXP] = {false, false, false, false};
	bool		pf_cand[PC_MAXP] = {false, false, false, false};

	if (P.nrows >= ctx->opt_pf_min_rows && np >= 1)
	{
		PfParams   *Fp = (PfParams *) cb_scratch(ctx, 6, sizeof(PfParams));

		if (!Fp)
			return CBGPU_ERR_NOMEM;
		PfParams   &F = *Fp;
		const uint64_t sig = (uint64_t) (uintptr_t) (P.nfilters ? P.filt[0].col : NULL) ^ ((uint64_t) (uintptr_t) P.probe[0].key[0].data << 1) ^
			((uint64_t) P.nrows << 20) ^ (uint64_t) P.nfilters ^ ((uint64_t) np << 4) ^ ((uint64_t) P.nearly << 8);
		bool		known_unselective = false;

		memset(&F, 0, sizeof(F));
		F.nrows = P.nrows;
		F.visimap = P.visimap;
		F.nfilters = P.nfilters;
		F.filt[0] = P.filt[0];
		F.filt[1] = P.filt[1];
		for (int f = 0; f < P.nearly; f++)
			F.bloom[F.nbloom++] = P.early[f];
		for (int j = 0; j < np && F.nbloom < PF_MAXBLOOM; j++)
		{
			const PcProbe &q = P.probe[j];

			if ((q.jointype != CB_JOIN_INNER && q.jointype != CB_JOIN_SEMI) || q.nkeys != 1 || (q.kind != 0 && q.kind != 1) ||
				q.key[0].src != 0 || !q.ht.bloom || ((uintptr_t) q.key[0].data & 15) != 0)
				continue;
			F.bloom[F.nbloom].col = q.key[0].data;
			F.bloom[F.nbloom].width = q.kind == 1 ? 8 : 4;
			F.bloom[F.nbloom].hashtype = q.keytype[0];
			F.bloom[F.nbloom].bloom = q.ht.bloom;
			F.bloom[F.nbloom].mask = q.ht.bloom_mask;
			F.nbloom++;
			pf_cand[j] = true;
		}
		for (int i = 0; i < ctx->pf_cache_n; i++)
			if (ctx->pf_cache[i] == sig)
				known_unselective = true;
		if (F.nbloom + F.nfilters > 0 && !known_unselective)
		{
			unsigned long long nsel = 0;
			const int64_t ft = (P.nrows + PC_TILE - 1) / PC_TILE;

			CB_CUDA(ctx, cudaMallocAsync(&pf_sel, (size_t) P.nrows * sizeof(uint32_t), ctx->stream));
			CB_CUDA(ctx, cudaMallocAsync(&pf_count, sizeof(unsigned long long), ctx->stream));
			CB_CUDA(ctx, cudaMemsetAsync(pf_count, 0, sizeof(unsigned long long), ctx->stream));
			F.out = pf_sel;
			F.out_count = pf_count;
			const int	pkl = cb_klog_begin(ctx, "k_prefilter");

			if (ctx->opt_pf_spec)
				k_prefilter<true><<<ctx->sm_count * 4 < ft ? ctx->sm_count * 4 : (int) ft, PC_THREADS, 0, ctx->stream>>>(F);
			else
				k_prefilter<false><<<ctx->sm_count * 8 < ft ? ctx->sm_count * 8 : (int) ft, PC_THREADS, 0, ctx->stream>>>(F);
			CB_LAUNCHED(ctx, "k_prefilter");
			cb_klog_end(ctx, pkl);
			CB_CUDA(ctx, cudaMemcpyAsync(&nsel, pf_count, sizeof(nsel), cudaMemcpyDeviceToHost, ctx->stream));
			CB_CUDA(ctx, cudaStreamSynchronize(ctx->stream));
			if (ctx->opt_debug)
				fprintf(stderr, "k_prefilter: %lld of %lld rows survive %d qual(s) + %d filter(s)\n", (long long) nsel, (long long) P.nrows, F.nfilters, F.nbloom);
			if (nsel * (unsigned long long) ctx->opt_pf_keep_div <= (unsigned long long) P.nrows)
			{
				P.sel = pf_sel;
				P.nrows = (int64_t) nsel;
				P.nfilters = 0;
				P.visimap = NULL;
				P.nearly = 0;
				for (int j = 0; j < np; j++)
					pf_bloom_done[j] = pf_cand[j];
			}
			else
			{
				if (ctx->pf_cache_n < (int) (sizeof(ctx->pf_cache) / sizeof(ctx->pf_cache[0])))
					ctx->pf_cache[ctx->pf_cache_n++] = sig;
			}
		}
	}
	const bool	iota = P.nfilters == 0 && P.visimap == NULL && P.nearly == 0;
	const int64_t ntiles = (P.nrows + (iota ? PC_BATCH : PC_TILE) - 1) / (iota ? PC_BATCH : PC_TILE);
	int			blocks = ctx->sm_count * PC_OCC;
	int64_t		words = 0;

	if (blocks > ntiles)
		blocks = (int) ntiles;
	if (blocks < 1)
		blocks = 1;
	{
		uint32_t	smem_slots = 0;

		for (int j = 0; j < np; j++)
		{
			const uint64_t bytes = ((uint64_t) P.probe[j].ht.mask + 1) * 8;

			P.probe[j].mode = 0;
			if (bytes <= 32768 && (smem_slots * 8 + bytes) <= 32768 && ((uintptr_t) P.probe[j].ht.slots & 15) == 0)
			{
				P.probe[j].mode = 2;
				P.probe[j].smem_off = (int32_t) smem_slots;
				smem_slots += (uint32_t) (bytes / 8);
			}
			else if (pf_bloom_done[j])
				P.probe[j].mode = 1;
		}
		P.smem_table_bytes = smem_slots * 8;
	}
	P.fuse0 = !iota && np >= 1 && P.probe[0].mode == 0 && P.probe[0].nkeys == 1 && (P.probe[0].kind == 0 || P.probe[0].kind == 1) &&
		P.probe[0].key[0].src == 0 && ((uintptr_t) P.probe[0].key[0].data & 15) == 0;
	for (int k = 1; k <= 2 * np; k++)
	{
		P.q_off[k] = (int32_t) words;
		P.q_cap[k] = (k == 1 && P.fuse0) ? PC_Q0CAP : PC_QCAP;
		words += (int64_t) P.q_cap[k] * ((k + 3) / 2);
	}
	P.q_cta_words = words;
	CB_CUDA(ctx, cudaMallocAsync(&P.qmem, (size_t) blocks * (size_t) (words ? words : 1) * sizeof(uint32_t), ctx->stream));
	if (ctx->opt_debug)
		fprintf(stderr, "k_probe_chain: modes %d %d %d %d (0 filter + HBM table, 1 table only, 2 table in shared memory: %u bytes) fuse0 %d\n",
				P.probe[0].mode, P.probe[1].mode, P.probe[2].mode, P.probe[3].mode, P.smem_table_bytes, P.fuse0);
	if (ctx->opt_debug)
		fprintf(stderr, "k_probe_chain: np %d nrows %lld tiles %lld blocks %d queue words/CTA %lld filters %d sink %d kinds %d %d %d %d\n", np,
				(long long) P.nrows, (long long) ntiles, blocks, (long long) words, P.nfilters, P.sink_kind, P.probe[0].kind,
				P.probe[1].kind, P.probe[2].kind, P.probe[3].kind);
	if (ctx->opt_debug && P.nearly)
		fprintf(stderr, "k_probe_chain: %d scan-level runtime filter(s)\n", P.nearly);
	CB_CUDA(ctx, cudaEventRecord(ctx->ev_k0, ctx->stream));
	int			kl = cb_klog_begin(ctx, "k_probe_chain");

	{
		static bool attr_done = false;

		if (!attr_done)
		{
			CB_CUDA(ctx, cudaFuncSetAttribute(k_probe_chain, cudaFuncAttributeMaxDynamicSharedMemorySize, 32768));
			attr_done = true;
		}
	}
	k_probe_chain<<<blocks, PC_THREADS, P.smem_table_bytes, ctx->stream>>>(P);
	ctx->last_kernel_name = "k_probe_chain";
	if (kl >= 0)
		ctx->klog_name[kl] = ctx->last_kernel_name;
	CB_LAUNCHED(ctx, "k_probe_chain");
	cb_klog_end(ctx, kl);
	CB_CUDA(ctx, cudaEventRecord(ctx->ev_k1, ctx->stream));
	CB_CUDA(ctx, cudaFreeAsync(P.qmem, ctx->stream));
	if (pf_sel)
		CB_CUDA(ctx, cudaFreeAsync(pf_sel, ctx->stream));
	if (pf_count)
		CB_CUDA(ctx, cudaFreeAsync(pf_count, ctx->stream));
	for (int f = 0; f < PC_MAXEARLY; f++)
		if (early_mem[f])
			CB_CUDA(ctx, cudaFreeAsync(early_mem[f], ctx->stream));
	ctx->kernel_timed = true;
	*handled = true;
	return CBGPU_OK;
}
```

### include/cb_exec.h

```cpp
#ifndef CB_EXEC_H
#define CB_EXEC_H

#include "cbgpu.h"

#ifdef __cplusplus
extern "C" {
#endif

struct CbPlanState;
struct CbEState;
struct CbInterconnect;

typedef struct CbNumericDatum
{
	int64_t		lo, hi;
	int32_t		dscale;
	char		text[84];
} CbNumericDatum;

typedef struct CbTupleTableSlot
{
	bool		tts_empty;
	int32_t		tts_nvalid;
	int32_t	   *tts_types;
	int64_t    *tts_values;
	bool	   *tts_isnull;
	int64_t    *tts_state_n;
	int64_t    *tts_state_lo;
	int64_t    *tts_state_hi;
} CbTupleTableSlot;

typedef CbTupleTableSlot *(*CbExecProcNodeMtd) (struct CbPlanState *pstate);

typedef struct CbInstrumentation
{
	double		ntuples;
	double		nloops;
	int64_t		kernels;
	double		device_ms;
	int64_t		rows_in;
	int64_t		motion_repartitions;
	int64_t		hashjoin_nbatch;
	int64_t		agg_npartitions;
} CbInstrumentation;

typedef struct CbPlanState
{
	CbNodeTag	type;
	CbPlan	   *plan;
	struct CbEState *state;
	CbExecProcNodeMtd ExecProcNode;
	CbInstrumentation instrument;
	struct CbPlanState *lefttree;
	struct CbPlanState *righttree;
	CbTupleTableSlot *ps_ResultTupleSlot;
	bool		squelched;
	void	   *priv;
} CbPlanState;

typedef void (*CbErrorHook) (struct CbEState *estate, int code, const char *message);

typedef struct CbEState
{
	cbgpu_ctx  *es_ctx;
	int32_t		es_nrels;
	cbgpu_rel **es_range_table;
	int32_t		es_segindex;
	int32_t		es_numsegments;
	struct CbInterconnect *es_interconnect;
	int32_t		es_errcode;
	char		es_errmsg[512];
	CbErrorHook es_error_hook;
	int32_t		es_force_generic;
	int64_t		es_processed;
	void	   *es_cluster;
	int			(*es_interrupt_pending) (struct CbEState *estate);
	void	   *es_interrupt_arg;
	int64_t		es_operator_mem_kb;
	int64_t		es_hashjoin_batches_run;
	int64_t		es_agg_partitions_run;
} CbEState;

CbEState   *cb_CreateExecutorState(cbgpu_ctx *ctx, cbgpu_rel **range_table, int32_t nrels);
void		cb_FreeExecutorState(CbEState *estate);
const char *cb_estate_error(CbEState *estate);

CbPlanState *cb_ExecInitNode(CbPlan *node, CbEState *estate, int eflags);
CbTupleTableSlot *cb_ExecProcNode(CbPlanState *node);
cbgpu_hashtable *cb_MultiExecProcNode(CbPlanState *node);
int			cb_ExecProcNodeBatch(CbPlanState *node, cbgpu_rel **out);
void		cb_ExecEndNode(CbPlanState *node);
void		cb_ExecReScan(CbPlanState *node);
void		cb_ExecSquelchNode(CbPlanState *node);

#define CbTupIsNull(slot) ((slot) == NULL || (slot)->tts_empty)
int			cb_slot_natts(const CbTupleTableSlot *slot);
int			cb_slot_isnull(const CbTupleTableSlot *slot, int attno);
int64_t		cb_slot_int64(const CbTupleTableSlot *slot, int attno);
double		cb_slot_float8(const CbTupleTableSlot *slot, int attno);
int			cb_slot_text(const CbTupleTableSlot *slot, int attno, char *buf, int buflen);

void		cb_numeric_sum_text(int64_t lo, int64_t hi, int32_t dscale, char *out, int32_t outlen);
void		cb_numeric_avg_text(int64_t lo, int64_t hi, int32_t dscale, int64_t n, char *out, int32_t outlen);
int			cb_numeric_avg_serialize(int64_t n, int64_t sum_lo, int64_t sum_hi, int32_t dscale, uint8_t *out, int32_t cap);
int			cb_int8_avg_serialize(int64_t n, int64_t sum_lo, int64_t sum_hi, uint8_t *out, int32_t cap);
int			cb_numeric_avg_deserialize(const uint8_t *in, int32_t len, int32_t with_tail, int64_t *n, int64_t *sum_lo, int64_t *sum_hi,
									   int32_t *dscale);

typedef struct CbInterconnect
{
	const char *name;
	int32_t		nsegs;
	int32_t		segindex;
	int			(*redistribute) (struct CbInterconnect *ic, struct CbEState *estate, int32_t motion_id,
								 cbgpu_rel *send, const int64_t *counts, const int64_t *offsets, cbgpu_rel **recv);
	int			(*gather) (struct CbInterconnect *ic, struct CbEState *estate, int32_t motion_id, int32_t root,
						   cbgpu_rel *send, int64_t nrows, cbgpu_rel **recv);
	int			(*broadcast) (struct CbInterconnect *ic, struct CbEState *estate, int32_t motion_id,
							  cbgpu_rel *send, int64_t nrows, cbgpu_rel **recv);
	void		(*teardown) (struct CbInterconnect *ic);
	void	   *priv;
	int			(*direct_begin) (struct CbInterconnect *ic, struct CbEState *estate, int32_t motion_id, int32_t ncols,
								 const int32_t *types, const int32_t *dscales, cbgpu_direct_dest *dest);
	int			(*direct_end) (struct CbInterconnect *ic, struct CbEState *estate, int32_t motion_id, int32_t local_flags,
							   uint64_t local_nullmask, const int64_t *dev_sent_counts, int64_t *sent_counts, cbgpu_rel **recv,
							   int32_t *outcome);
	void		(*abandon) (struct CbInterconnect *ic, struct CbEState *estate, int32_t motion_id, int32_t after_direct);
} CbInterconnect;

CbInterconnect *cb_interconnect_nccl_create(cbgpu_motion *motion);
void		cb_interconnect_destroy(CbInterconnect *ic);

typedef struct CbCluster CbCluster;
CbCluster  *cb_cluster_create(cbgpu_ctx *ctx, int32_t nsegs);
int			cb_cluster_set_range_table(CbCluster *c, int32_t seg, cbgpu_rel **range_table, int32_t nrels);
CbEState   *cb_cluster_estate(CbCluster *c, int32_t seg);
int			cb_cluster_init_plan(CbCluster *c, CbPlan *plan);
CbTupleTableSlot *cb_cluster_next(CbCluster *c);
int32_t		cb_cluster_current_segment(CbCluster *c);
void		cb_cluster_end(CbCluster *c);
void		cb_cluster_destroy(CbCluster *c);
const char *cb_cluster_error(CbCluster *c);

int			cb_aocs_segfile_path(const char *basepath, int segno, int filenum, char *out, size_t outsz);

typedef struct CbAocsColumnSpec
{
	int32_t		relcol;
	int32_t		filenum;
	int32_t		attlen;
	int32_t		varkind;
	int32_t		typalign;
	int32_t		compresstype;
	int64_t		eof;
	cbgpu_dict *dict;
} CbAocsColumnSpec;
int			cb_aocs_dict_collect_segfile(cbgpu_ctx *ctx, const char *basepath, int segno, int checksum, const CbAocsColumnSpec *spec,
										 char *err, size_t errsz);
int			cb_aocs_load_segfile(cbgpu_ctx *ctx, const char *basepath, int segno, int checksum, int ncols,
								 const CbAocsColumnSpec *cols, cbgpu_rel *rel, int64_t row_offset,
								 const cbgpu_visimap_entry *entries, int nentries, int64_t *nrows, int64_t *nhidden,
								 char *err, size_t errsz);

#define CB_TUPSER_MAX_ATTS 1600
#define CB_TUPSER_MAX_TEXT 8192
typedef struct CbTupAttr
{
	int32_t		type;
	int32_t		dscale;
	int32_t		bpchar_len;
	int32_t		ntexts;
	const char *const *texts;
	const int32_t *text_lens;
	struct CbAggStateDatum *state;
} CbTupAttr;
typedef struct CbAggStateDatum
{
	int64_t		n,
				lo,
				hi;
} CbAggStateDatum;
#define CB_TUPSER_STATE_NUMERIC 101
#define CB_TUPSER_STATE_INT8 102
int64_t		cb_tupser_row(const CbTupAttr *attrs, int natts, const int64_t *values, const uint8_t *isnull, int max_chunk,
						  unsigned char *out, int64_t outcap);
int			cb_tupser_end_of_stream(unsigned char *out, int64_t outcap);
#define CB_TUPSER_END 0
#define CB_TUPSER_NEED_MORE (-1)
#define CB_TUPSER_BAD (-2)
int64_t		cb_tupser_next(const CbTupAttr *attrs, int natts, const unsigned char *in, int64_t inlen, int64_t *consumed,
						   int64_t *values, uint8_t *isnull);

#ifdef __cplusplus
}
#endif
#endif
```

Baseline: 80.81 billion.

## Add exact key-range bitmap filters for joins and batch result draining

During the hash-table build, the min and max of integer keys are now tracked. When the key span is small enough, the prefilter and the scan-level runtime filters use an exact bitmap instead of a bloom filter, and the prefilter can stage that bitmap in shared memory with 1024-thread blocks. Separately, result rows are drained in C into one text buffer, replacing per-slot Python ctypes calls. TPC-H Q1 has no joins, so only the result-drain change is likely to affect this query, and Q1 returns only a few rows.

```diff
diff --git a/cloudberry_b200/capi.py b/cloudberry_b200/capi.py
--- a/cloudberry_b200/capi.py
+++ b/cloudberry_b200/capi.py
@@ -1,6 +1,7 @@
 import ctypes as C
 import os
 import re
+import struct
 
 import numpy as np
 
@@ -397,6 +398,10 @@
         L.cb_ExecInitNode.argtypes = [C.POINTER(P.CbPlan), C.POINTER(CbEState), C.c_int]
         L.cb_ExecProcNode.restype = C.POINTER(CbTupleTableSlot)
         L.cb_ExecProcNode.argtypes = [C.POINTER(CbPlanState)]
+        L.cb_ExecDrainText.restype = C.c_void_p
+        L.cb_ExecDrainText.argtypes = [C.POINTER(CbPlanState), C.POINTER(C.c_int64)]
+        L.cb_free_text.restype = None
+        L.cb_free_text.argtypes = [C.c_void_p]
         L.cb_MultiExecProcNode.restype = vp
         L.cb_MultiExecProcNode.argtypes = [C.POINTER(CbPlanState)]
         L.cb_ExecProcNodeBatch.restype = C.c_int
@@ -733,6 +738,29 @@
     return row, states
 
 
+_F8 = struct.Struct("<q"), struct.Struct("<d")
+
+
+def _drained_rows(text):
+    rows, states = [], []
+    for line in text.split("\n")[:-1]:
+        row, st = [], []
+        for field in (line.split("\t") if line else []):
+            tag, v, n, lo, hi = field.split(" ")
+            st.append((int(n), (int(hi) << 64) | (int(lo) & 0xFFFFFFFFFFFFFFFF)))
+            if tag == "i":
+                row.append(int(v))
+            elif tag == "s":
+                row.append(v)
+            elif tag == "f":
+                row.append(_F8[1].unpack(_F8[0].pack(int(v)))[0])
+            else:
+                row.append(None)
+        rows.append(row)
+        states.append(st)
+    return rows, states
+
+
 class Result:
     def __init__(self):
         self.rows = []
@@ -782,16 +810,21 @@
             raise CbgpuError(es.contents.es_errcode, E.cb_estate_error(es).decode())
         res = Result()
         try:
-            while True:
-                slot = E.cb_ExecProcNode(ps)
-                if es.contents.es_errcode:
-                    raise CbgpuError(es.contents.es_errcode, E.cb_estate_error(es).decode())
-                if not slot or slot.contents.tts_empty:
-                    break
-                row, st = _slot_row(E, slot)
-                res.rows.append(row)
-                res.states.append(st)
-                res.segments.append(0)
+            n = C.c_int64(0)
+            buf = E.cb_ExecDrainText(ps, C.byref(n))
+            if es.contents.es_errcode:
+                if buf:
+                    E.cb_free_text(buf)
+                raise CbgpuError(es.contents.es_errcode, E.cb_estate_error(es).decode())
+            if not buf:
+                raise MemoryError("cb_ExecDrainText")
+            try:
+                text = C.string_at(buf).decode()
+            finally:
+                E.cb_free_text(buf)
+            res.rows, res.states = _drained_rows(text)
+            assert len(res.rows) == n.value
+            res.segments = [0] * n.value
             _collect_instrument(ps, res.instrument)
         finally:
             E.cb_ExecEndNode(ps)
diff --git a/cloudberry_b200/csrc/common.cuh b/cloudberry_b200/csrc/common.cuh
--- a/cloudberry_b200/csrc/common.cuh
+++ b/cloudberry_b200/csrc/common.cuh
@@ -18,6 +18,7 @@
 	cudaStream_t stream;
 	char		err[512];
 	int			sm_count;
+	int64_t		smem_per_sm;
 	int64_t		launches;
 	cudaEvent_t ev_t0, ev_t1, ev_k0, ev_k1;
 	double		last_kernel_ms;
@@ -223,6 +224,27 @@
 	return keyslot == 1 ? key == (int64_t) (int32_t) key : (uint64_t) key <= 0xFFFFFFFFull;
 }
 
+static inline uint64_t
+ht_exact_nbits(int64_t kmin, int64_t kmax, uint64_t limit)
+{
+	const uint64_t span = (uint64_t) kmax - (uint64_t) kmin;
+
+	return kmin <= kmax && span < limit && span < 0xFFFFFFFFull ? span + 1 : 0;
+}
+
+CB_HD_DECL bool
+ht_exact_type(int32_t type)
+{
+	return type == CB_INT4 || type == CB_DATE || type == CB_INT8;
+}
+
+struct HtFillOut
+{
+	int			flags[4];
+	unsigned long long kmin_inv;
+	unsigned long long kmax;
+};
+
 struct cbgpu_hashtable
 {
 	cbgpu_ctx  *ctx;
@@ -230,11 +252,17 @@
 	cbgpu_rel  *inner;
 	int64_t		nslots;
 	int64_t		ninserted;
-	int		   *d_flags;
+	HtFillOut  *d_fill;
 	int			has_dups;
+	int64_t		kmin;
+	int64_t		kmax;
+	uint32_t   *xbits;
+	uint64_t	xnbits;
 	int64_t		total_rows;
 	int64_t		built_bytes;
 };
+
+int			cb_ht_exact(cbgpu_hashtable *ht);
 
 static inline int
 cb_fail(cbgpu_ctx *ctx, int code, const char *fmt, const char *a = "", long long b = 0)
diff --git a/cloudberry_b200/csrc/ctx.cu b/cloudberry_b200/csrc/ctx.cu
--- a/cloudberry_b200/csrc/ctx.cu
+++ b/cloudberry_b200/csrc/ctx.cu
@@ -27,6 +27,7 @@
 	CB_CUDA(ctx, cudaSetDevice(device));
 	CB_CUDA(ctx, cudaGetDeviceProperties(&prop, device));
 	ctx->sm_count = prop.multiProcessorCount;
+	ctx->smem_per_sm = (int64_t) prop.sharedMemPerMultiprocessor;
 	CB_CUDA(ctx, cudaStreamCreateWithFlags(&ctx->stream, cudaStreamNonBlocking));
 	{
 		cudaMemPool_t pool;
diff --git a/cloudberry_b200/csrc/exec/cb_exec.c b/cloudberry_b200/csrc/exec/cb_exec.c
--- a/cloudberry_b200/csrc/exec/cb_exec.c
+++ b/cloudberry_b200/csrc/exec/cb_exec.c
@@ -3238,6 +3238,80 @@
 	return node->ExecProcNode(node);
 }
 
+char *
+cb_ExecDrainText(CbPlanState *node, int64_t *ntuples)
+{
+	size_t		cap = 4096,
+				len = 0;
+	char	   *buf = (char *) malloc(cap);
+
+	*ntuples = 0;
+	if (!buf)
+		return NULL;
+	buf[0] = '\0';
+	for (;;)
+	{
+		CbTupleTableSlot *slot = node->ExecProcNode(node);
+
+		if (node->state->es_errcode || !slot || slot->tts_empty)
+			break;
+		for (int i = 0; i < slot->tts_nvalid; i++)
+		{
+			if (cap - len < 256)
+			{
+				char	   *nb = (char *) realloc(buf, cap * 2);
+
+				if (!nb)
+				{
+					free(buf);
+					return NULL;
+				}
+				buf = nb;
+				cap *= 2;
+			}
+			const int	t = slot->tts_types[i];
+			const char *sep = i + 1 < slot->tts_nvalid ? "\t" : "\n";
+			const long long n = (long long) slot->tts_state_n[i],
+						lo = (long long) slot->tts_state_lo[i],
+						hi = (long long) slot->tts_state_hi[i];
+
+			if (slot->tts_isnull[i])
+				len += (size_t) snprintf(buf + len, cap - len, "N 0 %lld %lld %lld%s", n, lo, hi, sep);
+			else if (t == CB_NUMERIC || t == CB_NUMERIC128)
+				len += (size_t) snprintf(buf + len, cap - len, "s %s %lld %lld %lld%s",
+										 ((CbNumericDatum *) (intptr_t) slot->tts_values[i])->text, n, lo, hi, sep);
+			else
+				len += (size_t) snprintf(buf + len, cap - len, "%c %lld %lld %lld %lld%s", t == CB_FLOAT8 ? 'f' : 'i',
+										 (long long) slot->tts_values[i], n, lo, hi, sep);
+		}
+		if (slot->tts_nvalid == 0)
+		{
+			if (cap - len < 2)
+			{
+				char	   *nb = (char *) realloc(buf, cap * 2);
+
+				if (!nb)
+				{
+					free(buf);
+					return NULL;
+				}
+				buf = nb;
+				cap *= 2;
+			}
+			buf[len++] = '\n';
+			buf[len] = '\0';
+		}
+		(*ntuples)++;
+	}
+	return buf;
+}
+
+void
+cb_free_text(char *p)
+{
+	free(p);
+}
+
 cbgpu_hashtable *
 cb_MultiExecProcNode(CbPlanState *node)
 {
diff --git a/cloudberry_b200/csrc/hashtable.cu b/cloudberry_b200/csrc/hashtable.cu
--- a/cloudberry_b200/csrc/hashtable.cu
+++ b/cloudberry_b200/csrc/hashtable.cu
@@ -7,7 +7,7 @@
 {
 	HtDev		ht;
 	int64_t		nrows;
-	int		   *flags;
+	HtFillOut  *out;
 };
 
 __device__ __forceinline__ bool
@@ -55,12 +55,21 @@
 	int			inserted = 0;
 	bool		dup = false;
 	bool		outside = false;
+	unsigned long long kmin_inv = 0, kmax = 0;
 
 	for (int64_t i = (int64_t) blockIdx.x * blockDim.x + threadIdx.x; i < p.nrows; i += stride)
 	{
 		uint32_t	h = 0, w;
 		int64_t		key0 = 0;
 		bool		v = ht_row_hash(p.ht, (uint32_t) i, &h, &key0);
+
+		if (v)
+		{
+			const unsigned long long o = (unsigned long long) key0 ^ (1ull << 63);
+
+			kmin_inv = max(kmin_inv, ~o);
+			kmax = max(kmax, o);
+		}
 
 		if (v && !ht_in_batch(p.ht.nbatch, p.ht.batch_shift, p.ht.batch_id, h))
 			v = false;
@@ -103,13 +112,43 @@
 		inserted++;
 	}
 	if (dup)
-		atomicExch(p.flags, 1);
+		atomicExch(p.out->flags, 1);
 	if (outside)
-		atomicExch(p.flags + 2, 1);
+		atomicExch(p.out->flags + 2, 1);
 	for (int o = 16; o; o >>= 1)
 		inserted += __shfl_xor_sync(0xffffffffu, inserted, o);
 	if ((threadIdx.x & 31) == 0 && inserted)
-		atomicAdd(p.flags + 1, inserted);
+		atomicAdd(p.out->flags + 1, inserted);
+	if (ht_exact_type(p.ht.keytype[0]))
+	{
+		for (int o = 16; o; o >>= 1)
+		{
+			kmin_inv = max(kmin_inv, __shfl_xor_sync(0xffffffffu, kmin_inv, o));
+			kmax = max(kmax, __shfl_xor_sync(0xffffffffu, kmax, o));
+		}
+		if ((threadIdx.x & 31) == 0 && (kmin_inv | kmax))
+		{
+			atomicMax(&p.out->kmin_inv, kmin_inv);
+			atomicMax(&p.out->kmax, kmax);
+		}
+	}
+}
+
+__global__ void
+k_ht_exact_build(HtDev ht, int64_t nrows, uint32_t *bits, int64_t kmin)
+{
+	for (int64_t i = (int64_t) blockIdx.x * blockDim.x + threadIdx.x; i < nrows; i += (int64_t) gridDim.x * blockDim.x)
+	{
+		uint32_t	h;
+		int64_t		key0;
+
+		if (ht_row_hash(ht, (uint32_t) i, &h, &key0) && ht_in_batch(ht.nbatch, ht.batch_shift, ht.batch_id, h))
+		{
+			const uint64_t off = (uint64_t) key0 - (uint64_t) kmin;
+
+			atomicOr(bits + (off >> 5), 1u << (off & 31));
+		}
+	}
 }
 
 static int
@@ -118,7 +157,7 @@
 	cbgpu_ctx  *ctx = ht->ctx;
 	cbgpu_rel  *inner = ht->inner;
 	BuildParams p;
-	int			h_flags[3];
+	HtFillOut	h_out;
 
 	ht->d.batch_id = batch;
 	if (ht->d.bloom)
@@ -127,14 +166,14 @@
 	{
 		int			blocks = (int) ((ht->nslots + 255) / 256);
 
-		CB_CUDA(ctx, cudaMemsetAsync(ht->d_flags, 0, 3 * sizeof(int), ctx->stream));
+		CB_CUDA(ctx, cudaMemsetAsync(ht->d_fill, 0, sizeof(HtFillOut), ctx->stream));
 		if (blocks > ctx->sm_count * 8)
 			blocks = ctx->sm_count * 8;
 		k_ht_clear<<<blocks, 256, 0, ctx->stream>>>(ht->d.slots, (size_t) ht->nslots);
 		CB_LAUNCHED(ctx, "k_ht_clear");
 		p.ht = ht->d;
 		p.nrows = inner->nrows;
-		p.flags = ht->d_flags;
+		p.out = ht->d_fill;
 		if (inner->nrows > 0)
 		{
 			blocks = (int) ((inner->nrows + 255) / 256);
@@ -143,9 +182,9 @@
 			k_ht_build<<<blocks, 256, 0, ctx->stream>>>(p);
 			CB_LAUNCHED(ctx, "k_ht_build");
 		}
-		CB_CUDA(ctx, cudaMemcpyAsync(h_flags, ht->d_flags, sizeof(h_flags), cudaMemcpyDeviceToHost, ctx->stream));
+		CB_CUDA(ctx, cudaMemcpyAsync(&h_out, ht->d_fill, sizeof(h_out), cudaMemcpyDeviceToHost, ctx->stream));
 		CB_CUDA(ctx, cudaStreamSynchronize(ctx->stream));
-		if (h_flags[2] && ht->d.keyslot)
+		if (h_out.flags[2] && ht->d.keyslot)
 		{
 			ht->d.keyslot = 0;
 			if (ht->d.bloom)
@@ -154,9 +193,39 @@
 		}
 		break;
 	}
-	if (h_flags[0])
+	if (h_out.flags[0])
 		ht->has_dups = 1;
-	ht->ninserted = h_flags[1];
+	ht->ninserted = h_out.flags[1];
+	ht->kmin = (int64_t) (~h_out.kmin_inv ^ (1ull << 63));
+	ht->kmax = (int64_t) (h_out.kmax ^ (1ull << 63));
+	if (ht->xbits)
+		CB_CUDA(ctx, cudaFreeAsync(ht->xbits, ctx->stream));
+	ht->xbits = NULL;
+	ht->xnbits = 0;
+	return CBGPU_OK;
+}
+
+int
+cb_ht_exact(cbgpu_hashtable *ht)
+{
+	cbgpu_ctx  *ctx = ht->ctx;
+	const uint64_t nbits = ht->d.nkeys == 1 && ht->d.bloom && ht_exact_type(ht->d.keytype[0]) ?
+		ht_exact_nbits(ht->kmin, ht->kmax, ((uint64_t) ht->d.bloom_mask + 1) * 32) : 0;
+
+	if (ht->xbits || !nbits)
+		return CBGPU_OK;
+	const size_t bytes = (size_t) ((nbits + 127) / 128) * 16;
+	int			blocks = (int) ((ht->inner->nrows + 255) / 256);
+
+	if (blocks > ctx->sm_count * 8)
+		blocks = ctx->sm_count * 8;
+	if (blocks < 1)
+		blocks = 1;
+	CB_CUDA(ctx, cudaMallocAsync(&ht->xbits, bytes, ctx->stream));
+	CB_CUDA(ctx, cudaMemsetAsync(ht->xbits, 0, bytes, ctx->stream));
+	ht->xnbits = nbits;
+	k_ht_exact_build<<<blocks, 256, 0, ctx->stream>>>(ht->d, ht->inner->nrows, ht->xbits, ht->kmin);
+	CB_LAUNCHED(ctx, "k_ht_exact_build");
 	return CBGPU_OK;
 }
 
@@ -257,7 +326,7 @@
 	ht->nslots = nslots;
 	ht->d.mask = (uint32_t) (nslots - 1);
 	CB_CUDA(ctx, cudaMallocAsync(&ht->d.slots, (size_t) nslots * sizeof(unsigned long long), ctx->stream));
-	CB_CUDA(ctx, cudaMallocAsync(&ht->d_flags, 3 * sizeof(int), ctx->stream));
+	CB_CUDA(ctx, cudaMallocAsync(&ht->d_fill, sizeof(HtFillOut), ctx->stream));
 	if (nkeys == 1)
 		switch (ht->d.keytype[0])
 		{
@@ -354,7 +423,9 @@
 	cudaFreeAsync(ht->d.slots, ht->ctx->stream);
 	if (ht->d.bloom)
 		cudaFreeAsync(ht->d.bloom, ht->ctx->stream);
-	cudaFreeAsync(ht->d_flags, ht->ctx->stream);
+	if (ht->xbits)
+		cudaFreeAsync(ht->xbits, ht->ctx->stream);
+	cudaFreeAsync(ht->d_fill, ht->ctx->stream);
 	free(ht);
 }
 
diff --git a/cloudberry_b200/csrc/probe_chain.cu b/cloudberry_b200/csrc/probe_chain.cu
--- a/cloudberry_b200/csrc/probe_chain.cu
+++ b/cloudberry_b200/csrc/probe_chain.cu
@@ -51,6 +51,9 @@
 	int32_t		hashtype;
 	const uint32_t *bloom;
 	uint32_t	mask;
+	const uint32_t *bits;
+	int64_t		kmin;
+	uint64_t	nbits;
 };
 
 struct PcParams
@@ -730,52 +733,63 @@
 		}
 }
 
+static inline bool
+pc_exact_ok(int32_t probe_type, int32_t build_type)
+{
+	return (probe_type == CB_INT4 || probe_type == CB_DATE) && ht_exact_type(build_type);
+}
+
 template <bool WIDE>
 __device__ __forceinline__ unsigned
-pc_early_filter8(const PcEarly &E, int64_t row0, bool full, unsigned am, uint64_t pol)
-{
-	const PcKeys8 keys = pc_warp_dense(full, am) ? pc_keys8_vec<WIDE>(E.col, row0, pol) : pc_keys8_pred<WIDE>(E.col, row0, am, pol);
-	uint32_t	bits[8], word[8];
-
+pc_filter8_keys(const PcEarly &E, const uint32_t *bits, const PcKeys8 &keys, unsigned am)
+{
+	uint32_t	m[8], word[8];
+
+	if (!WIDE && E.bits)
+	{
+		const int64_t kmin = E.kmin;
+		const uint32_t kmin32 = (uint32_t) kmin, nbits = (uint32_t) E.nbits;
+		unsigned	hit = 0;
+
+#pragma unroll
+		for (int u = 0; u < 8; u++)
+		{
+			const int64_t kv = pc_keys8_get<WIDE>(keys, u);
+			const uint32_t off = (uint32_t) kv - kmin32;
+
+			if (((am >> u) & 1) && off < nbits && (uint64_t) (kv - kmin) == off)
+				hit |= ((bits[off >> 5] >> (off & 31)) & 1u) << u;
+		}
+		return am & hit;
+	}
 #pragma unroll
 	for (int u = 0; u < 8; u++)
 	{
 		const int64_t kv = pc_keys8_get<WIDE>(keys, u);
 		uint32_t	w;
 
-		bits[u] = ht_bloom_bits(pg_hash_combine(0u, WIDE ? jh_int8(kv) : jh_mix32((uint32_t) (int32_t) kv), false), &w, E.mask);
+		m[u] = ht_bloom_bits(pg_hash_combine(0u, WIDE ? jh_int8(kv) : jh_mix32((uint32_t) (int32_t) kv), false), &w, E.mask);
 		word[u] = ((am >> u) & 1) ? __ldg(E.bloom + w) : 0u;
 	}
 #pragma unroll
 	for (int u = 0; u < 8; u++)
-		if ((word[u] & bits[u]) != bits[u])
+		if ((word[u] & m[u]) != m[u])
 			am &= ~(1u << u);
 	return am;
 }
 
 template <bool WIDE>
 __device__ __forceinline__ unsigned
-pc_bloom8_keys(const PcEarly &E, const PcKeys8 &keys, unsigned am)
-{
-	uint32_t	bits[8], word[8];
-
-#pragma unroll
-	for (int u = 0; u < 8; u++)
-	{
-		const int64_t kv = pc_keys8_get<WIDE>(keys, u);
-		uint32_t	w;
-
-		bits[u] = ht_bloom_bits(pg_hash_combine(0u, WIDE ? jh_int8(kv) : jh_mix32((uint32_t) (int32_t) kv), false), &w, E.mask);
-		word[u] = ((am >> u) & 1) ? __ldg(E.bloom + w) : 0u;
-	}
-#pragma unroll
-	for (int u = 0; u < 8; u++)
-		if ((word[u] & bits[u]) != bits[u])
-			am &= ~(1u << u);
-	return am;
+pc_early_filter8(const PcEarly &E, const uint32_t *bits, int64_t row0, bool full, unsigned am, uint64_t pol)
+{
+	const PcKeys8 keys = pc_warp_dense(full, am) ? pc_keys8_vec<WIDE>(E.col, row0, pol) : pc_keys8_pred<WIDE>(E.col, row0, am, pol);
+
+	return pc_filter8_keys<WIDE>(E, bits, keys, am);
 }
 
 #define PF_MAXBLOOM 6
+#define PF_SMEM_THREADS 1024
+#define PF_SMEM_BUDGET (160 * 1024)
 struct PfParams
 {
 	int64_t		nrows;
@@ -788,22 +802,33 @@
 	unsigned long long *out_count;
 };
 
-template <bool SPEC>
-__global__ void __launch_bounds__(PC_THREADS, SPEC ? 4 : 8)
+template <bool SPEC, bool SMEM>
+__global__ void __launch_bounds__(SMEM ? PF_SMEM_THREADS : PC_THREADS, SMEM ? (SPEC ? 1 : 2) : (SPEC ? 4 : 8))
 k_prefilter(const __grid_constant__ PfParams P)
 {
-	__shared__ uint32_t buf[PC_TILE];
+	constexpr int THREADS = SMEM ? PF_SMEM_THREADS : PC_THREADS;
+	constexpr int TILE = THREADS * 8;
+	__shared__ uint32_t buf[TILE];
 	__shared__ unsigned s_cnt;
 	__shared__ unsigned long long s_gbase;
-	const int64_t ntiles = (P.nrows + PC_TILE - 1) / PC_TILE;
+	extern __shared__ __align__(16) uint32_t s_bits[];
+	const int64_t ntiles = (P.nrows + TILE - 1) / TILE;
 	const unsigned o0 = threadIdx.x * 8;
 	const int	lane = threadIdx.x & 31;
 	const uint64_t pol_stream = l2_policy_evict_first();
 
+	if (SMEM)
+	{
+		const unsigned nvec = (unsigned) ((P.bloom[0].nbits + 127) / 128);
+
+		for (unsigned i = threadIdx.x; i < nvec; i += THREADS)
+			((uint4 *) s_bits)[i] = __ldg((const uint4 *) P.bloom[0].bits + i);
+		__syncthreads();
+	}
 	for (int64_t tile = blockIdx.x; tile < ntiles; tile += gridDim.x)
 	{
-		const int64_t base = tile * PC_TILE;
-		const unsigned nvalid = (unsigned) (P.nrows - base < PC_TILE ? P.nrows - base : PC_TILE);
+		const int64_t base = tile * TILE;
+		const unsigned nvalid = (unsigned) (P.nrows - base < TILE ? P.nrows - base : TILE);
 		const bool	full = o0 + 8 <= nvalid;
 		unsigned	am = 0;
 
@@ -867,11 +892,13 @@
 			}
 		for (int f = 0; f < P.nbloom && __any_sync(0xffffffffu, am != 0); f++)
 		{
+			const uint32_t *bits = SMEM && f == 0 ? s_bits : P.bloom[f].bits;
+
 			if (SPEC && f == 0 && have0)
-				am = P.bloom[0].width == 8 ? pc_bloom8_keys<true>(P.bloom[0], keys0, am) : pc_bloom8_keys<false>(P.bloom[0], keys0, am);
+				am = P.bloom[0].width == 8 ? pc_filter8_keys<true>(P.bloom[0], bits, keys0, am) : pc_filter8_keys<false>(P.bloom[0], bits, keys0, am);
 			else
-				am = P.bloom[f].width == 8 ? pc_early_filter8<true>(P.bloom[f], base + o0, full, am, pol_stream)
-					: pc_early_filter8<false>(P.bloom[f], base + o0, full, am, pol_stream);
+				am = P.bloom[f].width == 8 ? pc_early_filter8<true>(P.bloom[f], bits, base + o0, full, am, pol_stream)
+					: pc_early_filter8<false>(P.bloom[f], bits, base + o0, full, am, pol_stream);
 		}
 		__syncthreads();
 		{
@@ -903,7 +930,7 @@
 		if (threadIdx.x == 0 && s_cnt)
 			s_gbase = atomicAdd(P.out_count, (unsigned long long) s_cnt);
 		__syncthreads();
-		for (unsigned i = threadIdx.x; i < s_cnt; i += PC_THREADS)
+		for (unsigned i = threadIdx.x; i < s_cnt; i += THREADS)
 			P.out[s_gbase + i] = buf[i];
 		__syncthreads();
 	}
@@ -1057,8 +1084,8 @@
 					am |= (unsigned) alive << u;
 				}
 			for (int f = 0; f < P.nearly && __any_sync(0xffffffffu, am != 0); f++)
-				am = P.early[f].width == 8 ? pc_early_filter8<true>(P.early[f], base + o0, full, am, pol_stream)
-					: pc_early_filter8<false>(P.early[f], base + o0, full, am, pol_stream);
+				am = P.early[f].width == 8 ? pc_early_filter8<true>(P.early[f], P.early[f].bits, base + o0, full, am, pol_stream)
+					: pc_early_filter8<false>(P.early[f], P.early[f].bits, base + o0, full, am, pol_stream);
 			if (P.fuse0 && pc_warp_dense(full, am, 96u))
 			{
 				if (wide0)
@@ -1192,6 +1219,8 @@
 	int32_t		red_keytype[PC_MAXP][2];
 	uint32_t   *bloom;
 	uint32_t	mask;
+	uint32_t   *xbits;
+	int64_t		xmin;
 	unsigned long long *passed;
 };
 
@@ -1240,17 +1269,36 @@
 			}
 			ok = found;
 		}
-		if (ok && !B.bloom)
+		if (ok && !B.bloom && !B.xbits)
 			atomicAdd(B.passed, 1ull);
-		if (ok && B.bloom)
+		if (ok && (B.bloom || B.xbits))
 		{
 			uint32_t	w;
 			const int64_t kv = cb_load_widen(B.self.keydata[B.kc], B.self.keytype[B.kc], (uint32_t) r);
-			const uint32_t bits = ht_bloom_bits(pg_hash_combine(0u, jh_hash_datum(B.hashtype, kv, NULL), false), &w, B.mask);
-
-			atomicOr(B.bloom + w, bits);
-		}
-	}
+			const uint64_t off = (uint64_t) kv - (uint64_t) B.xmin;
+
+			if (B.xbits)
+				atomicOr(B.xbits + (off >> 5), 1u << (off & 31));
+			else
+			{
+				const uint32_t bits = ht_bloom_bits(pg_hash_combine(0u, jh_hash_datum(B.hashtype, kv, NULL), false), &w, B.mask);
+
+				atomicOr(B.bloom + w, bits);
+			}
+		}
+	}
+}
+
+static size_t
+pf_bytes(const PcEarly &e)
+{
+	return e.bits ? (size_t) ((e.nbits + 127) / 128) * 16 : ((size_t) e.mask + 1) * sizeof(uint32_t);
+}
+
+static void
+pf_print_form(const PcEarly &e, bool smem)
+{
+	fprintf(stderr, ", %s %zu B", !e.bits ? "bloom" : smem ? "bitmap-smem" : "bitmap-l2", pf_bytes(e));
 }
 
 #define PC_REJECT(n) \
@@ -1577,14 +1625,20 @@
 		}
 		while (words < inner->nrows / 2)
 			words <<= 1;
-		CB_CUDA(ctx, cudaMallocAsync(&early_mem[P.nearly], (size_t) words * sizeof(uint32_t), ctx->stream));
-		CB_CUDA(ctx, cudaMemsetAsync(early_mem[P.nearly], 0, (size_t) words * sizeof(uint32_t), ctx->stream));
+		const cbgpu_hashtable *T = p->probes[k].ht;
+		const uint64_t nbits = kc == 0 && pc_exact_ok(q->key[kc].type, q->ht.keytype[kc]) ? ht_exact_nbits(T->kmin, T->kmax, (uint64_t) words * 32) : 0;
+		const size_t bytes = nbits ? (size_t) ((nbits + 127) / 128) * 16 : (size_t) words * sizeof(uint32_t);
+
+		CB_CUDA(ctx, cudaMallocAsync(&early_mem[P.nearly], bytes, ctx->stream));
+		CB_CUDA(ctx, cudaMemsetAsync(early_mem[P.nearly], 0, bytes, ctx->stream));
 		B.nrows = inner->nrows;
 		B.self = q->ht;
 		B.kc = kc;
 		B.hashtype = q->keytype[kc];
-		B.bloom = (uint32_t *) early_mem[P.nearly];
+		B.bloom = nbits ? NULL : (uint32_t *) early_mem[P.nearly];
 		B.mask = (uint32_t) (words - 1);
+		B.xbits = nbits ? (uint32_t *) early_mem[P.nearly] : NULL;
+		B.xmin = T->kmin;
 		{
 			int			eb = (int) ((inner->nrows + 255) / 256);
 
@@ -1598,6 +1652,9 @@
 		P.early[P.nearly].hashtype = q->keytype[kc];
 		P.early[P.nearly].bloom = B.bloom;
 		P.early[P.nearly].mask = B.mask;
+		P.early[P.nearly].bits = B.xbits;
+		P.early[P.nearly].kmin = B.xmin;
+		P.early[P.nearly].nbits = nbits;
 		P.nearly++;
 	}
 	uint32_t   *pf_sel = NULL;
@@ -1636,9 +1693,30 @@
 			F.bloom[F.nbloom].hashtype = q.keytype[0];
 			F.bloom[F.nbloom].bloom = q.ht.bloom;
 			F.bloom[F.nbloom].mask = q.ht.bloom_mask;
+			if (pc_exact_ok(q.key[0].type, q.ht.keytype[0]))
+			{
+				const int	rc = cb_ht_exact(const_cast<cbgpu_hashtable *>(p->probes[j].ht));
+
+				if (rc != CBGPU_OK)
+					return rc;
+				F.bloom[F.nbloom].bits = p->probes[j].ht->xbits;
+				F.bloom[F.nbloom].kmin = p->probes[j].ht->kmin;
+				F.bloom[F.nbloom].nbits = p->probes[j].ht->xnbits;
+			}
 			F.nbloom++;
 			pf_cand[j] = true;
 		}
+		for (int f = 0; f < F.nbloom; f++)
+			if (F.bloom[f].bits && pf_bytes(F.bloom[f]) <= PF_SMEM_BUDGET)
+			{
+				const PcEarly e = F.bloom[f];
+
+				for (int g = f; g > 0; g--)
+					F.bloom[g] = F.bloom[g - 1];
+				F.bloom[0] = e;
+				break;
+			}
+		const bool	pf_smem = F.nbloom > 0 && F.bloom[0].bits && pf_bytes(F.bloom[0]) <= PF_SMEM_BUDGET;
 		for (int i = 0; i < ctx->pf_cache_n; i++)
 			if (ctx->pf_cache[i] == sig)
 				known_unselective = true;
@@ -1654,16 +1732,38 @@
 			F.out_count = pf_count;
 			const int	pkl = cb_klog_begin(ctx, "k_prefilter");
 
-			if (ctx->opt_pf_spec)
-				k_prefilter<true><<<ctx->sm_count * 4 < ft ? ctx->sm_count * 4 : (int) ft, PC_THREADS, 0, ctx->stream>>>(F);
+			if (pf_smem)
+			{
+				const size_t sm = pf_bytes(F.bloom[0]);
+				const void *kf = ctx->opt_pf_spec ? (const void *) k_prefilter<true, true> : (const void *) k_prefilter<false, true>;
+				int64_t		occ = ctx->smem_per_sm / ((int64_t) sm + PF_SMEM_THREADS * 8 * 4 + 2048);
+				const int64_t fts = (P.nrows + PF_SMEM_THREADS * 8 - 1) / (PF_SMEM_THREADS * 8);
+
+				occ = occ < 1 ? 1 : occ > (ctx->opt_pf_spec ? 1 : 2) ? (ctx->opt_pf_spec ? 1 : 2) : occ;
+				const int	grid = (int) (ctx->sm_count * occ < fts ? ctx->sm_count * occ : fts);
+
+				CB_CUDA(ctx, cudaFuncSetAttribute(kf, cudaFuncAttributeMaxDynamicSharedMemorySize, PF_SMEM_BUDGET));
+
+				if (ctx->opt_pf_spec)
+					k_prefilter<true, true><<<grid, PF_SMEM_THREADS, sm, ctx->stream>>>(F);
+				else
+					k_prefilter<false, true><<<grid, PF_SMEM_THREADS, sm, ctx->stream>>>(F);
+			}
+			else if (ctx->opt_pf_spec)
+				k_prefilter<true, false><<<ctx->sm_count * 4 < ft ? ctx->sm_count * 4 : (int) ft, PC_THREADS, 0, ctx->stream>>>(F);
 			else
-				k_prefilter<false><<<ctx->sm_count * 8 < ft ? ctx->sm_count * 8 : (int) ft, PC_THREADS, 0, ctx->stream>>>(F);
+				k_prefilter<false, false><<<ctx->sm_count * 8 < ft ? ctx->sm_count * 8 : (int) ft, PC_THREADS, 0, ctx->stream>>>(F);
 			CB_LAUNCHED(ctx, "k_prefilter");
 			cb_klog_end(ctx, pkl);
 			CB_CUDA(ctx, cudaMemcpyAsync(&nsel, pf_count, sizeof(nsel), cudaMemcpyDeviceToHost, ctx->stream));
 			CB_CUDA(ctx, cudaStreamSynchronize(ctx->stream));
 			if (ctx->opt_debug)
-				fprintf(stderr, "k_prefilter: %lld of %lld rows survive %d qual(s) + %d filter(s)\n", (long long) nsel, (long long) P.nrows, F.nfilters, F.nbloom);
+			{
+				fprintf(stderr, "k_prefilter: %lld of %lld rows survive %d qual(s) + %d filter(s)", (long long) nsel, (long long) P.nrows, F.nfilters, F.nbloom);
+				for (int f = 0; f < F.nbloom; f++)
+					pf_print_form(F.bloom[f], pf_smem && f == 0);
+				fputc('\n', stderr);
+			}
 			if (nsel * (unsigned long long) ctx->opt_pf_keep_div <= (unsigned long long) P.nrows)
 			{
 				P.sel = pf_sel;
@@ -1727,7 +1827,12 @@
 				(long long) P.nrows, (long long) ntiles, blocks, (long long) words, P.nfilters, P.sink_kind, P.probe[0].kind,
 				P.probe[1].kind, P.probe[2].kind, P.probe[3].kind);
 	if (ctx->opt_debug && P.nearly)
-		fprintf(stderr, "k_probe_chain: %d scan-level runtime filter(s)\n", P.nearly);
+	{
+		fprintf(stderr, "k_probe_chain: %d scan-level runtime filter(s)", P.nearly);
+		for (int f = 0; f < P.nearly; f++)
+			pf_print_form(P.early[f], false);
+		fputc('\n', stderr);
+	}
 	CB_CUDA(ctx, cudaEventRecord(ctx->ev_k0, ctx->stream));
 	int			kl = cb_klog_begin(ctx, "k_probe_chain");
 
diff --git a/include/cb_exec.h b/include/cb_exec.h
--- a/include/cb_exec.h
+++ b/include/cb_exec.h
@@ -87,6 +87,8 @@
 
 CbPlanState *cb_ExecInitNode(CbPlan *node, CbEState *estate, int eflags);
 CbTupleTableSlot *cb_ExecProcNode(CbPlanState *node);
+char	   *cb_ExecDrainText(CbPlanState *node, int64_t *ntuples);
+void		cb_free_text(char *p);
 cbgpu_hashtable *cb_MultiExecProcNode(CbPlanState *node);
 int			cb_ExecProcNodeBatch(CbPlanState *node, cbgpu_rel **out);
 void		cb_ExecEndNode(CbPlanState *node);
```

Result: no change. 81.33 billion (median of 6 runs) (+0.6%).
